# JaapWijnen/metal-raytracing

Hardware: AMD Instinct MI355X
Metric: Mrays/sec (primary+shadow) and ms/frame, DragonScene 1920x1080 spp=1 (higher is better)
Workload: dtype f32

## Files before the change

### include/mrt_debug.h

```cpp
#ifndef MRT_DEBUG_H
#define MRT_DEBUG_H
#include "mrt_abi.h"
#ifdef __cplusplus
extern "C" {
#endif

int mrt_debug_renderer_set_option(MRTRenderer r, const char *key, double value);
int mrt_debug_renderer_get_option(MRTRenderer r, const char *key, double *value);

int mrt_debug_halton(MRTContext ctx, const int32_t *i, const int32_t *d, size_t n, float *out);
int mrt_debug_hemisphere(MRTContext ctx, const float *u2, const float *normal3, size_t n, float *out3);
int mrt_debug_seeds(MRTContext ctx, uint32_t seed, int32_t width, int32_t height, uint32_t *out);
int mrt_debug_traversal_stats(MRTScene scene, const MRTRay *rays, size_t n, int32_t any_hit, uint32_t *out8);
int mrt_debug_stream_stats(MRTScene scene, const MRTRay *rays, size_t n, int32_t any_hit, uint32_t per_wave, uint32_t *out8, size_t nwaves);
int mrt_debug_intersect_stream(MRTScene scene, const MRTRay *rays, size_t n, int32_t any_hit, MRTIntersection *out);
int mrt_debug_wide_histogram(MRTScene scene, uint32_t *out12);
int mrt_debug_read_wnodes(MRTScene scene, void *out, size_t nbytes, uint64_t *num_nodes);
int mrt_debug_read_layout(MRTScene scene, int32_t part, void *out, size_t nbytes, uint64_t *count);
int mrt_debug_scene_refits(MRTScene scene, uint32_t *out);
int mrt_debug_commit_times(MRTScene scene, double *out6);
int mrt_debug_validate(MRTScene scene);
int mrt_debug_validate_patched(MRTScene scene, uint32_t node, uint32_t word, uint32_t value);
#ifdef MRT_DIAGNOSTICS
int mrt_debug_poke_wnode(MRTScene scene, uint32_t node, uint32_t word, uint32_t value, uint32_t *old_value);
#endif
int mrt_debug_host_sah(const float *lo4, const float *hi4, uint32_t n, uint32_t *order, uint32_t *left, uint32_t *right, uint32_t *parent);
int mrt_debug_tlas_host_build(const float *lo4, const float *hi4, uint32_t n, uint32_t *rope_order, uint32_t *rope_links, uint32_t *wide_order, uint32_t *wide_pos, uint32_t *counts68);
int mrt_debug_layout_limits(uint64_t triangles, uint64_t nodes);
int mrt_debug_calibrate(MRTContext ctx, size_t table_bytes, double *out5);

#ifdef __cplusplus
}
#endif
#endif
```

### metal-raytracing_amd/_ffi.py

```python
import ctypes as C
import os

_HERE = os.path.dirname(os.path.abspath(__file__))
LIB_PATH = os.environ.get("MRT_LIB_PATH") or os.path.join(_HERE, "libmrt_hip.so")

MRT_OK = 0
MRT_ERR_INVALID_ARGUMENT, MRT_ERR_NO_DEVICE, MRT_ERR_HIP, MRT_ERR_IO, MRT_ERR_STATE, MRT_ERR_OUT_OF_MEMORY, MRT_ERR_UNSUPPORTED = 1, 2, 3, 4, 5, 6, 7


class MRTError(RuntimeError):
    def __init__(self, code, message):
        super().__init__(f"mrt error {code}: {message}")
        self.code = code


class Float3(C.Structure):
    _fields_ = [("x", C.c_float), ("y", C.c_float), ("z", C.c_float), ("_pad", C.c_float)]

    def __init__(self, x=0.0, y=0.0, z=0.0):
        super().__init__(float(x), float(y), float(z), 0.0)

    def tolist(self):
        return [self.x, self.y, self.z]

# ... 128 lines not shown
    "mrt_scene_refit_device": (C.c_int, [_P, _P]),
    "mrt_scene_device_updates_rejected": (C.c_int, [_P, C.POINTER(C.c_uint64)]),
    "mrt_scene_set_instance_transforms_device": (C.c_int, [_P, _I32, _SZ, _P, _SZ, _P]),
    "mrt_scene_refit_instances_device": (C.c_int, [_P, _P]),
    "mrt_scene_rebuild_tlas_device": (C.c_int, [_P, _P]),
    "mrt_scene_update_blas_device": (C.c_int, [_P, _I32, _P, _SZ, _P, _SZ, _SZ, _P]),
    "mrt_scene_refit_blas_device": (C.c_int, [_P, _P]),
    "mrt_scene_resolve_hits_device": (C.c_int, [_P, _P, _P, _SZ, _P, _P]),
    "mrt_scene_interpolate_device": (C.c_int, [_P, _P, _SZ, _P, _SZ, _I32, _P, _SZ, _P]),
    "mrt_scene_vertex_offsets": (C.c_int, [_P, C.POINTER(C.c_uint64), _SZ]),
    "mrt_obj_load": (C.c_int, [C.c_char_p, C.POINTER(_P)]),
    "mrt_dragon_proxy": (C.c_int, [C.POINTER(_P)]),
    "mrt_dragon_proxy_irregular": (C.c_int, [C.POINTER(_P)]),
    "mrt_dragon_proxy_hostile": (C.c_int, [C.POINTER(_P)]),
    "mrt_bunny_proxy": (C.c_int, [C.POINTER(_P)]),
    "mrt_meshdata_free": (C.c_int, [_P]),
    "mrt_meshdata_counts": (C.c_int, [_P, C.POINTER(_SZ), _PI32]),
    "mrt_meshdata_vertices": (C.c_int, [_P, _P, _P]),
    "mrt_meshdata_submesh": (C.c_int, [_P, _I32, C.POINTER(_SZ), _P, C.POINTER(Material), C.c_char_p, _SZ]),
    "mrt_make_transform": (C.c_int, [_PF, _PF, _F, _PF]),
    "mrt_default_camera": (C.c_int, [_I32, _I32, C.POINTER(Camera)]),
    "mrt_renderer_create": (C.c_int, [_P, _P, _I32, _I32, _U32, _I32, C.POINTER(_P)]),
    "mrt_renderer_destroy": (C.c_int, [_P]),
    "mrt_renderer_resize": (C.c_int, [_P, _I32, _I32]),
    "mrt_renderer_set_camera": (C.c_int, [_P, C.POINTER(Camera)]),
    "mrt_renderer_set_uniforms": (C.c_int, [_P, C.POINTER(Uniforms)]),
    "mrt_renderer_get_uniforms": (C.c_int, [_P, C.POINTER(Uniforms)]),
    "mrt_renderer_frames_completed": (C.c_int, [_P, C.POINTER(C.c_uint64)]),
    "mrt_renderer_set_option": (C.c_int, [_P, C.c_char_p, C.c_double]),
    "mrt_renderer_get_option": (C.c_int, [_P, C.c_char_p, _P]),
    "mrt_debug_renderer_set_option": (C.c_int, [_P, C.c_char_p, C.c_double]),
    "mrt_debug_renderer_get_option": (C.c_int, [_P, C.c_char_p, _P]),
    "mrt_renderer_set_shard": (C.c_int, [_P, _I32, _I32]),
    "mrt_renderer_set_frame_index": (C.c_int, [_P, _U32]),
    "mrt_renderer_frame_index": (C.c_int, [_P, _PU32]),
    "mrt_renderer_render": (C.c_int, [_P, _I32]),
    "mrt_renderer_wait": (C.c_int, [_P]),
    "mrt_renderer_read_accum": (C.c_int, [_P, _P, _SZ]),
    "mrt_renderer_copy_accum_to_device": (C.c_int, [_P, _P, _SZ]),
    "mrt_renderer_write_accum_from_device": (C.c_int, [_P, _P, _SZ]),
    "mrt_renderer_shard_tiles": (C.c_int, [_P, _I32, _I32, C.POINTER(C.c_uint64)]),
    "mrt_renderer_pack_owned_tiles": (C.c_int, [_P, _P, _SZ]),
    "mrt_renderer_unpack_tiles": (C.c_int, [_P, _P, _SZ, _I32, _I32]),
    "mrt_renderer_unpack_tiles_into": (C.c_int, [_P, _P, _SZ, _P, _SZ, _I32, _I32]),
    "mrt_renderer_read_tonemapped_rgba8": (C.c_int, [_P, _P, _SZ]),
    "mrt_renderer_read_guide": (C.c_int, [_P, _I32, _P, _SZ]),
    "mrt_renderer_copy_guide_to_device": (C.c_int, [_P, _I32, _P, _SZ]),
    "mrt_renderer_denoise": (C.c_int, [_P, C.POINTER(DenoiseParams)]),
    "mrt_renderer_read_denoised": (C.c_int, [_P, _P, _SZ]),
    "mrt_renderer_copy_denoised_to_device": (C.c_int, [_P, _P, _SZ]),
    "mrt_renderer_read_denoised_tonemapped_rgba8": (C.c_int, [_P, _P, _SZ]),
    "mrt_renderer_stats": (C.c_int, [_P, C.POINTER(RenderStats)]),
    "mrt_renderer_reset_stats": (C.c_int, [_P]),
    "mrt_renderer_kernel_times": (C.c_int, [_P, C.POINTER(KernelTimes)]),
    "mrt_group_create": (C.c_int, [_PI32, _I32, C.POINTER(_P)]),
    "mrt_group_destroy": (C.c_int, [_P]),
    "mrt_group_size": (C.c_int, [_P, _PI32]),
    "mrt_group_context": (C.c_int, [_P, _I32, C.POINTER(_P)]),
    "mrt_group_reduce_mode": (C.c_int, [_P, _PI32, C.c_char_p, _SZ]),
    "mrt_group_set_reduce_mode": (C.c_int, [_P, _I32]),
    "mrt_group_renderer_create": (C.c_int, [_P, _P, _I32, _I32, _U32, _I32, C.POINTER(_P)]),
    "mrt_group_renderer_destroy": (C.c_int, [_P]),
    "mrt_group_renderer_rank": (C.c_int, [_P, _I32, C.POINTER(_P)]),
    "mrt_group_set_option": (C.c_int, [_P, C.c_char_p, C.c_double]),
    "mrt_group_set_camera": (C.c_int, [_P, C.POINTER(Camera)]),
    "mrt_group_render": (C.c_int, [_P, _I32]),
    "mrt_group_wait": (C.c_int, [_P]),
    "mrt_group_frames_completed": (C.c_int, [_P, C.POINTER(C.c_uint64)]),
    "mrt_group_gather": (C.c_int, [_P, _P, _SZ]),
    "mrt_group_gathered_device_ptr": (C.c_int, [_P, C.POINTER(_P)]),
    "mrt_group_stats": (C.c_int, [_P, C.POINTER(RenderStats)]),
    "mrt_debug_halton": (C.c_int, [_P, _P, _P, _SZ, _P]),
    "mrt_debug_hemisphere": (C.c_int, [_P, _P, _P, _SZ, _P]),
    "mrt_debug_seeds": (C.c_int, [_P, _U32, _I32, _I32, _P]),
    "mrt_debug_traversal_stats": (C.c_int, [_P, _P, _SZ, _I32, _P]),
    "mrt_debug_intersect_stream": (C.c_int, [_P, _P, _SZ, _I32, _P]),
    "mrt_debug_stream_stats": (C.c_int, [_P, _P, _SZ, _I32, _U32, _P, _SZ]),
    "mrt_debug_calibrate": (C.c_int, [_P, _SZ, _P]),
    "mrt_debug_wide_histogram": (C.c_int, [_P, _P]),
    "mrt_debug_commit_times": (C.c_int, [_P, _P]),
    "mrt_debug_read_wnodes": (C.c_int, [_P, _P, _SZ, C.POINTER(C.c_uint64)]),
    "mrt_debug_read_layout": (C.c_int, [_P, _I32, _P, _SZ, C.POINTER(C.c_uint64)]),
    "mrt_debug_layout_limits": (C.c_int, [C.c_uint64, C.c_uint64]),
    "mrt_debug_host_sah": (C.c_int, [_P, _P, _U32, _P, _P, _P, _P]),
    "mrt_debug_tlas_host_build": (C.c_int, [_P, _P, _U32, _P, _P, _P, _P, _P]),
    "mrt_debug_validate": (C.c_int, [_P]),
    "mrt_debug_validate_patched": (C.c_int, [_P, _U32, _U32, _U32]),
}

os.environ.setdefault("GPU_MAX_HW_QUEUES", "16")

if not os.path.exists(LIB_PATH):
    raise ImportError(
        f"{LIB_PATH} is missing: the HIP extension has not been built. Run `python -c 'import __graft_entry__ as g; g.build()'` "
        "or `make -C metal-raytracing_amd/csrc`. There is no CPU fallback for the render path.")



def _share_hip_runtime_with_torch():
    import sys
    if "torch" in sys.modules or os.environ.get("MRT_HIP_RUNTIME", "") == "system":
        return None
    try:
        import importlib.util
        spec = importlib.util.find_spec("torch")
    except (ImportError, ValueError):
        return None
    if spec is None or not spec.submodule_search_locations:
        return None
    libdir = os.path.join(list(spec.submodule_search_locations)[0], "lib")
    loaded = []
    for name in ("libhsa-runtime64.so", "libamdhip64.so"):
        path = os.path.join(libdir, name)
        if os.path.exists(path):
            try:
                C.CDLL(path)
                loaded.append(path)
            except OSError:
                return loaded
    return loaded


HIP_RUNTIME_PRELOADED = _share_hip_runtime_with_torch()
lib = C.CDLL(LIB_PATH)
for _name, (_res, _args) in SIGNATURES.items():
    if os.environ.get("MRT_LIB_PATH") and not hasattr(lib, _name):
        continue
    _fn = getattr(lib, _name)
    _fn.restype, _fn.argtypes = _res, _args


def check(rc):
    if rc != MRT_OK:
        raise MRTError(rc, lib.mrt_last_error().decode("utf-8", "replace"))


def ptr(a):
    return a.ctypes.data_as(C.c_void_p)
```

### metal-raytracing_amd/csrc/api.cpp

```cpp
#include "api_types.h"
#include "abi_check.h"
#include "../../include/mrt_debug.h"
#include <algorithm>
#include <cstring>
#include <cstdio>
#include <memory>
#include <new>

namespace mrt {
static thread_local std::string g_err;
void set_error(const std::string &msg) { g_err = msg; }
int hip_fail(hipError_t e, const char *what, const char *file, int line) {
    char buf[512];
    snprintf(buf, sizeof buf, "HIP error %d (%s) in %s at %s:%d", (int)e, hipGetErrorString(e), what, file, line);
    g_err = buf;
    return e == hipErrorOutOfMemory ? MRT_ERR_OUT_OF_MEMORY : MRT_ERR_HIP;
}
}

static int bind_device(MRTContext ctx) { MRT_HIP(hipSetDevice(ctx->device)); return MRT_OK; }

static int sync_host_meshes(MRTScene scene) {
    bool pending = false;
    int rc = mrt::download_stale_meshes(scene->meshes, scene->dev, &pending);
// ... 650 lines not shown
int mrt_renderer_resize(MRTRenderer r, int32_t width, int32_t height) {
    MRT_TRY
    RENDERER_PROLOGUE("mrt_renderer_resize")
    REQUIRE(width > 0 && height > 0 && (int64_t)width * height < (1ll << 30), "mrt_renderer_resize: bad size");
    MRT_HIP(hipStreamSynchronize(r->r.stream));
    return r->r.resize(width, height);
    MRT_CATCH
}
int mrt_renderer_set_camera(MRTRenderer r, const MRTCamera *camera) {
    REQUIRE(r && camera, "mrt_renderer_set_camera: bad argument");
    r->r.camera = *camera;
    return MRT_OK;
}
int mrt_renderer_set_uniforms(MRTRenderer r, const MRTUniforms *u) {
    MRT_TRY
    RENDERER_PROLOGUE("mrt_renderer_set_uniforms")
    REQUIRE(u, "mrt_renderer_set_uniforms: uniforms is NULL");
    REQUIRE(u->width > 0 && u->height > 0 && (int64_t)u->width * u->height < (1ll << 30), "mrt_renderer_set_uniforms: bad size");
    REQUIRE(u->lightCount >= 1 && u->lightCount <= r->scene->dev.light_count, "mrt_renderer_set_uniforms: lightCount must be in [1, lights of the scene]");
    if (u->width != r->r.width || u->height != r->r.height) {
        MRT_HIP(hipStreamSynchronize(r->r.stream));
        int rc = r->r.resize(u->width, u->height); if (rc) return rc;
    }
    r->r.frame_index = u->frameIndex;
    r->r.light_count_limit = u->lightCount == r->scene->dev.light_count ? 0 : u->lightCount;
    r->r.camera = u->camera;
    return MRT_OK;
    MRT_CATCH
}
int mrt_renderer_get_uniforms(MRTRenderer r, MRTUniforms *u) {
    REQUIRE(r && u, "mrt_renderer_get_uniforms: bad argument");
    memset(u, 0, sizeof *u);
    u->width = r->r.width; u->height = r->r.height; u->blocksWide = (r->r.width + 7) / 8;
    u->frameIndex = r->r.frame_index;
    u->lightCount = r->r.light_count_limit > 0 ? std::min(r->r.light_count_limit, r->scene->dev.light_count) : r->scene->dev.light_count;
    u->camera = r->r.camera;
    return MRT_OK;
}
int mrt_renderer_frames_completed(MRTRenderer r, uint64_t *frames) {
    MRT_TRY
    RENDERER_PROLOGUE("mrt_renderer_frames_completed")
    REQUIRE(frames, "mrt_renderer_frames_completed: NULL");
    return r->r.poll_completed(frames);
    MRT_CATCH
}
int mrt_renderer_set_option(MRTRenderer r, const char *key, double value) {
    MRT_TRY
    REQUIRE(r && key, "mrt_renderer_set_option: bad argument");
    std::string k(key);
    if (k == "max_bounces") { REQUIRE(value >= 1 && value <= (r->r.materials ? 16 : 19), "max_bounces must be in [1,19] ([1,16] with materials = 1)"); r->r.max_bounces = (int)value; }
    else if (k == "frames_in_flight") { REQUIRE(value >= 1 && value <= mrt::MAX_FRAMES_IN_FLIGHT, "frames_in_flight must be in [1,16]"); r->r.frames_in_flight = (int)value; }
    else if (k == "sample_offset") { REQUIRE(value >= 0 && value < 4294967296.0, "sample_offset out of range"); r->r.sample_offset = (uint32_t)value; }
    else if (k == "frame_batch") { REQUIRE(value >= 0 && value <= mrt::MAX_FRAME_BATCH, "frame_batch must be in [1,32], or 0 for the default (by image size)"); r->r.frame_batch = (int)value; }
    else if (k == "megakernel") r->r.megakernel = value != 0;
    else if (k == "guides") { REQUIRE(value == 0 || value == 1, "guides must be 0 or 1"); int rc = bind_device(r->ctx); if (rc) return rc; r->r.stream = r->ctx->stream; rc = r->r.set_guides(value != 0); if (rc) return rc; }
    else if (k == "materials") { REQUIRE(value == 0 || (value == 1 && r->r.max_bounces <= 16), "materials must be 0 or 1 (and max_bounces <= 16: the lobe choice uses Halton dimension 2 + 5 * max_bounces + bounce < 100)"); r->r.materials = value != 0; }
    else { mrt::set_error("mrt_renderer_set_option: unknown key " + k + " (keys: max_bounces, frames_in_flight, sample_offset, frame_batch, megakernel, materials, guides; the library's A/B switches are behind mrt_debug_renderer_set_option)"); return MRT_ERR_INVALID_ARGUMENT; }
    return MRT_OK;
    MRT_CATCH
}
int mrt_renderer_get_option(MRTRenderer r, const char *key, double *value) {
    MRT_TRY
    REQUIRE(r && key && value, "mrt_renderer_get_option: bad argument");
    std::string k(key);
    if (k == "max_bounces") *value = r->r.max_bounces;
    else if (k == "frames_in_flight") *value = r->r.frames_in_flight;
    else if (k == "sample_offset") *value = r->r.sample_offset;
    else if (k == "frame_batch") *value = r->r.batch_wanted();
    else if (k == "megakernel") *value = r->r.megakernel ? 1 : 0;
    else if (k == "materials") *value = r->r.materials ? 1 : 0;
    else if (k == "guides") *value = r->r.guides ? 1 : 0;
    else if (k == "lanes_used") *value = r->r.lanes_used;
    else if (k == "lane_bytes") *value = (double)r->r.lane_bytes();
    else { mrt::set_error("mrt_renderer_get_option: unknown key " + k); return MRT_ERR_INVALID_ARGUMENT; }
    return MRT_OK;
    MRT_CATCH
}
int mrt_debug_renderer_set_option(MRTRenderer r, const char *key, double value) {
    MRT_TRY
    REQUIRE(r && key, "mrt_debug_renderer_set_option: bad argument");
    std::string k(key);
    if (k == "persistent") { REQUIRE(value == 0 || value == 1 || value == 2, "persistent must be 0 (never), 1 (always) or 2 (by launch size)"); r->r.persistent = (int)value; }
    else if (k == "xcd_counters") { REQUIRE(value == 0 || value == 1, "xcd_counters must be 0 or 1"); r->r.xcd_counters = (int)value; }
    else if (k == "tile_groups") { REQUIRE(value >= 0 && value <= mrt::MAX_TILE_GROUPS && value == (int)value, "tile_groups must be 0 (by the draw), 1 (never) or 2..4"); r->r.tile_groups = (int)value; }
    else if (k == "shade_pack") { REQUIRE(value == 0 || value == 1, "shade_pack must be 0 or 1"); r->r.shade_pack = (int)value; }
    else if (k == "hit_lds") { REQUIRE(value == 0 || value == 1, "hit_lds must be 0 or 1"); r->r.hit_lds = (int)value; }
    else if (k == "persist_chunk") { REQUIRE(value >= 64 && value <= 65536 && ((int)value % 64) == 0, "persist_chunk must be a multiple of 64 in [64, 65536]"); r->r.persist_chunk = (int)value; }
    else if (k == "wave_slots") { REQUIRE(value >= 1 && value <= (1 << 20), "wave_slots must be in [1, 2^20]"); r->r.wave_slots = (int)value; r->r.wave_slots_user = true; }
    else if (k == "stream_stride") { REQUIRE(value >= 0 && value <= 2, "stream_stride must be 0 (contiguous ranges), 1 (round-robin batches) or 2 (round-robin for a shard's launches)"); r->r.stream_stride = (int)value; }
    else if (k == "halton_table") r->r.halton_table = value != 0;
    else if (k == "equal_passes") r->r.equal_passes = value != 0;
    else if (k == "frame_bundle") { REQUIRE(value == 0 || value == 1, "frame_bundle must be 0 (off) or 1 (the sub-frames of a slot side by side in a wave)"); r->r.frame_bundle = (int)value; }
    else if (k == "stream_even") { REQUIRE(value >= 0 && value <= 1600, "stream_even must be in [0,1600] (percent of the wave slots; 0 = off)"); r->r.stream_even = (int)value; }
    else if (k == "primary_hint") r->r.primary_hint = value != 0;
    else if (k == "throughput_chain") r->r.throughput_chain = value != 0;
    else if (k == "shadow_planes") r->r.shadow_planes = value != 0 ? 1 : 0;
    else if (k == "tail_accumulate") r->r.tail_accumulate = value != 0;
    else if (k == "fuse_primary") { REQUIRE(value == 0 || value == 1 || value == 2, "fuse_primary must be 0, 1 (not for one frame alone) or 2 (always)"); r->r.fuse_primary = (int)value; }
    else if (k == "wide_bounce") r->r.wide_bounce = value != 0;
    else if (k == "tl_pair_cap") { REQUIRE(value >= 0 && value <= 4294967295.0, "tl_pair_cap out of range"); r->r.tl_pair_cap = (int)std::min(value, 2147483647.0); }
    else if (k == "tl_pairs") { REQUIRE(value == 0 || value == 1 || value == 2, "tl_pairs must be 0 (two-level scenes walked in one loop), 1 (TLAS pass + BLAS pass over (ray, instance) pairs) or 2 (the same, the TLAS pass always as a walk of the 8-wide TLAS)"); r->r.tl_pairs = (int)value; }
    else if (k == "primary_wide") { REQUIRE(value == 0 || value == 1 || value == 2, "primary_wide must be 0 (rope walk inside shade(0)), 1 (own launch of the 8-wide stream kernel) or 2 (8-wide walk inside shade(0))"); r->r.primary_wide = (int)value; }
    else return mrt_renderer_set_option(r, key, value);
    return MRT_OK;
    MRT_CATCH
}
int mrt_debug_renderer_get_option(MRTRenderer r, const char *key, double *value) {
    MRT_TRY
    REQUIRE(r && key && value, "mrt_debug_renderer_get_option: bad argument");
    std::string k(key);
    if (k == "persistent") *value = r->r.persistent;
    else if (k == "persist_chunk") *value = r->r.persist_chunk;
    else if (k == "hit_lds") *value = r->r.hit_lds;
    else if (k == "shade_pack") *value = r->r.shade_pack;
    else if (k == "tile_groups") *value = r->r.tile_groups;
    else if (k == "groups_used") *value = r->r.groups_used;
    else if (k == "xcd_counters") *value = r->r.xcd_counters;
    else if (k == "wave_slots") *value = r->r.wave_slots;
    else if (k == "stream_stride") *value = r->r.stream_stride;
    else if (k == "halton_table") *value = r->r.halton_table;
    else if (k == "frame_bundle") *value = r->r.frame_bundle;
    else if (k == "stream_even") *value = r->r.stream_even;
    else if (k == "primary_hint") *value = r->r.primary_hint ? 1 : 0;
    else if (k == "throughput_chain") *value = r->r.throughput_chain ? 1 : 0;
    else if (k == "shadow_planes") *value = r->r.shadow_planes;
    else if (k == "tail_accumulate") *value = r->r.tail_accumulate ? 1 : 0;
    else if (k == "fuse_primary") *value = r->r.fuse_primary;
    else if (k == "wide_bounce") *value = r->r.wide_bounce ? 1 : 0;
    else if (k == "tl_pairs") *value = r->r.tl_pairs;
    else if (k == "tl_pair_cap") *value = r->r.tl_pair_cap;
    else if (k == "primary_wide") *value = r->r.primary_wide;
    else return mrt_renderer_get_option(r, key, value);
    return MRT_OK;
    MRT_CATCH
}
int mrt_renderer_set_shard(MRTRenderer r, int32_t rank, int32_t world) {
    MRT_TRY
    RENDERER_PROLOGUE("mrt_renderer_set_shard")
    return r->r.set_shard(rank, world);
    MRT_CATCH
}
int mrt_renderer_set_frame_index(MRTRenderer r, uint32_t fi) { REQUIRE(r, "mrt_renderer_set_frame_index: NULL"); r->r.frame_index = fi; return MRT_OK; }
int mrt_renderer_frame_index(MRTRenderer r, uint32_t *fi) { REQUIRE(r && fi, "mrt_renderer_frame_index: bad argument"); *fi = r->r.frame_index; return MRT_OK; }
int mrt_renderer_render(MRTRenderer r, int32_t n_frames) {
    MRT_TRY
    RENDERER_PROLOGUE("mrt_renderer_render")
    REQUIRE(n_frames >= 0, "mrt_renderer_render: n_frames < 0");
    if (!r->scene->committed) { mrt::set_error("mrt_renderer_render: scene was modified and not re-committed"); return MRT_ERR_STATE; }
    if (n_frames == 0) return MRT_OK;
    return r->r.render(n_frames);
    MRT_CATCH
}
int mrt_renderer_wait(MRTRenderer r) {
    MRT_TRY
    RENDERER_PROLOGUE("mrt_renderer_wait")
    return r->r.wait();
    MRT_CATCH
}
int mrt_renderer_read_accum(MRTRenderer r, float *rgba, size_t nbytes) {
    MRT_TRY
    RENDERER_PROLOGUE("mrt_renderer_read_accum")
    REQUIRE(rgba, "mrt_renderer_read_accum: NULL buffer");
    return r->r.read_accum(rgba, nbytes);
    MRT_CATCH
}
int mrt_renderer_copy_accum_to_device(MRTRenderer r, void *dptr, size_t nbytes) {
    MRT_TRY
    RENDERER_PROLOGUE("mrt_renderer_copy_accum_to_device")
    REQUIRE(dptr, "mrt_renderer_copy_accum_to_device: NULL pointer");
    return r->r.copy_accum_to_device(dptr, nbytes);
    MRT_CATCH
}
int mrt_renderer_write_accum_from_device(MRTRenderer r, const void *dptr, size_t nbytes) {
    MRT_TRY
    RENDERER_PROLOGUE("mrt_renderer_write_accum_from_device")
    REQUIRE(dptr, "mrt_renderer_write_accum_from_device: NULL pointer");
    return r->r.write_accum_from_device(dptr, nbytes);
    MRT_CATCH
}
int mrt_renderer_shard_tiles(MRTRenderer r, int32_t rank, int32_t world, uint64_t *tiles) {
    REQUIRE(r && tiles && world >= 1 && rank >= 0 && rank < world, "mrt_renderer_shard_tiles: bad argument");
    *tiles = mrt::shard_tiles(r->r.width, r->r.height, rank, world);
    return MRT_OK;
}
int mrt_renderer_pack_owned_tiles(MRTRenderer r, void *dptr, size_t nbytes) {
    MRT_TRY
    RENDERER_PROLOGUE("mrt_renderer_pack_owned_tiles")
    REQUIRE(dptr || nbytes == 0, "mrt_renderer_pack_owned_tiles: NULL pointer");
    return r->r.pack_owned_tiles(dptr, nbytes);
    MRT_CATCH
}
int mrt_renderer_unpack_tiles(MRTRenderer r, const void *dptr, size_t nbytes, int32_t rank, int32_t world) {
    MRT_TRY
    RENDERER_PROLOGUE("mrt_renderer_unpack_tiles")
    REQUIRE(dptr || nbytes == 0, "mrt_renderer_unpack_tiles: NULL pointer");
    return r->r.unpack_tiles(dptr, nbytes, rank, world);
    MRT_CATCH
}
int mrt_renderer_unpack_tiles_into(MRTRenderer r, void *image, size_t image_nbytes, const void *dptr, size_t nbytes, int32_t rank, int32_t world) {
    MRT_TRY
// ... 121 lines not shown
int mrt_debug_read_layout(MRTScene scene, int32_t part, void *out, size_t nbytes, uint64_t *count) {
    MRT_TRY
    REQUIRE(scene && count, "mrt_debug_read_layout: bad argument");
    REQUIRE(part >= 0 && part <= 7, "mrt_debug_read_layout: part must be 0 .. 7");
    if (!scene->committed) { mrt::set_error("mrt_debug_read_layout: scene not committed"); return MRT_ERR_STATE; }
    const mrt::DeviceScene &d = scene->dev;
    const size_t npk = d.wpackets.p ? d.wpackets.n / mrt::WPK : 0, ninst = d.num_inst, nwt = (d.num_inst && d.wtlas_index.p) ? d.wtlas_index.n : 0;
    uint32_t header[8] = {d.num_wnodes, d.num_inst ? d.tlas_wcap : 0u, d.num_inst, (uint32_t)d.wide_depth, (uint32_t)npk, (uint32_t)d.blas_wdepth, (uint32_t)nwt, mrt::WPK};
    const size_t nrope = d.num_inst ? d.rope_nodes : 0, ntl = d.num_inst ? d.tlas_instances : 0;
    const size_t elem[8] = {16 * (size_t)mrt::WNODE_STRIDE, 16 * (size_t)mrt::WPK, sizeof(mrt::InstanceDev), 64, 4, 4, 64, 4};
    const size_t n[8] = {d.num_wnodes, npk, ninst, ninst, nwt, 8, nrope, ntl};
    const void *src[8] = {d.wnodes.p, d.wpackets.p, d.inst.p, d.inst_box.p, d.wtlas_index.p, header, d.nodes.p, d.tlas_index.p};
    *count = n[part];
    if (out == nullptr) return MRT_OK;
    REQUIRE(nbytes == n[part] * elem[part], "mrt_debug_read_layout: nbytes must be count x the element size of the part");
    if (n[part] == 0) return MRT_OK;
    if (part == 5) { memcpy(out, header, sizeof(header)); return MRT_OK; }
    int rc = bind_device(scene->ctx); if (rc) return rc;
    MRT_HIP(hipMemcpy(out, src[part], nbytes, hipMemcpyDeviceToHost));
    return MRT_OK;
    MRT_CATCH
}
int mrt_debug_scene_refits(MRTScene scene, uint32_t *out) {
    REQUIRE(scene && out, "mrt_debug_scene_refits: bad argument");
    *out = scene->dev.refits;
    return MRT_OK;
}
int mrt_debug_commit_times(MRTScene scene, double *out6) {
    REQUIRE(scene && out6, "mrt_debug_commit_times: bad argument");
    for (int k = 0; k < 6; k++) out6[k] = scene->dev.commit_ms[k];
    return MRT_OK;
}
int mrt_debug_validate(MRTScene scene) {
    MRT_TRY
    REQUIRE(scene, "mrt_debug_validate: scene is NULL");
    if (!scene->committed) { mrt::set_error("mrt_debug_validate: scene not committed"); return MRT_ERR_STATE; }
    int rc = bind_device(scene->ctx); if (rc) return rc;
    return mrt::validate_layout(scene->dev, scene->ctx->stream, false);
    MRT_CATCH
}
int mrt_debug_validate_patched(MRTScene scene, uint32_t node, uint32_t word, uint32_t value) {
    MRT_TRY
    REQUIRE(scene && scene->committed && node < scene->dev.num_wnodes && word < 4 * mrt::WNODE_STRIDE, "mrt_debug_validate_patched: bad argument");
    int rc = bind_device(scene->ctx); if (rc) return rc;
    mrt::DevBuf<float4> copy; MRT_HIP(copy.alloc(scene->dev.wnodes.n));
    MRT_HIP(hipMemcpy(copy.p, scene->dev.wnodes.p, scene->dev.wnodes.bytes(), hipMemcpyDeviceToDevice));
    MRT_HIP(hipMemcpy(reinterpret_cast<uint32_t *>(copy.p + (size_t)mrt::WNODE_STRIDE * node) + word, &value, 4, hipMemcpyHostToDevice));
    return mrt::validate_layout(scene->dev, scene->ctx->stream, false, copy.p);
    MRT_CATCH
}
#ifdef MRT_DIAGNOSTICS
int mrt_debug_poke_wnode(MRTScene scene, uint32_t node, uint32_t word, uint32_t value, uint32_t *old_value) {
    MRT_TRY
    REQUIRE(scene && scene->committed && node < scene->dev.num_wnodes && word < 4 * mrt::WNODE_STRIDE, "mrt_debug_poke_wnode: bad argument");
    int rc = bind_device(scene->ctx); if (rc) return rc;
    uint32_t *p = reinterpret_cast<uint32_t *>(scene->dev.wnodes.p + (size_t)mrt::WNODE_STRIDE * node) + word;
    if (old_value) MRT_HIP(hipMemcpy(old_value, p, 4, hipMemcpyDeviceToHost));
    MRT_HIP(hipMemcpy(p, &value, 4, hipMemcpyHostToDevice));
    return MRT_OK;
    MRT_CATCH
}
#endif
int mrt_debug_host_sah(const float *lo4, const float *hi4, uint32_t n, uint32_t *order, uint32_t *left, uint32_t *right, uint32_t *parent) {
    MRT_TRY
    REQUIRE(lo4 && hi4 && n >= 1 && order && left && right && parent, "mrt_debug_host_sah: bad argument");
    std::vector<uint32_t> o, l, r, p;
    mrt::host_sah_topology(reinterpret_cast<const float4 *>(lo4), reinterpret_cast<const float4 *>(hi4), n, o, l, r, p);
    memcpy(order, o.data(), (size_t)n * 4); memcpy(parent, p.data(), (2 * (size_t)n - 1) * 4);
    if (n > 1) { memcpy(left, l.data(), (size_t)(n - 1) * 4); memcpy(right, r.data(), (size_t)(n - 1) * 4); }
    return MRT_OK;
    MRT_CATCH
}
int mrt_debug_tlas_host_build(const float *lo4, const float *hi4, uint32_t n, uint32_t *rope_order, uint32_t *rope_links, uint32_t *wide_order, uint32_t *wide_pos, uint32_t *counts68) {
    MRT_TRY
    REQUIRE(lo4 && hi4 && n >= 1 && n <= 65536 && rope_order && rope_links && wide_order && wide_pos && counts68, "mrt_debug_tlas_host_build: bad argument");
    return mrt::tlas_host_build(lo4, hi4, n, rope_order, rope_links, wide_order, wide_pos, counts68);
    MRT_CATCH
}
int mrt_debug_layout_limits(uint64_t triangles, uint64_t nodes) {
    MRT_TRY
    return mrt::layout_limits(triangles, nodes);
    MRT_CATCH
}
int mrt_debug_calibrate(MRTContext ctx, size_t table_bytes, double *out3) {
    MRT_TRY
    REQUIRE(ctx && out3 && table_bytes >= 4096 && table_bytes <= ((size_t)1 << 34), "mrt_debug_calibrate: bad argument");
    int rc = bind_device(ctx); if (rc) return rc;
    return mrt::calibrate(ctx->stream, table_bytes, out3);
    MRT_CATCH
}

}
```

### metal-raytracing_amd/csrc/renderer.h

```cpp
#pragma once
#include "scene_device.h"
#include "host_geometry.h"
#include <algorithm>
#include <array>
#include <deque>
#include <vector>

namespace mrt {

struct EvPair { hipEvent_t a = nullptr, b = nullptr; int kind = 0; };

struct FrameLane {
    hipStream_t stream = nullptr;
    hipEvent_t accumulated = nullptr;
    DevBuf<float4> sample;
    DevBuf<float4> rayA[2], rayB[2], thr[2], hits, srayA, srayB, scon;
    DevBuf<unsigned long long> bounce_counts;
    DevBuf<float4> f_con[2];
    DevBuf<uint8_t> f_lit;
    DevBuf<uint4> pairs;
};
constexpr int MAX_FRAMES_IN_FLIGHT = 16;
constexpr int MAX_TILE_GROUPS = 4;
struct TileGroup { int rank = 0, world = 1, tiles_local = 0; uint32_t capacity = 0; uint64_t owned = 0; const uint32_t *seeds = nullptr; };
constexpr int MAX_FRAME_BATCH = 32;
constexpr int DEFAULT_FRAME_BATCH = 8;

struct DrawPlan {
    int n_frames = 0;
    bool mega = false;
    bool equal = true, tail = true;
    int batch_max = 1;
    int n_passes = 0;
    int G = 1;
    int lanes = 1;
    int lanes_plain = 1;
    int Fp = 1;
    int tail_from = 0;
    bool long_call = false;
    int pass_size(int p) const { return equal ? n_frames / n_passes + (p < n_frames % n_passes ? 1 : 0) : std::min(batch_max, n_frames - p * batch_max); }
    void settle(int lanes_ready);
};

enum class PrimaryForm { none, stream, lane_wide, rope };
enum class TraceForm { pairs, pull_x, pull, static_x, static_split, rope };
struct PullGrid { uint32_t chunk = 0, waves = 0; size_t grid_slots = 0; };
struct PassPlan {
    int B = 0;
    uint32_t grid_tiles = 1, grid_shade = 1;
    bool two_level = false, on_wide = false, chain = false, planes = false, pairs = false, tl_flat = false, prim_rope = false;
    bool trace0_pass = false, trace0_wide = false, trace0_hint = false, primary_hinted = false, bundle = false, pull = false, strided = false;
    PrimaryForm primary = PrimaryForm::none;
    TraceForm trace = TraceForm::rope;
    size_t stack_bytes = 0, trace_lds = 0, pair_cap = 0;
    uint32_t pair_cap_used = 0, rpw_p = 0, rpw_m = 0, pack_range = 0;
    int wave_slots = 0;
    PullGrid pg;
    uint32_t even = 0, static_grid = 0;
    uint32_t mega_waves = 0;
};
struct SlotCache { size_t lds_bytes = ~(size_t)0; int per_cu = 0; };
struct DrawCtx;

struct Renderer {
    hipStream_t stream = nullptr;
    const DeviceScene *scene = nullptr;
    int width = 0, height = 0, max_bounces = 3;
    uint32_t seed = 1;
    MRTCamera camera{};
    uint32_t frame_index = 0;
    uint32_t sample_offset = 0;
    int cur = 0;
    int shard_rank = 0, shard_world = 1;
    int tiles_local = 0;
    uint32_t capacity = 0;
    uint64_t owned_pixels = 0;
    uint64_t frames_rendered = 0;

    DevBuf<uint32_t> seeds;
    DevBuf<float> halton_tab;
    uint32_t halton_w0 = 0;
    int halton_table = 1;
    int ensure_halton_table(uint32_t sample_index, uint32_t frames);
    DevBuf<uint32_t> hint;
    bool primary_hint = true;
    bool throughput_chain = true;
    DevBuf<float4> accum[2];
    FrameLane lanes[MAX_FRAMES_IN_FLIGHT];
    int frames_in_flight = 3;
    int frame_batch = 0;
    int batch_wanted() const;
    int tile_groups = 0;
    int groups_used = 1;
    TileGroup tgroups[MAX_TILE_GROUPS];
    DevBuf<uint32_t> seeds_g[MAX_TILE_GROUPS]; int tgroups_for = 0, tgroups_batch = 0;
    int ensure_tile_groups(int G);
    int lanes_used = 0;
    int lanes_ready = 0;
    int alloc_batch = 0;
    bool megakernel = false;
    bool materials = false;
    int primary_wide = 2;
    int persistent = 2;
    int xcd_counters = 1;
    int hit_lds = 1;
    int shade_pack = 1;
    int persist_chunk = 256;
    int wave_slots = 7168;
    bool wave_slots_user = false;
    mutable SlotCache mega_cache, persist_cache, persist_x_cache;
    mutable int cu_count = 0;
    int alloc_planes(FrameLane &L);
    bool tail_accumulate = true;
    int fuse_primary = 1;
    int shadow_planes = 1;
    int equal_passes = 1;
    int frame_bundle = 1;
    int stream_stride = 2;
    int stream_even = 200;
    int tl_pair_cap = 0;
    int tl_pairs = 1;
    bool wide_bounce = true;
    hipEvent_t ev_fork = nullptr;
    DevBuf<unsigned long long> totals;

    bool guides = false;
    bool guides_valid = false;
    bool guides_keep = false;
    DevBuf<float4> guide_nd, guide_albedo; DevBuf<int4> guide_ids;
    hipStream_t guide_stream = nullptr;
    hipEvent_t guide_fork = nullptr, guide_done = nullptr;
    DevBuf<float4> dn_scratch[2], denoised; bool denoised_valid = false;
    int set_guides(bool on);
    int ensure_guides();
    int clear_guides();
    int read_guide(int which, void *out, size_t nbytes);
    int copy_guide_to_device(int which, void *dptr, size_t nbytes);
    int enqueue_denoise(const MRTDenoiseParams *params);
    int read_denoised(float *rgba, size_t nbytes);
    int copy_denoised_to_device(void *dptr, size_t nbytes);
    int read_denoised_tonemapped(uint8_t *rgba, size_t nbytes);

    int light_count_limit = 0;
    struct PassDone { hipEvent_t ev; uint64_t frames_through; };
    std::deque<PassDone> passes_pending;
    std::vector<hipEvent_t> pass_events_free;
    uint64_t frames_completed_known = 0;
    int note_pass(hipStream_t st);
    int poll_completed(uint64_t *out);

    hipEvent_t ev_begin = nullptr, ev_end = nullptr;
    std::array<EvPair, 512> ev_ext;
    int ext_used = 0;
    bool pending_timing = false;
    float ms_last = 0, ms_extend_last = 0; uint32_t extend_launches_last = 0;
    MRTKernelTimes kernel_times{};

    Renderer() = default;
    Renderer(const Renderer &) = delete;
    ~Renderer();
    int init(hipStream_t st, const DeviceScene *sc, int w, int h, uint32_t seed, int max_bounces);
    int resize(int w, int h);
    int alloc_queues();
    int alloc_lane(FrameLane &L);
    void release_lane(FrameLane &L);
    size_t lane_bytes() const;
    int set_shard(int rank, int world);
    int render(int n_frames);
    DrawPlan plan_draw(int n_frames) const;
    int plan_pass(const DrawPlan &dp, const SceneView &sv, const TileGroup &TG, int B, PassPlan &pp) const;
    PullGrid pull_grid(size_t slots, size_t slots_of_chip, size_t min_chunk, bool long_call) const;
    int draw_nothing(int n_frames);
    int rebuild_for_batch();
    int ensure_lanes(int want);
    void begin_draw(DrawCtx &d) const;
    int prepare_lane(FrameLane &L, const TileGroup &TG, const PassPlan &pp);
    int enqueue_pass(DrawCtx &d, FrameLane &L, const TileGroup &TG, const PassPlan &pp, int pass, int g);
    int enqueue_megakernel_pass(DrawCtx &d, FrameLane &L, const TileGroup &TG, const PassPlan &pp);
    void enqueue_primary(DrawCtx &d, FrameLane &L, const TileGroup &TG, const PassPlan &pp);
    void enqueue_shade(DrawCtx &d, FrameLane &L, const TileGroup &TG, const PassPlan &pp, int b);
    void enqueue_trace(DrawCtx &d, FrameLane &L, const TileGroup &TG, const PassPlan &pp, int b);
    int enqueue_accumulate(DrawCtx &d, FrameLane &L, const TileGroup &TG, const PassPlan &pp, int pass, int g);
    int enqueue_guides(DrawCtx &d);
    EvPair *timed(int kind);
    int wait();
    int read_accum(float *rgba, size_t nbytes);
    int copy_accum_to_device(void *dptr, size_t nbytes);
    int write_accum_from_device(const void *dptr, size_t nbytes);
    int read_tonemapped(uint8_t *rgba, size_t nbytes);
    int pack_owned_tiles(void *dptr, size_t nbytes);
    int unpack_tiles(const void *dptr, size_t nbytes, int rank, int world);
    int stats(MRTRenderStats *out);
    int reset_stats();
// ... 19 lines not shown
```

### metal-raytracing_amd/csrc/renderer.hip

```cpp
#include <hip/hip_ext.h>
#include "renderer.h"
#include "device_math.h"
#include "traverse.h"
#include "traverse_wide.h"
#include "traverse_instanced.h"
#include "shade.h"
#include "two_level_passes.h"
#include <cstdlib>
#include <cstring>
#include <algorithm>

namespace mrt {
namespace {

__global__ void k_halton_table(float *__restrict__ tab, uint32_t w0, uint32_t n) {
    const uint32_t j = blockIdx.x * blockDim.x + threadIdx.x;
    if (j < n) tab[MRT_HALTON_INTERLEAVED ? (size_t)j * HALTON_TAB_DIMS + blockIdx.y : (size_t)blockIdx.y * n + j] = halton_dev((int)(w0 + j), (int)blockIdx.y + 1);
}

__global__ void k_seed(uint32_t *__restrict__ seeds, uint32_t n, uint32_t seed) {
    uint32_t i = blockIdx.x * blockDim.x + threadIdx.x;
    if (i < n) seeds[(size_t)blockIdx.y * n + i] = seed_hash_dev(seed, i) + blockIdx.y;
}

// ... 81 lines not shown
#else
constexpr uint32_t WIDE_STREAM_RAYS_FIXED = 0;
#endif
static inline uint32_t stream_rays_per_wave(size_t slots) {
    if (WIDE_STREAM_RAYS_FIXED) return WIDE_STREAM_RAYS_FIXED;
    const size_t batches = slots / 64 / 10240;
    return 64u * (uint32_t)std::min<size_t>(16, std::max<size_t>(6, batches));
}
template <bool TWO_LEVEL>
__global__ void __launch_bounds__(64, TWO_LEVEL ? MRT_TWO_LEVEL_WAVES : MRT_WIDE_STREAM_WAVES) k_trace_mixed_wide_stream(SceneView s, const float4 *__restrict__ rayA, const float4 *__restrict__ rayB, float4 *__restrict__ hits,
                                                                const float4 *__restrict__ srayA, const float4 *__restrict__ srayB, const float4 *__restrict__ scon,
                                                                const unsigned long long *__restrict__ counts, float4 *__restrict__ sample, uint32_t rays_per_wave, uint8_t *__restrict__ lit, uint32_t even_waves) {
    extern __shared__ uint32_t stk_dyn[];
    const unsigned long long c = *counts;
    const uint32_t n_next = (uint32_t)c, n_shadow = (uint32_t)(c >> 32), n = n_next + n_shadow;
    if (even_waves) rays_per_wave = max(64u, ((n + even_waves - 1u) / even_waves + 63u) & ~63u);
    const uint32_t begin = blockIdx.x * rays_per_wave;
    if (begin >= n) return;
    traverse_wide_stream<TWO_LEVEL>(s, OneRange{begin, min(n, begin + rays_per_wave)}, stk_dyn,
        [&](uint32_t i, float4 &A, float4 &B, uint32_t &tag, uint32_t &is_any) {
            const bool sh = i >= n_next; tag = sh ? i - n_next : i; is_any = sh ? 1u : 0u;
            A = qload(sh ? &srayA[tag] : &rayA[tag]); B = qload(sh ? &srayB[tag] : &rayB[tag]);
            if (!sh) A.w = __builtin_inff();
            else if (lit) tag = __float_as_uint(B.w);
        },
        [&](uint32_t j, bool is_any, bool hit, const TravHit &h) {
            if (is_any) {
                if (!hit) {
                    if (lit) lit[4 * (size_t)j] = 1;
                    else { const uint32_t pix = __float_as_uint(srayB[j].w); float4 cc = qload(&scon[j]), a = q2load(&sample[pix]); q2store(&sample[pix], make_float4(a.x + cc.x, a.y + cc.y, a.z + cc.z, 0.0f)); }
                }
            } else {
                qstore(&hits[j], hit ? make_float4(h.t, h.U / h.ad, h.V / h.ad, __uint_as_float(h.gid)) : make_float4(-1.0f, 0.0f, 0.0f, __uint_as_float(0xFFFFFFFFu)));
            }
        });
}

#ifdef MRT_WAVE_TIMES
__device__ unsigned long long g_wave_times[2 * 8192];
__device__ uint32_t g_wave_iters[4 * 8192];
__device__ unsigned long long g_drain_probe[2][9];
#endif
template <bool TWO_LEVEL>
__global__ void __launch_bounds__(64, TWO_LEVEL ? MRT_TWO_LEVEL_WAVES : MRT_WIDE_STREAM_WAVES) k_trace_mixed_wide_persist(SceneView s, const float4 *__restrict__ rayA, const float4 *__restrict__ rayB, float4 *__restrict__ hits,
                                                                const float4 *__restrict__ srayA, const float4 *__restrict__ srayB, const float4 *__restrict__ scon,
                                                                const unsigned long long *__restrict__ counts, float4 *__restrict__ sample, uint32_t *__restrict__ work, uint32_t chunk, uint8_t *__restrict__ lit, uint32_t subframes ) {
    extern __shared__ uint32_t stk_dyn[];
    const unsigned long long c = *counts;
    const uint32_t n_next = (uint32_t)c, n_shadow = (uint32_t)(c >> 32), n = n_next + n_shadow;
#ifdef MRT_WAVE_TIMES
    const uint32_t wt_tag = chunk >> 24; chunk &= 0xFFFFFFu;
    const unsigned long long wt0 = wall_clock64();
    StreamStats wst{0, 0, 0, 0, 0, 0};
    struct WT { unsigned long long t0; uint32_t tag; StreamStats &st; __device__ ~WT() { if ((threadIdx.x & 63) == 0 && tag == 0 && blockIdx.x < 8192) {
        g_wave_times[2 * blockIdx.x] = t0; g_wave_times[2 * blockIdx.x + 1] = wall_clock64();
        g_wave_iters[4 * blockIdx.x] = st.iters | (st.drain_le8 << 16); g_wave_iters[4 * blockIdx.x + 1] = st.drain_iters | (st.maxdt << 12); g_wave_iters[4 * blockIdx.x + 2] = st.drain_live; g_wave_iters[4 * blockIdx.x + 3] = (uint32_t)st.drain_t0; } } } wt{wt0, wt_tag, wst};
#endif
    if (blockIdx.x * chunk >= n) return;
    auto fetch = [&](uint32_t i, float4 &A, float4 &B, uint32_t &tag, uint32_t &is_any) {
            const bool sh = i >= n_next; tag = sh ? i - n_next : i; is_any = sh ? 1u : 0u;
            A = qload(sh ? &srayA[tag] : &rayA[tag]); B = qload(sh ? &srayB[tag] : &rayB[tag]);
            if (!sh) A.w = __builtin_inff();
            else if (lit) tag = __float_as_uint(B.w);
        };
    auto emit = [&](uint32_t j, bool is_any, bool hit, const TravHit &h) {
            if (is_any) {
                if (!hit) {
                    if (lit) lit[4 * (size_t)j] = 1;
                    else { const uint32_t pix = __float_as_uint(srayB[j].w); float4 cc = qload(&scon[j]), a = q2load(&sample[pix]); q2store(&sample[pix], make_float4(a.x + cc.x, a.y + cc.y, a.z + cc.z, 0.0f)); }
                }
            } else {
                qstore(&hits[j], hit ? make_float4(h.t, h.U / h.ad, h.V / h.ad, __uint_as_float(h.gid)) : make_float4(-1.0f, 0.0f, 0.0f, __uint_as_float(0xFFFFFFFFu)));
            }
        };
#ifdef MRT_WAVE_TIMES
    StreamStats *const wss = wt_tag == 0 ? &wst : nullptr;
#else
    StreamStats *const wss = nullptr;
#endif
    if constexpr (TWO_LEVEL) traverse_wide_stream<true>(s, SharedCounter{work, n, chunk}, stk_dyn, fetch, emit, wss);
    else traverse_wide_stream<false>(s, XcdRegions{work, n_next, n, chunk, subframes, blockIdx.x & 7u}, stk_dyn, fetch, emit, wss);
}

__global__ void __launch_bounds__(64, MRT_WIDE_STREAM_WAVES) k_trace_mixed_wide_persist_x(SceneView s, const float4 *__restrict__ rayA, const float4 *__restrict__ rayB, float4 *__restrict__ hits,
                                                                const float4 *__restrict__ srayA, const float4 *__restrict__ srayB, const unsigned long long *__restrict__ counts,
                                                                uint32_t *__restrict__ work, uint32_t chunk, uint8_t *__restrict__ lit, uint32_t subframes) {
    extern __shared__ uint32_t lds_dyn[];
    const unsigned long long c = *counts;
    const uint32_t n_next = (uint32_t)c, n_shadow = (uint32_t)(c >> 32), n = n_next + n_shadow;
    if (blockIdx.x * chunk >= n) return;
    auto fetch = [&](uint32_t i, float4 &A, float4 &B, uint32_t &tag, uint32_t &is_any) {
            const bool sh = i >= n_next; tag = sh ? i - n_next : i; is_any = sh ? 1u : 0u;
            A = qload(sh ? &srayA[tag] : &rayA[tag]); B = qload(sh ? &srayB[tag] : &rayB[tag]);
            if (!sh) A.w = __builtin_inff();
            else tag = __float_as_uint(B.w);
        };
    auto emit = [&](uint32_t j, bool is_any, bool hit, const TravHit &h) {
            if (is_any) { if (!hit) lit[4 * (size_t)j] = 1; }
            else qstore(&hits[j], hit ? make_float4(h.t, h.U / h.ad, h.V / h.ad, __uint_as_float(h.gid)) : make_float4(-1.0f, 0.0f, 0.0f, __uint_as_float(0xFFFFFFFFu)));
        };
    StreamExt<true> ext{reinterpret_cast<float *>(lds_dyn), lds_dyn + 256u};
    traverse_wide_stream<false, false, false, NoPairs, StreamExt<true>>(s, XcdRegions{work, n_next, n, chunk, subframes, blockIdx.x & 7u}, lds_dyn + HIT_LDS_WORDS, fetch, emit, nullptr, NoPairs{}, ext);
}

__global__ void __launch_bounds__(64, MRT_WIDE_STREAM_WAVES) k_trace_mixed_wide_stream_x(SceneView s, const float4 *__restrict__ rayA, const float4 *__restrict__ rayB, float4 *__restrict__ hits,
                                                                const float4 *__restrict__ srayA, const float4 *__restrict__ srayB, const unsigned long long *__restrict__ counts,
                                                                uint32_t rays_per_wave, uint8_t *__restrict__ lit, uint32_t even_waves) {
    extern __shared__ uint32_t lds_dyn[];
    const unsigned long long c = *counts;
    const uint32_t n_next = (uint32_t)c, n_shadow = (uint32_t)(c >> 32), n = n_next + n_shadow;
#ifdef MRT_WAVE_TIMES
    const uint32_t wt_tag = rays_per_wave >> 24; rays_per_wave &= 0xFFFFFFu;
    StreamStats wst{0, 0, 0, 0, 0, 0};
    struct WT { unsigned long long t0; uint32_t tag; StreamStats &st; __device__ ~WT() { if ((threadIdx.x & 63) == 0 && tag == 0 && blockIdx.x < 8192) {
        g_wave_times[2 * blockIdx.x] = t0; g_wave_times[2 * blockIdx.x + 1] = wall_clock64();
        g_wave_iters[4 * blockIdx.x] = st.iters | (st.drain_le8 << 16); g_wave_iters[4 * blockIdx.x + 1] = st.drain_iters | (st.maxdt << 12); g_wave_iters[4 * blockIdx.x + 2] = st.drain_live; g_wave_iters[4 * blockIdx.x + 3] = (uint32_t)st.drain_t0; }
        if ((threadIdx.x & 63) == 0 && tag == 0) for (int c_ = 0; c_ < 2; c_++) { for (int d_ = 0; d_ < 6; d_++) atomicAdd(&g_drain_probe[c_][d_], (unsigned long long)st.dr_hist[c_][d_]);
            atomicAdd(&g_drain_probe[c_][6], (unsigned long long)st.dr_kids[c_]); atomicAdd(&g_drain_probe[c_][7], (unsigned long long)st.dr_tris[c_]); atomicAdd(&g_drain_probe[c_][8], (unsigned long long)st.dr_n[c_]); } } } wt{(unsigned long long)wall_clock64(), wt_tag, wst};
    StreamStats *const wss = wt_tag == 0 ? &wst : nullptr;
#else
    StreamStats *const wss = nullptr;
#endif
    const bool strided = (even_waves >> 31) != 0u; even_waves &= 0x7FFFFFFFu;
    if (even_waves) rays_per_wave = max(64u, ((n + even_waves - 1u) / even_waves + 63u) & ~63u);
    const uint32_t begin = blockIdx.x * rays_per_wave;
    if (begin >= n) return;
    StreamExt<true> ext{reinterpret_cast<float *>(lds_dyn), lds_dyn + 256u};
    const BatchStride src = strided ? BatchStride{blockIdx.x * 64u, 64u * ((n + rays_per_wave - 1u) / rays_per_wave), n} : BatchStride{begin, 64u, min(n, begin + rays_per_wave)};
    traverse_wide_stream<false, false, false, NoPairs, StreamExt<true>>(s, src, lds_dyn + HIT_LDS_WORDS,
        [&](uint32_t i, float4 &A, float4 &B, uint32_t &tag, uint32_t &is_any) {
            const bool sh = i >= n_next; tag = sh ? i - n_next : i; is_any = sh ? 1u : 0u;
            A = qload(sh ? &srayA[tag] : &rayA[tag]); B = qload(sh ? &srayB[tag] : &rayB[tag]);
            if (!sh) A.w = __builtin_inff();
            else tag = __float_as_uint(B.w);
        },
        [&](uint32_t j, bool is_any, bool hit, const TravHit &h) {
            if (is_any) { if (!hit) lit[4 * (size_t)j] = 1; }
            else qstore(&hits[j], hit ? make_float4(h.t, h.U / h.ad, h.V / h.ad, __uint_as_float(h.gid)) : make_float4(-1.0f, 0.0f, 0.0f, __uint_as_float(0xFFFFFFFFu)));
        }, wss, NoPairs{}, ext);
}

#include "megakernel.h"
#include "guides.h"

template <bool TWO_LEVEL, bool SEED>
__global__ void __launch_bounds__(64, 5) k_trace_primary_wide_stream(SceneView s, FrameParams fp, const uint32_t *__restrict__ seeds, float4 *__restrict__ hits, float4 *__restrict__ dirs, uint32_t capacity, uint32_t rays_per_wave,
                                                                     uint32_t *__restrict__ hint ) {
    extern __shared__ uint32_t stk_dyn[];
    const uint32_t begin = blockIdx.x * rays_per_wave, sub = blockIdx.y;
    if (begin >= capacity) return;
    hits += (size_t)sub * capacity; dirs += (size_t)sub * capacity;
    auto make_ray = [&](uint32_t slot, float4 &A, float4 &B, uint32_t &tag, uint32_t &is_any, f3 &org, f3 &dir, int &x, int &y) -> bool {
        is_any = 0u; tag = slot;
        if (slot_to_pixel(fp, slot, x, y)) {
            primary_ray(fp, seeds, sub * fp.capacity + slot, x, y, org, dir);
            A = make_float4(org.x, org.y, org.z, __builtin_inff()); B = make_float4(dir.x, dir.y, dir.z, 0.0f);
            dirs[slot] = make_float4(dir.x, dir.y, dir.z, __uint_as_float(sub * fp.capacity + slot));
            return true;
        }
        A = make_float4(0.0f, 0.0f, 0.0f, -1.0f); B = make_float4(0.0f, 0.0f, 1.0f, 0.0f);
        return false;
    };
    if constexpr (SEED) {
        traverse_wide_stream<TWO_LEVEL, true>(s, OneRange{begin, min(capacity, begin + rays_per_wave)}, stk_dyn,
            [&](uint32_t slot, float4 &A, float4 &B, uint32_t &tag, uint32_t &is_any, uint32_t &seed) {
                f3 org, dir; int x, y;
                seed = 0xFFFFFFFFu;
                if (!make_ray(slot, A, B, tag, is_any, org, dir, x, y)) return;
                const uint32_t guess = hint[(uint32_t)y * (uint32_t)fp.width + (uint32_t)x];
                const uint32_t pk = TWO_LEVEL ? (guess & 0xFFFFFFu) : guess, in = TWO_LEVEL ? guess >> 24 : 0u;
                if (guess == 0xFFFFFFFFu) return;
                float t, U, V, ad;
                if (TWO_LEVEL) {
                    if (in >= s.num_inst) return;
                    const InstanceDev &I = s.inst[in];
                    if (pk - I.packet_base >= I.ntri) return;
                    const float4 *__restrict__ q = s.wpackets + WPK * (size_t)pk;
                    if (tri_test(q[0], q[1], q[2], to_object_point(I, org), to_object_dir(I, dir), 0.0f, __builtin_inff(), t, U, V, ad)) { A.w = t; seed = guess; }
                } else {
                    if (pk >= s.num_tris) return;
                    const float4 *__restrict__ q = s.wpackets + WPK * (size_t)pk;
                    if (tri_test(q[0], q[1], q[2], org, dir, 0.0f, __builtin_inff(), t, U, V, ad)) { A.w = t; seed = guess; }
                }
            },
            [&](uint32_t slot, bool, bool hit, const TravHit &h) {
                hits[slot] = hit ? make_float4(h.t, h.U / h.ad, h.V / h.ad, __uint_as_float(h.gid)) : make_float4(-1.0f, 0.0f, 0.0f, __uint_as_float(0xFFFFFFFFu));
                int x, y;
                if (hit && slot_to_pixel(fp, slot, x, y)) hint[(uint32_t)y * (uint32_t)fp.width + (uint32_t)x] = h.pk;
            });
    } else {
        traverse_wide_stream<TWO_LEVEL>(s, OneRange{begin, min(capacity, begin + rays_per_wave)}, stk_dyn,
            [&](uint32_t slot, float4 &A, float4 &B, uint32_t &tag, uint32_t &is_any) { f3 org, dir; int x, y; (void)make_ray(slot, A, B, tag, is_any, org, dir, x, y); },
            [&](uint32_t slot, bool, bool hit, const TravHit &h) {
                hits[slot] = hit ? make_float4(h.t, h.U / h.ad, h.V / h.ad, __uint_as_float(h.gid)) : make_float4(-1.0f, 0.0f, 0.0f, __uint_as_float(0xFFFFFFFFu));
            });
    }
}

constexpr size_t WORK_COUNTERS = 128, WORK_COUNTERS_PER_BOUNCE = 8 * XCD_COUNTER_STRIDE / 2;
__global__ void __launch_bounds__(64) k_accumulate(FrameParams fp, const float4 *__restrict__ sample, const float4 *__restrict__ prev, float4 *__restrict__ dst,
                                                   unsigned long long *__restrict__ bounce_counts, unsigned long long *__restrict__ totals, uint32_t primary) {
    if (blockIdx.x == 0 && threadIdx.x == 0) {
        unsigned long long closest = primary, shadow = 0;
        for (int b = 0; b < fp.max_bounces; b++) {
            unsigned long long c = bounce_counts[b];
            if (b + 1 < fp.max_bounces) closest += (uint32_t)c;
            shadow += c >> 32;
            bounce_counts[b] = 0;
            bounce_counts[32 + b] = 0;
            for (int x = 0; x < 8; x++) reinterpret_cast<uint32_t *>(bounce_counts + WORK_COUNTERS + (size_t)b * WORK_COUNTERS_PER_BOUNCE)[x * XCD_COUNTER_STRIDE] = 0;
            bounce_counts[65 + b] = 0;
        }
        atomicAdd(&totals[0], closest); atomicAdd(&totals[1], shadow); atomicAdd(&totals[2], (unsigned long long)primary);
    }
    uint32_t slot = blockIdx.x * 64 + threadIdx.x;
    int x, y;
    if (!slot_to_pixel(fp, slot, x, y)) return;
    uint32_t pix = (uint32_t)y * (uint32_t)fp.width + (uint32_t)x;
    float4 c = make_float4(0.0f, 0.0f, 0.0f, 0.0f);
    for (int sub = 0; sub < fp.batch; sub++) {
        const float4 sm = qload(&sample[(size_t)sub * fp.capacity + slot]);
        const uint32_t frame = fp.frameIndex + (uint32_t)sub;
        if (frame > 0) {
            const float4 p = sub == 0 ? q2load(&prev[pix]) : c;
            float fi = (float)frame;
            float den = (float)(frame + 1);
            c.x = (sm.x + p.x * fi) / den; c.y = (sm.y + p.y * fi) / den; c.z = (sm.z + p.z * fi) / den;
        } else c = sm;
    }
    q2store(&dst[pix], make_float4(c.x, c.y, c.z, 1.0f));
}

MRT_DEV float4 planes_sample(const float4 *const (&con)[3], const uint8_t *__restrict__ lit, int max_bounces, size_t sp) {
    float4 sm = make_float4(0.0f, 0.0f, 0.0f, 0.0f);
    const uint32_t flags = reinterpret_cast<const uint32_t *>(lit)[sp];
#pragma unroll
    for (int b = 0; b < 3; b++)
        if (b < max_bounces && ((flags >> (8 * b)) & 0xFFu) != 0u) { const float4 cc = qload(&con[b][sp]); sm = make_float4(sm.x + cc.x, sm.y + cc.y, sm.z + cc.z, 0.0f); }
    return sm;
}
__global__ void __launch_bounds__(64) k_accumulate_planes(FrameParams fp, const float4 *__restrict__ con0, const float4 *__restrict__ con1, const float4 *__restrict__ con2, const uint8_t *__restrict__ lit,
                                                          const float4 *__restrict__ prev, float4 *__restrict__ dst, unsigned long long *__restrict__ bounce_counts, unsigned long long *__restrict__ totals, uint32_t primary) {
    if (blockIdx.x == 0 && threadIdx.x == 0) {
        unsigned long long closest = primary, shadow = 0;
        for (int b = 0; b < fp.max_bounces; b++) {
            unsigned long long c = bounce_counts[b];
            if (b + 1 < fp.max_bounces) closest += (uint32_t)c;
            shadow += c >> 32;
            bounce_counts[b] = 0;
            bounce_counts[32 + b] = 0;
            for (int x = 0; x < 8; x++) reinterpret_cast<uint32_t *>(bounce_counts + WORK_COUNTERS + (size_t)b * WORK_COUNTERS_PER_BOUNCE)[x * XCD_COUNTER_STRIDE] = 0;
            bounce_counts[65 + b] = 0;
        }
        atomicAdd(&totals[0], closest); atomicAdd(&totals[1], shadow); atomicAdd(&totals[2], (unsigned long long)primary);
    }
    const uint32_t slot = blockIdx.x * 64 + threadIdx.x;
    int x, y;
    if (!slot_to_pixel(fp, slot, x, y)) return;
    const uint32_t pix = (uint32_t)y * (uint32_t)fp.width + (uint32_t)x;
    const float4 *const con[3] = {con0, con1, con2};
    float4 c = make_float4(0.0f, 0.0f, 0.0f, 0.0f);
    for (int sub = 0; sub < fp.batch; sub++) {
        const float4 sm = planes_sample(con, lit, fp.max_bounces, (size_t)sub * fp.capacity + slot);
        const uint32_t frame = fp.frameIndex + (uint32_t)sub;
        if (frame > 0) {
            const float4 p = sub == 0 ? q2load(&prev[pix]) : c;
            const float fi = (float)frame, den = (float)(frame + 1);
            c.x = (sm.x + p.x * fi) / den; c.y = (sm.y + p.y * fi) / den; c.z = (sm.z + p.z * fi) / den;
        } else c = sm;
    }
    q2store(&dst[pix], make_float4(c.x, c.y, c.z, 1.0f));
}

struct AccPass { const float4 *con0, *con1, *con2; const uint8_t *lit; unsigned long long *counts; uint32_t frameIndex; int32_t batch; uint32_t primary; uint32_t pad; };
struct AccGroup { AccPass p[MAX_FRAMES_IN_FLIGHT]; int32_t n; };
__global__ void __launch_bounds__(64) k_accumulate_planes_group(FrameParams fp, AccGroup g, const float4 *__restrict__ prev, float4 *__restrict__ dst, unsigned long long *__restrict__ totals) {
    if (blockIdx.x == 0 && threadIdx.x == 0) {
        unsigned long long closest = 0, shadow = 0, primary = 0;
        for (int p = 0; p < MAX_FRAMES_IN_FLIGHT; p++) {
            if (p >= g.n) break;
            closest += g.p[p].primary; primary += g.p[p].primary;
            for (int b = 0; b < fp.max_bounces; b++) {
                const unsigned long long c = g.p[p].counts[b];
                if (b + 1 < fp.max_bounces) closest += (uint32_t)c;
                shadow += c >> 32;
                g.p[p].counts[b] = 0; g.p[p].counts[32 + b] = 0; g.p[p].counts[65 + b] = 0;
                for (int x = 0; x < 8; x++) reinterpret_cast<uint32_t *>(g.p[p].counts + WORK_COUNTERS + (size_t)b * WORK_COUNTERS_PER_BOUNCE)[x * XCD_COUNTER_STRIDE] = 0;
            }
        }
        totals[0] += closest; totals[1] += shadow; totals[2] += primary;
    }
    const uint32_t slot = blockIdx.x * 64 + threadIdx.x;
    int x, y;
    if (!slot_to_pixel(fp, slot, x, y)) return;
    const uint32_t pix = (uint32_t)y * (uint32_t)fp.width + (uint32_t)x;
    float4 c = make_float4(0.0f, 0.0f, 0.0f, 0.0f);
    bool first = true;
    for (int p = 0; p < MAX_FRAMES_IN_FLIGHT; p++) {
        if (p >= g.n) break;
        const float4 *const con[3] = {g.p[p].con0, g.p[p].con1, g.p[p].con2};
        for (int sub = 0; sub < g.p[p].batch; sub++) {
            const float4 sm = planes_sample(con, g.p[p].lit, fp.max_bounces, (size_t)sub * fp.capacity + slot);
            const uint32_t frame = g.p[p].frameIndex + (uint32_t)sub;
            if (frame > 0) {
                const float4 q = first ? q2load(&prev[pix]) : c;
                const float fi = (float)frame, den = (float)(frame + 1);
                c.x = (sm.x + q.x * fi) / den; c.y = (sm.y + q.y * fi) / den; c.z = (sm.z + q.z * fi) / den;
            } else c = sm;
            first = false;
        }
    }
    q2store(&dst[pix], make_float4(c.x, c.y, c.z, 1.0f));
}

template <bool PACK>
__global__ void k_tiles(float4 *__restrict__ image, int w, int h, int tiles_x, int rank, int world, uint32_t tiles_local, float4 *__restrict__ compact) {
    const uint32_t slot = blockIdx.x * blockDim.x + threadIdx.x, lt = slot >> 6, k = slot & 63u;
    if (lt >= tiles_local) return;
    const uint32_t tile = lt * (uint32_t)world + (uint32_t)rank, ty = tile / (uint32_t)tiles_x, tx = tile - ty * (uint32_t)tiles_x;
    const int x = (int)(tx * 8u + (k & 7u)), y = (int)(ty * 8u + (k >> 3));
    const bool in = x < w && y < h;
    if (PACK) compact[slot] = in ? image[(size_t)y * w + x] : make_float4(0.0f, 0.0f, 0.0f, 0.0f);
    else if (in) image[(size_t)y * w + x] = compact[slot];
}

__global__ void k_tonemap(const float4 *__restrict__ accum, int w, int h, uchar4 *__restrict__ out) {
    int x = blockIdx.x * blockDim.x + threadIdx.x, y = blockIdx.y * blockDim.y + threadIdx.y;
    if (x >= w || y >= h) return;
    float4 a = accum[(size_t)(h - 1 - y) * w + x];
    float c[3] = {a.x, a.y, a.z};
    unsigned char o[3];
    for (int k = 0; k < 3; k++) { float v = c[k] / (1.0f + c[k]); v = saturatef(v); o[k] = (unsigned char)(v * 255.0f + 0.5f); }
    out[(size_t)y * w + x] = make_uchar4(o[0], o[1], o[2], 255);
}

template <bool WIDE>
__global__ void __launch_bounds__(64) k_query_closest(SceneView s, const MRTRay *__restrict__ rays, uint32_t n, MRTIntersection *__restrict__ out) {
    extern __shared__ uint32_t stk[];
    uint32_t i = blockIdx.x * 64 + threadIdx.x;
    if (i >= n) return;
    MRTRay r = rays[i];
    TravHit h;
    const f3 ro = mk3(r.origin[0], r.origin[1], r.origin[2]), rd = mk3(r.direction[0], r.direction[1], r.direction[2]);
    bool hit = s.num_inst ? traverse_instanced<false>(s, ro, rd, r.min_distance, r.max_distance, h)
             : WIDE ? traverse_wide<false>(s, ro, rd, r.min_distance, r.max_distance, h, stk) : traverse<false>(s, ro, rd, r.min_distance, r.max_distance, h);
    MRTIntersection o;
    o._pad = 0;
    if (hit) {
        uint32_t inst, geom;
        if (s.num_inst) { inst = instance_of_gid(s, h.gid); const InstanceDev &I = s.inst[inst]; geom = s.tri_shade[I.ts_base + (h.gid - I.gid_base)].w & 0xFFFFu; }
        else { const uint4 ts = s.tri_shade[h.gid]; inst = ts.w >> 16; geom = ts.w & 0xFFFFu; }
        o.type = 1; o.distance = h.t; o.instance_id = (int32_t)inst; o.geometry_id = (int32_t)geom;
        o.primitive_id = (int32_t)(h.gid - s.geom_base[inst * (uint32_t)s.max_sub + geom]);
        o.u = h.U / h.ad; o.v = h.V / h.ad;
    } else { o.type = 0; o.distance = -1.0f; o.instance_id = o.geometry_id = o.primitive_id = -1; o.u = o.v = 0.0f; }
    out[i] = o;
}
template <bool WIDE>
__global__ void __launch_bounds__(64) k_query_any(SceneView s, const MRTRay *__restrict__ rays, uint32_t n, int32_t *__restrict__ out) {
    extern __shared__ uint32_t stk[];
    uint32_t i = blockIdx.x * 64 + threadIdx.x;
    if (i >= n) return;
    MRTRay r = rays[i];
    TravHit h;
    const f3 ro = mk3(r.origin[0], r.origin[1], r.origin[2]), rd = mk3(r.direction[0], r.direction[1], r.direction[2]);
    out[i] = (s.num_inst ? traverse_instanced<true>(s, ro, rd, r.min_distance, r.max_distance, h)
              : WIDE ? traverse_wide<true>(s, ro, rd, r.min_distance, r.max_distance, h, stk) : traverse<true>(s, ro, rd, r.min_distance, r.max_distance, h)) ? 1 : 0;
}

template <bool WIDE>
// ... 89 lines not shown
template <bool TWO_LEVEL, bool ANY>
__global__ void __launch_bounds__(64, TWO_LEVEL ? MRT_TWO_LEVEL_WAVES : MRT_WIDE_STREAM_WAVES) k_query_stream_device(SceneView s, const MRTRay *__restrict__ rays, uint32_t n, void *__restrict__ out) {
    extern __shared__ uint32_t stk_dyn[];
    const uint32_t begin = blockIdx.x * QUERY_STREAM_RAYS;
    if (begin >= n) return;
    traverse_wide_stream<TWO_LEVEL>(s, OneRange{begin, min(n, begin + QUERY_STREAM_RAYS)}, stk_dyn,
        [&](uint32_t i, float4 &A, float4 &B, uint32_t &tag, uint32_t &is_any) {
            const MRTRay r = rays[i]; tag = i; is_any = ANY ? 1u : 0u;
            if (r.min_distance != 0.0f) { A = make_float4(0.0f, 0.0f, 0.0f, -1.0f); B = make_float4(0.0f, 0.0f, 1.0f, 0.0f); }
            else { A = make_float4(r.origin[0], r.origin[1], r.origin[2], r.max_distance); B = make_float4(r.direction[0], r.direction[1], r.direction[2], 0.0f); }
        },
        [&](uint32_t i, bool, bool hit, const TravHit &h) {
            if (rays[i].min_distance != 0.0f) return;
            if (ANY) static_cast<int32_t *>(out)[i] = hit ? 1 : 0;
            else static_cast<MRTIntersection *>(out)[i] = closest_record(s, TWO_LEVEL, hit, h);
        });
}
template <bool WIDE, bool ANY>
__global__ void __launch_bounds__(64) k_query_lane_device(SceneView s, const MRTRay *__restrict__ rays, uint32_t n, void *__restrict__ out) {
    extern __shared__ uint32_t stk[];
    const uint32_t i = blockIdx.x * 64 + threadIdx.x;
    const bool mine = i < n && (s.num_wnodes == 0 || rays[i].min_distance != 0.0f);
    if (__ballot(mine) == 0ull) return;
    if (!mine) return;
    const MRTRay r = rays[i];
    TravHit h;
    const f3 ro = mk3(r.origin[0], r.origin[1], r.origin[2]), rd = mk3(r.direction[0], r.direction[1], r.direction[2]);
    const bool hit = s.num_inst ? traverse_instanced<ANY>(s, ro, rd, r.min_distance, r.max_distance, h)
                   : WIDE ? traverse_wide<ANY>(s, ro, rd, r.min_distance, r.max_distance, h, stk) : traverse<ANY>(s, ro, rd, r.min_distance, r.max_distance, h);
    if (ANY) static_cast<int32_t *>(out)[i] = hit ? 1 : 0;
    else static_cast<MRTIntersection *>(out)[i] = closest_record(s, s.num_inst != 0, hit, h);
}

__global__ void k_probe_halton(const int32_t *i, const int32_t *d, uint32_t n, float *out) {
    uint32_t k = blockIdx.x * blockDim.x + threadIdx.x;
    if (k < n) out[k] = halton_dev(i[k], d[k]);
}
__global__ void k_probe_hemisphere(const float *u2, const float *n3, uint32_t n, float *out3) {
    uint32_t k = blockIdx.x * blockDim.x + threadIdx.x;
    if (k >= n) return;
    f3 v = align_hemisphere_dev(sample_cosine_hemisphere_dev(u2[2 * k], u2[2 * k + 1]), mk3(n3[3 * k], n3[3 * k + 1], n3[3 * k + 2]));
    out3[3 * k] = v.x; out3[3 * k + 1] = v.y; out3[3 * k + 2] = v.z;
}

static inline uint32_t cdiv(size_t a, size_t b) { return (uint32_t)((a + b - 1) / b); }

template <class... KArgs, class... Args>
static inline void launch_timed(EvPair *ev, void (*kernel)(KArgs...), dim3 grid, dim3 block, size_t shmem, hipStream_t st, Args... args) {
    if (ev) hipExtLaunchKernelGGL(kernel, grid, block, (uint32_t)shmem, st, ev->a, ev->b, 0, static_cast<KArgs>(args)...);
    else hipLaunchKernelGGL(kernel, grid, block, shmem, st, static_cast<KArgs>(args)...);
}

}

#ifdef MRT_WAVE_TIMES
int read_wave_times(unsigned long long *out) { return hipMemcpyFromSymbol(out, HIP_SYMBOL(g_wave_times), sizeof(g_wave_times)) == hipSuccess ? MRT_OK : MRT_ERR_HIP; }
int read_wave_iters(uint32_t *out) { return hipMemcpyFromSymbol(out, HIP_SYMBOL(g_wave_iters), sizeof(g_wave_iters)) == hipSuccess ? MRT_OK : MRT_ERR_HIP; }
int read_drain_probe(unsigned long long *out18, int reset) {
    if (hipMemcpyFromSymbol(out18, HIP_SYMBOL(g_drain_probe), sizeof(g_drain_probe)) != hipSuccess) return MRT_ERR_HIP;
    if (reset) { static const unsigned long long z[18] = {0}; if (hipMemcpyToSymbol(HIP_SYMBOL(g_drain_probe), z, sizeof z) != hipSuccess) return MRT_ERR_HIP; }
    return MRT_OK;
}
#endif

int Renderer::ensure_halton_table(uint32_t sample_index, uint32_t frames) {
    const uint64_t first_pass = std::min<uint64_t>(frames, MAX_FRAME_BATCH);
    const bool fits = halton_tab.p != nullptr && sample_index >= halton_w0 && (uint64_t)sample_index + first_pass + (1u << 20) <= (uint64_t)halton_w0 + HALTON_TAB_SPAN;
    if (fits) return MRT_OK;
    if (!halton_tab.p) MRT_HIP(halton_tab.alloc((size_t)HALTON_TAB_DIMS * HALTON_TAB_SPAN));
    halton_w0 = sample_index;
    hipLaunchKernelGGL(k_halton_table, dim3(cdiv(HALTON_TAB_SPAN, 256), HALTON_TAB_DIMS), dim3(256), 0, stream, halton_tab.p, halton_w0, HALTON_TAB_SPAN);
    MRT_HIP(hipGetLastError());
    return MRT_OK;
}

int Renderer::init(hipStream_t st, const DeviceScene *sc, int w, int h, uint32_t seed_, int max_bounces_) {
    stream = st; scene = sc; seed = seed_; max_bounces = max_bounces_;
    MRT_HIP(hipEventCreate(&ev_begin)); MRT_HIP(hipEventCreate(&ev_end));
    MRT_HIP(hipEventCreateWithFlags(&ev_fork, hipEventDisableTiming));
    for (auto &e : ev_ext) { MRT_HIP(hipEventCreate(&e.a)); MRT_HIP(hipEventCreate(&e.b)); }
    for (auto &L : lanes) {
        MRT_HIP(hipStreamCreateWithFlags(&L.stream, hipStreamNonBlocking));
        MRT_HIP(hipEventCreateWithFlags(&L.accumulated, hipEventDisableTiming));
        MRT_HIP(L.bounce_counts.alloc(WORK_COUNTERS + 32 * WORK_COUNTERS_PER_BOUNCE));
        MRT_HIP(hipMemsetAsync(L.bounce_counts.p, 0, L.bounce_counts.bytes(), stream));
    }
    MRT_HIP(totals.alloc(4));
    MRT_HIP(hipMemsetAsync(totals.p, 0, totals.bytes(), stream));
    return resize(w, h);
}

Renderer::~Renderer() {
    if (ev_begin) (void)hipEventDestroy(ev_begin);
    if (ev_end) (void)hipEventDestroy(ev_end);
    if (ev_fork) (void)hipEventDestroy(ev_fork);
    for (auto &e : ev_ext) { if (e.a) (void)hipEventDestroy(e.a); if (e.b) (void)hipEventDestroy(e.b); }
    for (auto &pd : passes_pending) (void)hipEventDestroy(pd.ev);
    for (auto e : pass_events_free) (void)hipEventDestroy(e);
    if (guide_stream) { (void)hipStreamSynchronize(guide_stream); (void)hipStreamDestroy(guide_stream); }
    if (guide_done) (void)hipEventDestroy(guide_done);
    if (guide_fork) (void)hipEventDestroy(guide_fork);
    for (auto &L : lanes) {
        if (L.stream) { (void)hipStreamSynchronize(L.stream); (void)hipStreamDestroy(L.stream); }
        if (L.accumulated) (void)hipEventDestroy(L.accumulated);
    }
}

int Renderer::batch_wanted() const {
    if (frame_batch > 0) return std::min(frame_batch, MAX_FRAME_BATCH);
    const size_t owned = std::max<size_t>(1, (size_t)std::max(width, 1) * (size_t)std::max(height, 1) / (size_t)std::max(shard_world, 1));
    const size_t ref = (size_t)DEFAULT_FRAME_BATCH * 1920 * 1080;
    return (int)std::min<size_t>(MAX_FRAME_BATCH, std::max<size_t>(DEFAULT_FRAME_BATCH, (ref + owned - 1) / owned));
}

int Renderer::resize(int w, int h) {
    width = w; height = h;
    const size_t npix = (size_t)w * h;
    const int B = batch_wanted();
    alloc_batch = B;
    MRT_HIP(hint.alloc(npix));
    MRT_HIP(hipMemsetAsync(hint.p, 0xFF, hint.bytes(), stream));
    MRT_HIP(accum[0].alloc(npix)); MRT_HIP(accum[1].alloc(npix));
    MRT_HIP(hipMemsetAsync(accum[0].p, 0, accum[0].bytes(), stream));
    MRT_HIP(hipMemsetAsync(accum[1].p, 0, accum[1].bytes(), stream));
    default_camera(w, h, &camera);
    frame_index = 0; cur = 0;
    MRT_HIP(hipMemsetAsync(totals.p, 0, totals.bytes(), stream));
    frames_rendered = 0;
    for (auto &pd : passes_pending) pass_events_free.push_back(pd.ev);
    passes_pending.clear(); frames_completed_known = 0;
    denoised_valid = false;
    if (guides && !guides_keep) {
        if (guide_nd.p && guide_nd.n != npix) { guide_nd.release(); guide_albedo.release(); guide_ids.release(); }
        for (auto &b : dn_scratch) b.release();
        denoised.release();
        if (int rc = clear_guides()) return rc;
    }
    return alloc_queues();
}

int Renderer::note_pass(hipStream_t st) {
    if (passes_pending.size() < 1024 || passes_pending.empty()) {
        hipEvent_t e = nullptr;
        if (!pass_events_free.empty()) { e = pass_events_free.back(); pass_events_free.pop_back(); }
        else MRT_HIP(hipEventCreateWithFlags(&e, hipEventDisableTiming));
        passes_pending.push_back(PassDone{e, frames_rendered});
    } else passes_pending.back().frames_through = frames_rendered;
    MRT_HIP(hipEventRecord(passes_pending.back().ev, st));
    return MRT_OK;
}
int Renderer::poll_completed(uint64_t *out) {
    while (!passes_pending.empty()) {
        const hipError_t q = hipEventQuery(passes_pending.front().ev);
        if (q == hipErrorNotReady) { (void)hipGetLastError(); break; }
        if (q != hipSuccess) return hip_fail(q, "hipEventQuery", __FILE__, __LINE__);
        frames_completed_known = passes_pending.front().frames_through;
        pass_events_free.push_back(passes_pending.front().ev);
        passes_pending.pop_front();
    }
    *out = frames_completed_known;
    return MRT_OK;
}

int Renderer::alloc_queues() {
    const int tiles_x = (width + 7) / 8, tiles_y = (height + 7) / 8;
    const int tiles = tiles_x * tiles_y;
    tiles_local = (tiles - shard_rank + shard_world - 1) / shard_world;
    if (tiles_local < 0) tiles_local = 0;
    capacity = (uint32_t)tiles_local * 64u;
    {
        const int B = std::max(1, alloc_batch);
        MRT_HIP(seeds.alloc((size_t)std::max<uint32_t>(capacity, 1u) * B));
        FrameParams sp{}; sp.width = width; sp.height = height; sp.shard_rank = shard_rank; sp.shard_world = shard_world; sp.tiles_x = tiles_x; sp.tiles_local = tiles_local; sp.capacity = capacity;
        if (capacity) hipLaunchKernelGGL(k_seed_slots, dim3(cdiv(capacity, 256), B), dim3(256), 0, stream, seeds.p, sp, seed);
    }
    tgroups_for = 0;
    lanes_ready = 0;
    for (auto &L : lanes) release_lane(L);
    uint64_t owned = 0;
    for (int lt = 0; lt < tiles_local; lt++) {
        int tile = lt * shard_world + shard_rank, ty = tile / tiles_x, tx = tile % tiles_x;
        int pw = std::min(8, width - tx * 8), ph = std::min(8, height - ty * 8);
        owned += (uint64_t)pw * ph;
    }
    owned_pixels = owned;
    return MRT_OK;
}

constexpr int PLANES_MAX_BOUNCES = 3;

size_t Renderer::lane_bytes() const {
    const size_t qcap = (size_t)capacity * (size_t)std::max(1, alloc_batch);
    const bool need_thr = !(throughput_chain && !materials && max_bounces <= 3);
    const size_t spix = (size_t)std::max<uint32_t>(capacity, 1u) * (size_t)std::max(1, alloc_batch);
    const size_t planes_bytes = shadow_planes ? 2 * spix * sizeof(float4) + spix * 4 : 0;
    const bool need_scon = need_thr || !shadow_planes;
    const size_t pairs_bytes = (scene && scene->num_inst && scene->num_wnodes && tl_pairs && shadow_planes && !need_thr) ? 2 * PairQueue::WORDS * qcap * sizeof(uint4) : 0;
    return ((need_thr ? 9 : 7) * qcap + (need_scon ? qcap : 0) + spix) * sizeof(float4) + planes_bytes + pairs_bytes;
}
void Renderer::release_lane(FrameLane &L) {
    for (int k = 0; k < 2; k++) { L.rayA[k].release(); L.rayB[k].release(); L.thr[k].release(); L.f_con[k].release(); }
    L.hits.release(); L.srayA.release(); L.srayB.release(); L.scon.release(); L.sample.release(); L.f_lit.release(); L.pairs.release();
}
int Renderer::alloc_planes(FrameLane &L) {
    const size_t spix = (size_t)std::max<uint32_t>(capacity, 1u) * (size_t)std::max(1, alloc_batch);
    for (int k = 0; k < 2; k++) MRT_HIP(L.f_con[k].alloc(spix));
    MRT_HIP(L.f_lit.alloc(spix * 4));
    return MRT_OK;
}
int Renderer::alloc_lane(FrameLane &L) {
    const size_t qcap = (size_t)capacity * (size_t)std::max(1, alloc_batch);
    const bool need_thr = !(throughput_chain && !materials && max_bounces <= 3);
    for (int k = 0; k < 2; k++) { MRT_HIP(L.rayA[k].alloc(qcap)); MRT_HIP(L.rayB[k].alloc(qcap)); if (need_thr) MRT_HIP(L.thr[k].alloc(qcap)); }
    MRT_HIP(L.hits.alloc(qcap)); MRT_HIP(L.srayA.alloc(qcap)); MRT_HIP(L.srayB.alloc(qcap));
    if (need_thr || !shadow_planes) MRT_HIP(L.scon.alloc(qcap));
    MRT_HIP(L.sample.alloc((size_t)std::max<uint32_t>(capacity, 1u) * (size_t)std::max(1, alloc_batch)));
    MRT_HIP(hipMemsetAsync(L.sample.p, 0, L.sample.bytes(), stream));
    if (shadow_planes && !need_thr) { if (int rc = alloc_planes(L)) return rc; }
    return MRT_OK;
}

int Renderer::ensure_tile_groups(int G) {
    const int Bq = std::max(1, alloc_batch);
    if (tgroups_for == G && tgroups_batch == Bq) return MRT_OK;
    const int tiles_x = (width + 7) / 8, tiles_y = (height + 7) / 8, tiles = tiles_x * tiles_y;
    for (int g = 0; g < G; g++) {
        TileGroup &T = tgroups[g];
        T.rank = g * shard_world + shard_rank; T.world = G * shard_world;
        T.tiles_local = std::max(0, (tiles - T.rank + T.world - 1) / T.world);
        T.capacity = (uint32_t)T.tiles_local * 64u;
        T.owned = 0;
        for (int lt = 0; lt < T.tiles_local; lt++) {
            const int tile = lt * T.world + T.rank, ty = tile / tiles_x, tx = tile % tiles_x;
            T.owned += (uint64_t)std::min(8, width - tx * 8) * (uint64_t)std::min(8, height - ty * 8);
        }
        MRT_HIP(seeds_g[g].alloc((size_t)std::max<uint32_t>(T.capacity, 1u) * Bq));
        FrameParams sp{}; sp.width = width; sp.height = height; sp.shard_rank = T.rank; sp.shard_world = T.world; sp.tiles_x = tiles_x; sp.tiles_local = T.tiles_local; sp.capacity = T.capacity;
        if (T.capacity) hipLaunchKernelGGL(k_seed_slots, dim3(cdiv(T.capacity, 256), Bq), dim3(256), 0, stream, seeds_g[g].p, sp, seed);
        T.seeds = seeds_g[g].p;
    }
    tgroups_for = G; tgroups_batch = Bq;
    return MRT_OK;
}

int Renderer::set_shard(int rank, int world) {
    if (world < 1 || rank < 0 || rank >= world) { set_error("invalid shard"); return MRT_ERR_INVALID_ARGUMENT; }
    shard_rank = rank; shard_world = world;
    MRT_HIP(hipStreamSynchronize(stream));
    MRT_HIP(hipMemsetAsync(accum[0].p, 0, accum[0].bytes(), stream));
    MRT_HIP(hipMemsetAsync(accum[1].p, 0, accum[1].bytes(), stream));
    frame_index = 0; cur = 0;
    if (int rc = clear_guides()) return rc;
    return alloc_queues();
}

int Renderer::clear_guides() {
    guides_valid = false; denoised_valid = false;
    if (guide_nd.p) {
        MRT_HIP(hipMemsetAsync(guide_nd.p, 0, guide_nd.bytes(), stream)); MRT_HIP(hipMemsetAsync(guide_albedo.p, 0, guide_albedo.bytes(), stream));
        MRT_HIP(hipMemsetAsync(guide_ids.p, 0, guide_ids.bytes(), stream));
    }
    return MRT_OK;
}
int Renderer::set_guides(bool on) {
    if (on == guides) return MRT_OK;
    guides = on;
    if (!on) {
        MRT_HIP(hipStreamSynchronize(stream));
        guide_nd.release(); guide_albedo.release(); guide_ids.release(); denoised.release();
        for (auto &b : dn_scratch) b.release();
        guides_valid = false; denoised_valid = false;
    }
    return MRT_OK;
}
int Renderer::ensure_guides() {
    const size_t npix = (size_t)width * height;
    if (!guide_stream) { MRT_HIP(hipStreamCreateWithFlags(&guide_stream, hipStreamNonBlocking)); MRT_HIP(hipEventCreateWithFlags(&guide_done, hipEventDisableTiming)); MRT_HIP(hipEventCreateWithFlags(&guide_fork, hipEventDisableTiming)); }
    if (guide_nd.p && guide_nd.n == npix) return MRT_OK;
    MRT_HIP(guide_nd.alloc(npix)); MRT_HIP(guide_albedo.alloc(npix)); MRT_HIP(guide_ids.alloc(npix));
    return clear_guides();
}
int Renderer::read_guide(int which, void *out, size_t nbytes) {
    if (which < 0 || which >= MRT_GUIDE_COUNT) { set_error("read_guide: which must be MRT_GUIDE_NORMAL_DEPTH, MRT_GUIDE_ALBEDO or MRT_GUIDE_IDS"); return MRT_ERR_INVALID_ARGUMENT; }
    if (nbytes != (size_t)width * height * 16) { set_error("read_guide: nbytes must be width*height*16"); return MRT_ERR_INVALID_ARGUMENT; }
    if (!guides || !guides_valid) { set_error("read_guide: no guide buffers (renderer option guides = 1, then render)"); return MRT_ERR_STATE; }
    int rc = wait(); if (rc) return rc;
    MRT_HIP(hipMemcpy(out, which == MRT_GUIDE_NORMAL_DEPTH ? (const void *)guide_nd.p : which == MRT_GUIDE_ALBEDO ? (const void *)guide_albedo.p : (const void *)guide_ids.p, nbytes, hipMemcpyDeviceToHost));
    return MRT_OK;
}
int Renderer::copy_guide_to_device(int which, void *dptr, size_t nbytes) {
    if (which < 0 || which >= MRT_GUIDE_COUNT) { set_error("copy_guide_to_device: which must be MRT_GUIDE_NORMAL_DEPTH, MRT_GUIDE_ALBEDO or MRT_GUIDE_IDS"); return MRT_ERR_INVALID_ARGUMENT; }
    if (nbytes != (size_t)width * height * 16) { set_error("copy_guide_to_device: nbytes must be width*height*16"); return MRT_ERR_INVALID_ARGUMENT; }
    if (!guides || !guides_valid) { set_error("copy_guide_to_device: no guide buffers (renderer option guides = 1, then render)"); return MRT_ERR_STATE; }
    MRT_HIP(hipMemcpyAsync(dptr, which == MRT_GUIDE_NORMAL_DEPTH ? (const void *)guide_nd.p : which == MRT_GUIDE_ALBEDO ? (const void *)guide_albedo.p : (const void *)guide_ids.p, nbytes, hipMemcpyDeviceToDevice, stream));
    return MRT_OK;
}
int Renderer::enqueue_denoise(const MRTDenoiseParams *params) {
    MRTDenoiseParams p{};
    if (params) p = *params;
    else { p.iterations = MRT_DENOISE_DEFAULT_ITERATIONS; p.sigma_color = MRT_DENOISE_DEFAULT_SIGMA_COLOR; p.sigma_normal = MRT_DENOISE_DEFAULT_SIGMA_NORMAL; p.sigma_depth = MRT_DENOISE_DEFAULT_SIGMA_DEPTH; p.demodulate = 1; }
    if (p.iterations < 1 || p.iterations > 8) { set_error("denoise: iterations must be in [1,8]"); return MRT_ERR_INVALID_ARGUMENT; }
    const float big = 3.0e38f;
    if (!(p.sigma_color > 0.0f && p.sigma_color < big) || !(p.sigma_normal > 0.0f && p.sigma_normal < big) || !(p.sigma_depth > 0.0f && p.sigma_depth < big)) { set_error("denoise: sigma_color, sigma_normal and sigma_depth must be finite and > 0"); return MRT_ERR_INVALID_ARGUMENT; }
    if (p.demodulate != 0 && p.demodulate != 1) { set_error("denoise: demodulate must be 0 or 1"); return MRT_ERR_INVALID_ARGUMENT; }
    if (!guides || !guides_valid) { set_error("denoise: no guide buffers (renderer option guides = 1, then render)"); return MRT_ERR_STATE; }
    if (shard_world > 1) { set_error("denoise: a sharded renderer holds only its own tiles and the filter needs a pixel's neighbours"); return MRT_ERR_STATE; }
    const size_t npix = (size_t)width * height;
    for (auto &b : dn_scratch) MRT_HIP(b.alloc(npix));
    MRT_HIP(denoised.alloc(npix));
    if (int rc = denoise_enqueue(stream, width, height, accum[cur].p, guide_nd.p, guide_albedo.p, dn_scratch[0].p, dn_scratch[1].p, denoised.p, p)) return rc;
    denoised_valid = true;
    return MRT_OK;
}
int Renderer::read_denoised(float *rgba, size_t nbytes) {
    if (nbytes != (size_t)width * height * 16) { set_error("read_denoised: nbytes must be width*height*16"); return MRT_ERR_INVALID_ARGUMENT; }
    if (!denoised_valid) { set_error("read_denoised: no denoised image (mrt_renderer_denoise first)"); return MRT_ERR_STATE; }
    int rc = wait(); if (rc) return rc;
    MRT_HIP(hipMemcpy(rgba, denoised.p, nbytes, hipMemcpyDeviceToHost));
    return MRT_OK;
}
int Renderer::copy_denoised_to_device(void *dptr, size_t nbytes) {
    if (nbytes != (size_t)width * height * 16) { set_error("copy_denoised_to_device: nbytes must be width*height*16"); return MRT_ERR_INVALID_ARGUMENT; }
    if (!denoised_valid) { set_error("copy_denoised_to_device: no denoised image (mrt_renderer_denoise first)"); return MRT_ERR_STATE; }
    MRT_HIP(hipMemcpyAsync(dptr, denoised.p, nbytes, hipMemcpyDeviceToDevice, stream));
    return MRT_OK;
}
int Renderer::read_denoised_tonemapped(uint8_t *rgba, size_t nbytes) {
    if (nbytes != (size_t)width * height * 4) { set_error("read_denoised_tonemapped: nbytes must be width*height*4"); return MRT_ERR_INVALID_ARGUMENT; }
    if (!denoised_valid) { set_error("read_denoised_tonemapped: no denoised image (mrt_renderer_denoise first)"); return MRT_ERR_STATE; }
    DevBuf<uchar4> tmp; MRT_HIP(tmp.alloc((size_t)width * height));
    hipLaunchKernelGGL(k_tonemap, dim3(cdiv(width, 16), cdiv(height, 16)), dim3(16, 16), 0, stream, (const float4 *)denoised.p, width, height, tmp.p);
    int rc = wait(); if (rc) return rc;
    MRT_HIP(hipMemcpy(rgba, tmp.p, nbytes, hipMemcpyDeviceToHost));
    return MRT_OK;
}

#ifdef MRT_DIAGNOSTICS
static inline int ablate_mask() { static const int mask = getenv("MRT_ABLATE") ? atoi(getenv("MRT_ABLATE")) : 0; return mask; }
#else
static constexpr int ablate_mask() { return 0; }
#endif
static inline uint32_t tag_bounce(uint32_t arg, int b) {
#ifdef MRT_WAVE_TIMES
    return arg | ((uint32_t)b << 24);
#else
    (void)b; return arg;
#endif
}

struct DrawCtx {
    SceneView sv;
    DrawPlan dp;
    FrameParams fp;
    FrameParams gp;
    hipEvent_t last_acc, last_acc_g[MAX_TILE_GROUPS];
    AccGroup tail;
};

template <class K>
static int wave_slots_for(K kernel, size_t lds_bytes, SlotCache &cache, int &cu_count) {
    if (cu_count == 0) { int dev = 0; hipDeviceProp_t prop; MRT_HIP(hipGetDevice(&dev)); MRT_HIP(hipGetDeviceProperties(&prop, dev)); cu_count = prop.multiProcessorCount; }
    if (cache.lds_bytes != lds_bytes) { MRT_HIP(hipOccupancyMaxActiveBlocksPerMultiprocessor(&cache.per_cu, kernel, 64, lds_bytes)); cache.lds_bytes = lds_bytes; }
    return MRT_OK;
}

EvPair *Renderer::timed(int kind) { if (ext_used >= (int)ev_ext.size()) return nullptr; ev_ext[ext_used].kind = kind; return &ev_ext[ext_used++]; }

DrawPlan Renderer::plan_draw(int n_frames) const {
    DrawPlan dp;
    dp.n_frames = n_frames; dp.mega = megakernel; dp.equal = equal_passes != 0; dp.tail = tail_accumulate;
    const int batch_cap = alloc_batch > DEFAULT_FRAME_BATCH ? std::min(alloc_batch, std::max(DEFAULT_FRAME_BATCH, (n_frames + 2) / 3)) : alloc_batch;
    dp.batch_max = megakernel ? 1 : batch_cap;
    dp.n_passes = (n_frames + dp.batch_max - 1) / dp.batch_max;
    dp.lanes = dp.lanes_plain = std::max(1, std::min(frames_in_flight, MAX_FRAMES_IN_FLIGHT));
    if (!megakernel && tile_groups != 1 && tiles_local >= 64) {
        const int in_flight = std::max(1, std::min(dp.lanes, dp.n_passes));
        const int by_draw = tile_groups >= 2 ? tile_groups : dp.batch_max > 1 ? 1 : in_flight == 1 ? 3 : in_flight <= 3 ? 2 : 1;
        dp.G = std::max(1, std::min(by_draw, std::min(MAX_FRAMES_IN_FLIGHT / in_flight, tiles_local / 32)));
        if (dp.G > 1) dp.lanes = in_flight * dp.G;
    }
    return dp;
}

void DrawPlan::settle(int lanes_ready) {
    if (G > 1 && lanes_ready < lanes) { G = 1; lanes = lanes_plain; }
    lanes = std::min(lanes, lanes_ready);
    Fp = G > 1 ? lanes / G : lanes;
    tail_from = (tail && G == 1) ? n_passes - std::min(lanes, n_passes) : n_passes;
    long_call = n_passes >= 2 * lanes;
}

PullGrid Renderer::pull_grid(size_t slots, size_t slots_of_chip, size_t min_chunk, bool long_call) const {
    PullGrid pg;
    pg.chunk = (uint32_t)std::min<size_t>((size_t)persist_chunk, std::max<size_t>(min_chunk, slots / (slots_of_chip * 4) / 64 * 64));
    pg.grid_slots = (!wave_slots_user && long_call) ? std::max<size_t>(1, slots_of_chip / 2) : slots_of_chip;
    pg.waves = (uint32_t)std::max<size_t>(1, std::min<size_t>(cdiv(slots, pg.chunk), pg.grid_slots));
    return pg;
}

int Renderer::plan_pass(const DrawPlan &dp, const SceneView &sv, const TileGroup &TG, int B, PassPlan &pp) const {
    pp = PassPlan{};
    pp.B = B; pp.two_level = sv.num_inst > 0;
    pp.grid_tiles = std::max<uint32_t>(1u, (uint32_t)TG.tiles_local); pp.grid_shade = std::max<uint32_t>(1u, cdiv(TG.capacity, SHADE_THREADS));
    pp.wave_slots = wave_slots;
    const bool two_level = pp.two_level;
    const size_t wide_stack = (size_t)scene->wide_depth * WIDE_STACK_LEVEL_BYTES;
    if (dp.mega) {
        if (two_level || materials || sv.num_wnodes == 0) {
            set_error(std::string("megakernel = 1 renders flattened scenes with the 8-wide layout and the reference's diffuse kernel only; this renderer has ") + (two_level ? "a two-level scene (scene option instancing = 1)" : materials ? "materials = 1" : "a scene without the 8-wide layout") + ": set megakernel = 0");
            return MRT_ERR_UNSUPPORTED;
        }
        pp.stack_bytes = wide_stack;
        if (int rc = wave_slots_for(k_megakernel, wide_stack, mega_cache, cu_count)) return rc;
        pp.mega_waves = (uint32_t)std::min<size_t>(std::max<size_t>(1, cdiv(TG.capacity, 64)), (size_t)(std::max(1, mega_cache.per_cu) * cu_count));
        return MRT_OK;
    }
    pp.on_wide = wide_bounce && sv.num_wnodes > 0;
    pp.stack_bytes = wide_stack + (two_level ? WIDE_WORLD_RAY_BYTES : 0);
    if (pp.on_wide && persistent != 0) {
        if (int rc = two_level ? wave_slots_for(k_trace_mixed_wide_persist<true>, pp.stack_bytes, persist_cache, cu_count) : wave_slots_for(k_trace_mixed_wide_persist<false>, pp.stack_bytes, persist_cache, cu_count)) return rc;
        if (!wave_slots_user) pp.wave_slots = std::max(1, persist_cache.per_cu) * cu_count;
    }
    pp.chain = throughput_chain && !materials && max_bounces <= 3 && (uint64_t)scene->stats.instances * (uint64_t)std::max(1, scene->stats.max_submeshes) <= 65536ull;
    const size_t slots = 2 * (size_t)TG.capacity * B;
    pp.rpw_p = stream_rays_per_wave((size_t)TG.capacity * B); pp.rpw_m = stream_rays_per_wave(slots);
    pp.planes = shadow_planes != 0 && pp.chain && pp.on_wide && !materials && max_bounces <= PLANES_MAX_BOUNCES && !ablate_mask();
    pp.pairs = two_level && pp.planes && tl_pairs != 0 && sv.tri_packet != nullptr;
    pp.pair_cap = 2 * (size_t)capacity * (size_t)std::max(1, alloc_batch);
    pp.tl_flat = pp.pairs && sv.num_inst <= TL_FLAT_MAX_INSTANCES && tl_pairs != 2;
    pp.pair_cap_used = (uint32_t)std::min<size_t>(tl_pair_cap > 0 ? std::min<size_t>((size_t)tl_pair_cap, pp.pair_cap) : pp.pair_cap, 0xFFFFFFFFu);
    pp.prim_rope = !two_level && (!sv.num_wnodes || primary_wide == 0);
    if (pp.prim_rope && sv.num_nodes == 0 && sv.num_tris != 0) { set_error("primary_wide = 0 walks the rope layout: commit the scene with scene option rope = 1"); return MRT_ERR_STATE; }
    if (!pp.on_wide && !two_level && sv.num_nodes == 0 && sv.num_tris != 0) { set_error("wide_bounce = 0 walks the rope layout: commit the scene with scene option rope = 1"); return MRT_ERR_STATE; }
    pp.trace0_pass = pp.planes && fuse_primary != 0 && primary_wide != 1 && !(two_level && primary_wide == 0) && (fuse_primary == 2 || dp.lanes > 1 || B > 1 || two_level);
    pp.trace0_wide = pp.trace0_pass && !pp.prim_rope;
    pp.trace0_hint = primary_hint && (!two_level || (sv.num_inst <= 255u && scene->wpackets.n / WPK < ((size_t)1 << 24)));
    pp.primary = ((ablate_mask() & 1) || pp.trace0_pass) ? PrimaryForm::none
               : ((two_level && pp.on_wide) || (primary_wide == 1 && sv.num_wnodes && !two_level)) ? PrimaryForm::stream
               : (two_level || pp.prim_rope) ? PrimaryForm::rope : PrimaryForm::lane_wide;
    pp.primary_hinted = pp.trace0_hint && !(two_level && pp.primary == PrimaryForm::rope);
    pp.bundle = frame_bundle && pp.trace0_wide && B > 1;
    pp.pack_range = (uint32_t)std::min<size_t>(SHADE_PACK_RANGE, std::max<size_t>(2 * SHADE_THREADS, (size_t)TG.capacity * B / 2048 / SHADE_THREADS * SHADE_THREADS));
    pp.pull = persistent == 1 || (persistent == 2 && (slots >= (size_t)pp.wave_slots * 1024 || (std::min(dp.lanes, dp.G > 1 ? dp.Fp * dp.G : dp.n_passes) >= 5 && slots >= (size_t)pp.wave_slots * 256)));
    const bool takes_x = !two_level && pp.planes && hit_lds;
    pp.trace = pp.pairs ? TraceForm::pairs : !pp.on_wide ? TraceForm::rope : pp.pull ? (takes_x ? TraceForm::pull_x : TraceForm::pull) : (takes_x ? TraceForm::static_x : TraceForm::static_split);
    pp.trace_lds = pp.trace == TraceForm::rope ? 0 : pp.stack_bytes + (takes_x ? (size_t)HIT_LDS_WORDS * 4 : 0);
    if (pp.trace == TraceForm::pairs) pp.pg = pull_grid(slots, (size_t)pp.wave_slots, 64, dp.long_call);
    else if (pp.trace == TraceForm::pull) pp.pg = pull_grid(slots, (size_t)pp.wave_slots, 128, dp.long_call);
    else if (pp.trace == TraceForm::pull_x) {
        if (int rc = wave_slots_for(k_trace_mixed_wide_persist_x, pp.trace_lds, persist_x_cache, cu_count)) return rc;
        if (persist_x_cache.per_cu < 1) { set_error("hit_lds: the traversal kernel does not fit a compute unit with " + std::to_string(pp.trace_lds) + " bytes of LDS"); return MRT_ERR_UNSUPPORTED; }
        pp.pg = pull_grid(slots, wave_slots_user ? (size_t)pp.wave_slots : (size_t)(persist_x_cache.per_cu * cu_count), 128, dp.long_call);
    }
    else if (pp.trace != TraceForm::rope) {
        const bool shard_auto = stream_stride == 2 && stream_even == 200 && shard_world > 1 && dp.G == 1 && takes_x;
        pp.strided = stream_stride == 1 || shard_auto;
        const int even_pct = shard_auto ? 100 : stream_even;
        pp.even = even_pct > 0 ? (uint32_t)std::max<size_t>(1, std::min<size_t>(cdiv(slots, 64), (size_t)pp.wave_slots * (size_t)even_pct / 100)) : 0u;
        pp.static_grid = pp.even ? pp.even : cdiv(slots, pp.rpw_m);
    }
    return MRT_OK;
}

int Renderer::draw_nothing(int n_frames) {
    if (guides) { if (int rc = ensure_guides()) return rc; guides_valid = true; }
    MRT_HIP(hipEventRecord(ev_begin, stream));
    frame_index += (uint32_t)n_frames; frames_rendered += (uint64_t)n_frames;
    ext_used = 0;
    if (int rc = note_pass(stream)) return rc;
    MRT_HIP(hipEventRecord(ev_end, stream));
    pending_timing = true;
    return MRT_OK;
}

int Renderer::rebuild_for_batch() {
    MRT_HIP(hipStreamSynchronize(stream));
    const uint32_t keep_frame = frame_index; const int keep_cur = cur; const uint64_t keep_rendered = frames_rendered;
    DevBuf<float4> keep; MRT_HIP(keep.alloc(accum[cur].n));
    MRT_HIP(hipMemcpyAsync(keep.p, accum[cur].p, accum[cur].bytes(), hipMemcpyDeviceToDevice, stream));
    const MRTCamera keep_cam = camera;
    unsigned long long keep_totals[3] = {0, 0, 0};
    MRT_HIP(hipMemcpy(keep_totals, totals.p, sizeof keep_totals, hipMemcpyDeviceToHost));
    const bool keep_denoised = denoised_valid;
    guides_keep = true;
    int rc = resize(width, height);
    guides_keep = false; denoised_valid = keep_denoised;
    if (rc) return rc;
    MRT_HIP(hipMemcpyAsync(totals.p, keep_totals, sizeof keep_totals, hipMemcpyHostToDevice, stream));
    MRT_HIP(hipMemcpyAsync(accum[keep_cur].p, keep.p, keep.bytes(), hipMemcpyDeviceToDevice, stream));
    MRT_HIP(hipStreamSynchronize(stream));
    frame_index = keep_frame; cur = keep_cur; frames_rendered = keep_rendered; frames_completed_known = keep_rendered; camera = keep_cam;
    return MRT_OK;
}

int Renderer::ensure_lanes(int want) {
    for (; lanes_ready < want; lanes_ready++) {
        const size_t need = lane_bytes() + (lanes_ready == 0 && !halton_tab.p ? (size_t)HALTON_TAB_DIMS * HALTON_TAB_SPAN * sizeof(float) : 0);
        size_t free_b = 0, total_b = 0;
        const bool fits = hipMemGetInfo(&free_b, &total_b) != hipSuccess || free_b > need + (size_t(1) << 30);
        int rc = fits ? alloc_lane(lanes[lanes_ready]) : MRT_ERR_OUT_OF_MEMORY;
        if (rc == MRT_ERR_OUT_OF_MEMORY && lanes_ready >= 1) { (void)hipGetLastError(); release_lane(lanes[lanes_ready]); break; }
        if (rc == MRT_ERR_OUT_OF_MEMORY) { set_error("not enough device memory for one pass in flight: " + std::to_string(need >> 20) + " MiB of ray queues needed (" + std::to_string(width) + "x" + std::to_string(height) + ", frame_batch " + std::to_string(alloc_batch) + "); lower frame_batch"); return rc; }
        if (rc) return rc;
    }
    return MRT_OK;
}

void Renderer::begin_draw(DrawCtx &d) const {
    FrameParams &fp = d.fp;
    fp = FrameParams{};
    fp.width = width; fp.height = height; fp.lightCount = light_count_limit > 0 ? std::min(light_count_limit, d.sv.light_count) : d.sv.light_count;
    fp.cam_pos = make_float4(camera.position.x, camera.position.y, camera.position.z, 0);
    fp.cam_right = make_float4(camera.right.x, camera.right.y, camera.right.z, 0);
    fp.cam_up = make_float4(camera.up.x, camera.up.y, camera.up.z, 0);
    fp.cam_fwd = make_float4(camera.forward.x, camera.forward.y, camera.forward.z, 0);
    fp.shard_rank = shard_rank; fp.shard_world = shard_world;
    fp.tiles_x = (width + 7) / 8; fp.tiles_local = tiles_local; fp.max_bounces = max_bounces;
    d.gp = fp;
    d.gp.frameIndex = frame_index; d.gp.sampleIndex = frame_index + sample_offset; d.gp.npix = (uint32_t)((size_t)width * height); d.gp.capacity = capacity; d.gp.batch = 1;
    fp.npix = (uint32_t)((size_t)width * height); fp.capacity = capacity;
    d.last_acc = nullptr;
    for (hipEvent_t &e : d.last_acc_g) e = nullptr;
    d.tail.n = 0;
}

int Renderer::prepare_lane(FrameLane &L, const TileGroup &TG, const PassPlan &pp) {
    const size_t shard_qcap = (size_t)capacity * (size_t)std::max(1, alloc_batch);
    if (!pp.chain && !L.thr[0].p) {
        for (int k = 0; k < 2; k++) MRT_HIP(L.thr[k].alloc(shard_qcap));
    }
    if (pp.planes) {
        if (!L.f_lit.p) { if (int rc = alloc_planes(L)) return rc; }
        MRT_HIP(hipMemsetAsync(L.f_lit.p, 0, 4 * (size_t)TG.capacity * (size_t)pp.B, L.stream));
    }
    if (pp.pairs && !L.pairs.p) MRT_HIP(L.pairs.alloc(std::max<size_t>(PairQueue::WORDS * pp.pair_cap, 1)));
    if (!pp.planes && !L.scon.p) MRT_HIP(L.scon.alloc(shard_qcap));
    return MRT_OK;
}

int Renderer::enqueue_megakernel_pass(DrawCtx &d, FrameLane &L, const TileGroup &TG, const PassPlan &pp) {
    FrameParams &fp = d.fp;
    uint32_t *work = reinterpret_cast<uint32_t *>(L.bounce_counts.p + 64);
    for (int sub = 0; sub < pp.B; sub++) {
        fp.frameIndex = frame_index + (uint32_t)sub; fp.sampleIndex = frame_index + (uint32_t)sub + sample_offset; fp.batch = 1;
        if (d.last_acc) { MRT_HIP(hipStreamWaitEvent(L.stream, d.last_acc, 0)); d.last_acc = nullptr; }
        MRT_HIP(hipMemsetAsync(work, 0, 4, L.stream));
        launch_timed(timed(MRT_KERNEL_TRACE), k_megakernel, dim3(pp.mega_waves), dim3(64), pp.stack_bytes, L.stream, d.sv, fp, TG.seeds, accum[cur].p, accum[1 - cur].p, work, totals.p, (uint32_t)TG.owned);
        cur = 1 - cur;
    }
    MRT_HIP(hipEventRecord(L.accumulated, L.stream));
    d.last_acc = L.accumulated;
    frame_index += (uint32_t)pp.B; frames_rendered += (uint64_t)pp.B;
    return note_pass(L.stream);
}

void Renderer::enqueue_primary(DrawCtx &d, FrameLane &L, const TileGroup &TG, const PassPlan &pp) {
    if (pp.primary == PrimaryForm::none) return;
    float4 *const dirs = L.rayB[1].p;
    uint32_t *const hint_p = pp.primary_hinted ? hint.p : nullptr;
    if (pp.primary == PrimaryForm::stream) {
        const auto kernel = pp.two_level ? (pp.primary_hinted ? k_trace_primary_wide_stream<true, true> : k_trace_primary_wide_stream<true, false>)
                                         : (pp.primary_hinted ? k_trace_primary_wide_stream<false, true> : k_trace_primary_wide_stream<false, false>);
        launch_timed(timed(MRT_KERNEL_PRIMARY), kernel, dim3(cdiv(TG.capacity, pp.rpw_p), pp.B), dim3(64), pp.stack_bytes, L.stream, d.sv, d.fp, TG.seeds, L.hits.p, dirs, TG.capacity, pp.rpw_p, hint_p);
        return;
    }
    const bool lane_wide = pp.primary == PrimaryForm::lane_wide;
    auto kernel = k_trace_primary<true>;
    if (!pp.two_level) kernel = lane_wide ? k_trace_primary<false, true> : k_trace_primary<false>;
    launch_timed(timed(MRT_KERNEL_PRIMARY), kernel, dim3(pp.grid_tiles, pp.B), dim3(64), lane_wide ? pp.stack_bytes : 0, L.stream, d.sv, d.fp, TG.seeds, L.hits.p, dirs, hint_p);
}

using ShadeKernel = void (*)(SceneView, FrameParams, const uint32_t *, const float4 *, const float4 *, const float4 *, const float4 *, const unsigned long long *, uint32_t, float4 *, float4 *, float4 *, float4 *, float4 *, float4 *,
                             unsigned long long *, float4 *, float4 *, uint32_t *);
static ShadeKernel shade_kernel_for(const PassPlan &pp, bool materials, bool pack, int b) {
    if (pack) return materials ? (ShadeKernel)k_shade_pack<true, false, false, false>
                   : pp.pairs ? (ShadeKernel)k_shade_pack<false, true, true, true>
                   : pp.planes ? (ShadeKernel)k_shade_pack<false, true, true, false>
                   : pp.chain ? (ShadeKernel)k_shade_pack<false, true, false, false> : (ShadeKernel)k_shade_pack<false, false, false, false>;
    return materials ? (ShadeKernel)k_shade<true, false, false, false>
         : (pp.pairs && b > 0) ? (ShadeKernel)k_shade<false, true, true, true>
         : (pp.trace0_wide && b == 0 && pp.two_level) ? (ShadeKernel)k_shade_primary<3>
         : (pp.trace0_wide && b == 0) ? (ShadeKernel)k_shade_primary<2>
         : (pp.trace0_pass && b == 0) ? (ShadeKernel)k_shade_primary<1>
         : pp.planes ? (ShadeKernel)k_shade<false, true, true, false>
         : pp.chain ? (ShadeKernel)k_shade<false, true, false, false> : (ShadeKernel)k_shade<false, false, false, false>;
}

void Renderer::enqueue_shade(DrawCtx &d, FrameLane &L, const TileGroup &TG, const PassPlan &pp, int b) {
    FrameParams &fp = d.fp;
    const int q = b & 1, B = pp.B;
    unsigned long long *const bc = L.bounce_counts.p;
    fp.bounce = b;
    const bool pack = shade_pack && b > 0;
    fp.pack_range = pp.pack_range;
    fp.frame_bundle = (pp.bundle && b == 0) ? 1 : 0;
    if (fp.frame_bundle) {
        fp.bundle_groups = ((uint32_t)B + 7u) / 8u; fp.bundle_w = ((uint32_t)B + fp.bundle_groups - 1u) / fp.bundle_groups;
        fp.bundle_per_wave = 64u / fp.bundle_w; fp.bundle_magic = (65536u + fp.bundle_w - 1u) / fp.bundle_w;
    }
    fp.halton_tab = nullptr; fp.halton_w0 = 0; fp.halton_n = 0;
    if (fp.frame_bundle && fp.bundle_w >= 4u && halton_table && halton_tab.p) {
        fp.halton_tab = halton_tab.p; fp.halton_w0 = halton_w0; fp.halton_n = HALTON_TAB_SPAN;
    }
    const dim3 gs = b == 0 ? (fp.frame_bundle ? dim3(cdiv(cdiv((size_t)TG.capacity * fp.bundle_groups, fp.bundle_per_wave) * 64, SHADE_THREADS), 1) : dim3(pp.grid_shade, B)) : dim3(cdiv((size_t)TG.capacity * B, pack ? fp.pack_range : (uint32_t)SHADE_THREADS));
    float4 *const con_b = !pp.planes ? L.scon.p : b == 0 ? L.sample.p : L.f_con[b - 1].p;
    const size_t shade_lds = (pp.trace0_wide && b == 0) ? (size_t)SHADE_WAVES * (scene->wide_depth * WIDE_STACK_LEVEL_BYTES + (MRT_LANE_HIT_LDS ? 1024 : 0)) : 0;
    launch_timed(timed(MRT_KERNEL_SHADE), shade_kernel_for(pp, materials, pack, b), gs, dim3(SHADE_THREADS), shade_lds, L.stream, d.sv, fp, TG.seeds, L.rayA[1 - q].p, L.rayB[1 - q].p, L.thr[1 - q].p, L.hits.p,
                 b == 0 ? nullptr : bc + (b - 1), TG.capacity, L.rayA[q].p, L.rayB[q].p, L.thr[q].p, L.srayA.p, L.srayB.p, con_b, bc + b, b == 0 ? L.sample.p : nullptr, L.sample.p,
                 (b == 0 && pp.trace0_pass && pp.trace0_hint) ? hint.p : nullptr);
}

void Renderer::enqueue_trace(DrawCtx &d, FrameLane &L, const TileGroup &TG, const PassPlan &pp, int b) {
    if (ablate_mask() & 2) return;
    const int q = b & 1;
    hipStream_t st = L.stream;
    unsigned long long *const bc = L.bounce_counts.p;
    const unsigned long long *const counts = bc + b;
    uint32_t *const work = reinterpret_cast<uint32_t *>(bc + WORK_COUNTERS + (size_t)b * WORK_COUNTERS_PER_BOUNCE);
    uint8_t *const lit_b = pp.planes ? L.f_lit.p + b : nullptr;
    const float4 *const rayA = L.rayA[q].p, *const rayB = L.rayB[q].p, *const srayA = L.srayA.p, *const srayB = L.srayB.p;
    const uint32_t xcd_frames = xcd_counters ? (uint32_t)pp.B : 0u;
    switch (pp.trace) {
    case TraceForm::pairs: {
        unsigned long long *const keys = reinterpret_cast<unsigned long long *>(L.hits.p);
        uint32_t *const pc = reinterpret_cast<uint32_t *>(bc + 65 + b);
        const uint32_t stack_words = (uint32_t)(pp.stack_bytes / 4);
        if (pp.tl_flat) launch_timed(timed(MRT_KERNEL_TRACE), k_tl_top_flat, dim3((uint32_t)std::max<size_t>(1, std::min<size_t>(cdiv(2 * (size_t)TG.capacity * pp.B, 64), 2 * pp.pg.grid_slots))), dim3(64), pp.stack_bytes + 8, st, d.sv, rayA, rayB, keys, srayA, srayB,
                                     counts, lit_b, L.pairs.p, pc, pp.pair_cap_used, stack_words);
        else launch_timed(timed(MRT_KERNEL_TRACE), k_tl_top, dim3(pp.pg.waves), dim3(64), pp.stack_bytes + 8, st, d.sv, rayA, rayB, keys, srayA, srayB,
                          counts, reinterpret_cast<uint32_t *>(bc + 32 + b), pp.pg.chunk, lit_b, L.pairs.p, pc, pp.pair_cap_used, stack_words);
        launch_timed(timed(MRT_KERNEL_TRACE), k_tl_blas, dim3((uint32_t)pp.pg.grid_slots), dim3(64), (size_t)scene->wide_depth * WIDE_STACK_LEVEL_BYTES, st, d.sv, rayA, rayB, keys, srayA, srayB,
                     counts, pc + 1, 256u, lit_b, (const uint4 *)L.pairs.p, (const uint32_t *)pc, pp.pair_cap_used);
        break;
    }
    case TraceForm::pull_x:
        launch_timed(timed(MRT_KERNEL_TRACE), k_trace_mixed_wide_persist_x, dim3(pp.pg.waves), dim3(64), pp.trace_lds, st, d.sv, rayA, rayB, L.hits.p, srayA, srayB, counts, work, pp.pg.chunk, lit_b, xcd_frames);
        break;
    case TraceForm::pull:
        launch_timed(timed(MRT_KERNEL_TRACE), pp.two_level ? k_trace_mixed_wide_persist<true> : k_trace_mixed_wide_persist<false>, dim3(pp.pg.waves), dim3(64), pp.trace_lds, st, d.sv, rayA, rayB, L.hits.p, srayA, srayB, L.scon.p,
                     counts, L.sample.p, work, tag_bounce(pp.pg.chunk, b), lit_b, xcd_frames);
        break;
    case TraceForm::static_x:
        launch_timed(timed(MRT_KERNEL_TRACE), k_trace_mixed_wide_stream_x, dim3(pp.static_grid), dim3(64), pp.trace_lds, st, d.sv, rayA, rayB, L.hits.p, srayA, srayB, counts, tag_bounce(pp.rpw_m, b), lit_b, pp.even | (pp.strided ? 0x80000000u : 0u));
        break;
    case TraceForm::static_split:
        launch_timed(timed(MRT_KERNEL_TRACE), pp.two_level ? k_trace_mixed_wide_stream<true> : k_trace_mixed_wide_stream<false>, dim3(pp.static_grid), dim3(64), pp.trace_lds, st, d.sv, rayA, rayB, L.hits.p, srayA, srayB, L.scon.p,
                     counts, L.sample.p, pp.rpw_m, lit_b, pp.even);
        break;
    case TraceForm::rope:
        launch_timed(timed(MRT_KERNEL_TRACE), pp.two_level ? k_trace_mixed<true> : k_trace_mixed<false>, dim3(2 * pp.grid_tiles * (uint32_t)pp.B), dim3(64), 0, st, d.sv, rayA, rayB, L.hits.p, srayA, srayB, L.scon.p, counts, L.sample.p);
        break;
    }
}

int Renderer::enqueue_accumulate(DrawCtx &d, FrameLane &L, const TileGroup &TG, const PassPlan &pp, int pass, int g) {
    const int B = pp.B;
    hipStream_t st = L.stream;
    unsigned long long *const bc = L.bounce_counts.p;
    const uint32_t primary = (uint32_t)(TG.owned * (uint64_t)B);
    if (pp.planes && pass >= d.dp.tail_from && d.tail.n < MAX_FRAMES_IN_FLIGHT) {
        AccPass &P = d.tail.p[d.tail.n++];
        P.con0 = L.sample.p; P.con1 = L.f_con[0].p; P.con2 = L.f_con[1].p; P.lit = L.f_lit.p; P.counts = bc; P.frameIndex = d.fp.frameIndex; P.batch = B; P.primary = primary; P.pad = 0;
        MRT_HIP(hipEventRecord(L.accumulated, st));
        frame_index += (uint32_t)B; frames_rendered += (uint64_t)B;
        return MRT_OK;
    }
    const bool grouped = d.dp.G > 1;
    if (grouped) { if (d.last_acc_g[g] && d.last_acc_g[g] != L.accumulated) MRT_HIP(hipStreamWaitEvent(st, d.last_acc_g[g], 0)); }
    else if (d.last_acc) MRT_HIP(hipStreamWaitEvent(st, d.last_acc, 0));
    if (pp.planes) launch_timed(timed(MRT_KERNEL_ACCUMULATE), k_accumulate_planes, dim3(pp.grid_tiles), dim3(64), 0, st, d.fp, L.sample.p, L.f_con[0].p, L.f_con[1].p, L.f_lit.p, accum[cur].p, accum[1 - cur].p, bc, totals.p, primary);
    else launch_timed(timed(MRT_KERNEL_ACCUMULATE), k_accumulate, dim3(pp.grid_tiles), dim3(64), 0, st, d.fp, L.sample.p, accum[cur].p, accum[1 - cur].p, bc, totals.p, primary);
    MRT_HIP(hipEventRecord(L.accumulated, st));
    if (grouped) { d.last_acc_g[g] = L.accumulated; return MRT_OK; }
    d.last_acc = L.accumulated;
    cur = 1 - cur;
    frame_index += (uint32_t)B; frames_rendered += (uint64_t)B;
    return note_pass(st);
}

int Renderer::enqueue_pass(DrawCtx &d, FrameLane &L, const TileGroup &TG, const PassPlan &pp, int pass, int g) {
    FrameParams &fp = d.fp;
    fp.batch = pp.B;
    fp.frameIndex = frame_index;
    fp.sampleIndex = frame_index + sample_offset;
    fp.shard_rank = TG.rank; fp.shard_world = TG.world; fp.tiles_local = TG.tiles_local; fp.capacity = TG.capacity;
    if (d.dp.mega) return enqueue_megakernel_pass(d, L, TG, pp);
    if (int rc = prepare_lane(L, TG, pp)) return rc;
    fp.bounce = 0; fp.chain = pp.chain ? 1 : 0;
    fp.wide_stack_words = (uint32_t)((size_t)scene->wide_depth * WIDE_STACK_LEVEL_BYTES / 4);
    enqueue_primary(d, L, TG, pp);
    for (int b = 0; b < max_bounces; b++) { enqueue_shade(d, L, TG, pp, b); enqueue_trace(d, L, TG, pp, b); }
    return enqueue_accumulate(d, L, TG, pp, pass, g);
}

int Renderer::enqueue_guides(DrawCtx &d) {
    const bool two_level = d.sv.num_inst > 0;
    const size_t lds = d.sv.num_wnodes ? (size_t)scene->wide_depth * WIDE_STACK_LEVEL_BYTES : 0;
    const auto kernel = two_level ? (d.sv.num_wnodes ? k_guides<3> : k_guides<0>) : (d.sv.num_wnodes ? k_guides<2> : k_guides<1>);
    hipLaunchKernelGGL(kernel, dim3(std::max<uint32_t>(1u, (uint32_t)tiles_local)), dim3(64), lds, guide_stream, d.sv, d.gp, (const uint32_t *)seeds.p, (uint32_t)d.dp.n_frames, guide_nd.p, guide_albedo.p, guide_ids.p);
    const hipError_t le = hipGetLastError();
    (void)hipEventRecord(guide_done, guide_stream);
    (void)hipStreamWaitEvent(stream, guide_done, 0);
    if (le != hipSuccess) return hip_fail(le, "k_guides launch", __FILE__, __LINE__);
    guides_valid = true;
    return MRT_OK;
}

int Renderer::render(int n_frames) {
    if (!scene) { set_error("renderer has no scene"); return MRT_ERR_STATE; }
    DrawCtx d;
    d.sv = scene->view();
    if (d.sv.light_count < 1) { set_error("scene has no lights (lightCount must be >= 1, Raytracing.metal:273)"); return MRT_ERR_STATE; }
    if (tiles_local == 0) return draw_nothing(n_frames);
    if (alloc_batch != batch_wanted()) { if (int rc = rebuild_for_batch()) return rc; return render(n_frames); }
    DrawPlan &dp = d.dp;
    dp = plan_draw(n_frames);
    if (int rc = ensure_lanes(dp.lanes)) return rc;
    dp.settle(lanes_ready);
    lanes_used = dp.lanes; groups_used = dp.G;
    if (dp.G > 1) { if (int rc = ensure_tile_groups(dp.G)) return rc; }
    const TileGroup self_group{shard_rank, shard_world, tiles_local, capacity, owned_pixels, seeds.p};
    PassPlan plans[2][MAX_TILE_GROUPS];
    for (int k = 0; k < 2; k++)
        for (int g = 0; g < dp.G; g++) { if (int rc = plan_pass(dp, d.sv, dp.G > 1 ? tgroups[g] : self_group, dp.pass_size(k == 0 ? 0 : dp.n_passes - 1), plans[k][g])) return rc; }
    wave_slots = plans[0][0].wave_slots;
    begin_draw(d);
    ext_used = 0;
    if (halton_table && frame_bundle && !megakernel && n_frames > 1) { if (int rc = ensure_halton_table(frame_index + sample_offset, (uint32_t)n_frames)) return rc; }
    MRT_HIP(hipEventRecord(ev_begin, stream));
    MRT_HIP(hipEventRecord(ev_fork, stream));
    for (int k = 0; k < dp.lanes; k++) MRT_HIP(hipStreamWaitEvent(lanes[k].stream, ev_fork, 0));
    if (guides) {
        if (int rc = ensure_guides()) return rc;
        MRT_HIP(hipEventRecord(guide_fork, stream));
        MRT_HIP(hipStreamWaitEvent(guide_stream, guide_fork, 0));
    }
    for (int pass = 0; pass < dp.n_passes; pass++) {
        const int B = dp.pass_size(pass);
        for (int g = 0; g < dp.G; g++) {
            const TileGroup &TG = dp.G > 1 ? tgroups[g] : self_group;
            if (dp.G > 1 && TG.capacity == 0) continue;
            FrameLane &L = lanes[dp.G > 1 ? (pass % dp.Fp) * dp.G + g : pass % dp.lanes];
            if (int rc = enqueue_pass(d, L, TG, plans[B == plans[0][g].B ? 0 : 1][g], pass, g)) return rc;
        }
        if (dp.G > 1) { cur = 1 - cur; frame_index += (uint32_t)B; frames_rendered += (uint64_t)B; }
    }
    for (int k = 0; k < (dp.G > 1 ? std::min(dp.Fp, dp.n_passes) * dp.G : std::min(dp.lanes, dp.n_passes)); k++) MRT_HIP(hipStreamWaitEvent(stream, lanes[k].accumulated, 0));
    if (guides) { if (int rc = enqueue_guides(d)) return rc; }
    if (dp.G > 1) { if (int rc = note_pass(stream)) return rc; }
    if (d.tail.n > 0) {
        launch_timed(timed(MRT_KERNEL_ACCUMULATE), k_accumulate_planes_group, dim3(std::max<uint32_t>(1u, (uint32_t)tiles_local)), dim3(64), 0, stream, d.fp, d.tail, accum[cur].p, accum[1 - cur].p, totals.p);
        cur = 1 - cur;
        if (int rc = note_pass(stream)) return rc;
    }
    MRT_HIP(hipEventRecord(ev_end, stream));
    MRT_HIP(hipGetLastError());
    pending_timing = true;
    return MRT_OK;
}

#ifdef MRT_DEBUG_BOUNDS
static int check_bounds_record() {
    uint32_t v = 0;
    MRT_HIP(hipMemcpyFromSymbol(&v, HIP_SYMBOL(g_bounds_violation), 4));
    if (v) {
        static const char *kinds[] = {"?", "8-wide node", "triangle packet", "wtlas_index slot", "instance id"};
        const uint32_t zero = 0; (void)hipMemcpyToSymbol(HIP_SYMBOL(g_bounds_violation), &zero, 4);
        set_error(std::string("MRT_DEBUG_BOUNDS: the stream traversal followed an index outside its array: ") + kinds[std::min(v >> 28, 4u)] + " " + std::to_string(v & 0x0FFFFFFFu));
        return MRT_ERR_STATE;
    }
    return MRT_OK;
}
#else
static int check_bounds_record() { return MRT_OK; }
#endif

int Renderer::wait() {
    MRT_HIP(hipStreamSynchronize(stream));
    if (int rc = check_bounds_record()) return rc;
    { uint64_t done = 0; if (int rc = poll_completed(&done)) return rc; }
    if (pending_timing) {
        float ms = 0;
        MRT_HIP(hipEventElapsedTime(&ms, ev_begin, ev_end));
        ms_last = ms;
        float ext = 0; uint32_t next = 0;
        kernel_times = MRTKernelTimes{};
        for (int k = 0; k < ext_used; k++) {
            float e = 0; MRT_HIP(hipEventElapsedTime(&e, ev_ext[k].a, ev_ext[k].b));
            const int kind = ev_ext[k].kind;
            kernel_times.ms[kind] += e; kernel_times.launches[kind]++;
            if (kind == MRT_KERNEL_PRIMARY || kind == MRT_KERNEL_TRACE) { ext += e; next++; }
        }
        ms_extend_last = ext; extend_launches_last = next;
        pending_timing = false;
    }
    return MRT_OK;
}

int Renderer::read_accum(float *rgba, size_t nbytes) {
    if (nbytes != (size_t)width * height * 16) { set_error("read_accum: nbytes must be width*height*16"); return MRT_ERR_INVALID_ARGUMENT; }
    int rc = wait(); if (rc) return rc;
    MRT_HIP(hipMemcpy(rgba, accum[cur].p, nbytes, hipMemcpyDeviceToHost));
    return MRT_OK;
}
int Renderer::copy_accum_to_device(void *dptr, size_t nbytes) {
    if (nbytes != (size_t)width * height * 16) { set_error("copy_accum_to_device: nbytes must be width*height*16"); return MRT_ERR_INVALID_ARGUMENT; }
    MRT_HIP(hipMemcpyAsync(dptr, accum[cur].p, nbytes, hipMemcpyDeviceToDevice, stream));
    return MRT_OK;
}
int Renderer::write_accum_from_device(const void *dptr, size_t nbytes) {
    if (nbytes != (size_t)width * height * 16) { set_error("write_accum_from_device: nbytes must be width*height*16"); return MRT_ERR_INVALID_ARGUMENT; }
    MRT_HIP(hipMemcpyAsync(accum[cur].p, dptr, nbytes, hipMemcpyDeviceToDevice, stream));
    return MRT_OK;
}
uint32_t shard_tiles(int width, int height, int rank, int world) {
    const int tiles = ((width + 7) / 8) * ((height + 7) / 8);
    return (uint32_t)std::max(0, (tiles - rank + world - 1) / world);
}
int unpack_tiles_into(float4 *image, int width, int height, const void *compact, size_t nbytes, int rank, int world, hipStream_t st) {
    if (world < 1 || rank < 0 || rank >= world) { set_error("unpack_tiles: invalid shard"); return MRT_ERR_INVALID_ARGUMENT; }
    const uint32_t tl = shard_tiles(width, height, rank, world);
    if (nbytes != (size_t)tl * 64 * sizeof(float4)) { set_error("unpack_tiles: nbytes must be tiles x 64 x 16 for that shard (mrt_renderer_shard_tiles)"); return MRT_ERR_INVALID_ARGUMENT; }
    if (tl) hipLaunchKernelGGL(k_tiles<false>, dim3(cdiv((size_t)tl * 64, 256)), dim3(256), 0, st, image, width, height, (width + 7) / 8, rank, world, tl, (float4 *)const_cast<void *>(compact));
    MRT_HIP(hipGetLastError());
    return MRT_OK;
}
int Renderer::pack_owned_tiles(void *dptr, size_t nbytes) {
    const uint32_t tl = shard_tiles(width, height, shard_rank, shard_world);
    if (nbytes != (size_t)tl * 64 * sizeof(float4)) { set_error("pack_owned_tiles: nbytes must be tiles x 64 x 16 for this renderer's shard (mrt_renderer_shard_tiles)"); return MRT_ERR_INVALID_ARGUMENT; }
    if (tl) hipLaunchKernelGGL(k_tiles<true>, dim3(cdiv((size_t)tl * 64, 256)), dim3(256), 0, stream, accum[cur].p, width, height, (width + 7) / 8, shard_rank, shard_world, tl, (float4 *)dptr);
    MRT_HIP(hipGetLastError());
    return MRT_OK;
}
int Renderer::unpack_tiles(const void *dptr, size_t nbytes, int rank, int world) { return unpack_tiles_into(accum[cur].p, width, height, dptr, nbytes, rank, world, stream); }
int Renderer::read_tonemapped(uint8_t *rgba, size_t nbytes) {
    if (nbytes != (size_t)width * height * 4) { set_error("read_tonemapped: nbytes must be width*height*4"); return MRT_ERR_INVALID_ARGUMENT; }
    DevBuf<uchar4> tmp; MRT_HIP(tmp.alloc((size_t)width * height));
    hipLaunchKernelGGL(k_tonemap, dim3(cdiv(width, 16), cdiv(height, 16)), dim3(16, 16), 0, stream, accum[cur].p, width, height, tmp.p);
    int rc = wait(); if (rc) return rc;
    MRT_HIP(hipMemcpy(rgba, tmp.p, nbytes, hipMemcpyDeviceToHost));
    return MRT_OK;
}

int Renderer::stats(MRTRenderStats *out) {
    int rc = wait(); if (rc) return rc;
    unsigned long long t[4];
    MRT_HIP(hipMemcpy(t, totals.p, sizeof t, hipMemcpyDeviceToHost));
    memset(out, 0, sizeof *out);
    out->frames = frames_rendered; out->closest_rays = t[0]; out->shadow_rays = t[1]; out->primary_rays = t[2];
    uint64_t px = owned_pixels;
    uint64_t per_frame_px = px * 36;
    out->bytes_alg = t[0] * 96 + t[1] * 72 + frames_rendered * per_frame_px + frames_rendered * scene->stats.scene_bytes;
    out->ms_gpu_last = ms_last; out->ms_extend_last = ms_extend_last; out->extend_launches_last = extend_launches_last;
    return MRT_OK;
}
int Renderer::reset_stats() {
    MRT_HIP(hipMemsetAsync(totals.p, 0, totals.bytes(), stream));
    MRT_HIP(hipStreamSynchronize(stream));
    for (auto &pd : passes_pending) pass_events_free.push_back(pd.ev);
    passes_pending.clear(); frames_completed_known = 0;
    frames_rendered = 0;
    return MRT_OK;
}

int query_closest(const DeviceScene &sc, hipStream_t stream, const MRTRay *rays, size_t n, MRTIntersection *out) {
    if (n == 0) return MRT_OK;
    DevBuf<MRTRay> d_r; DevBuf<MRTIntersection> d_o;
    MRT_HIP(d_r.alloc(n)); MRT_HIP(d_o.alloc(n));
    MRT_HIP(hipMemcpyAsync(d_r.p, rays, n * sizeof(MRTRay), hipMemcpyHostToDevice, stream));
    if (sc.num_wnodes) hipLaunchKernelGGL(k_query_closest<true>, dim3(cdiv(n, 64)), dim3(64), (size_t)sc.wide_depth * WIDE_STACK_LEVEL_BYTES, stream, sc.view(), d_r.p, (uint32_t)n, d_o.p);
    else hipLaunchKernelGGL(k_query_closest<false>, dim3(cdiv(n, 64)), dim3(64), 0, stream, sc.view(), d_r.p, (uint32_t)n, d_o.p);
    MRT_HIP(hipMemcpyAsync(out, d_o.p, n * sizeof(MRTIntersection), hipMemcpyDeviceToHost, stream));
    MRT_HIP(hipStreamSynchronize(stream));
// ... 114 lines not shown
```

### metal-raytracing_amd/csrc/shade.h

```cpp
#pragma once
#include "device_math.h"
#include "traverse.h"
#include "traverse_wide.h"
#include "traverse_instanced.h"

namespace mrt {
namespace {

struct FrameParams {
    int32_t width, height;
    uint32_t frameIndex;
    uint32_t sampleIndex;
    int32_t lightCount;
    float4 cam_pos, cam_right, cam_up, cam_fwd;
    int32_t shard_rank, shard_world;
    int32_t tiles_x, tiles_local;
    int32_t bounce, max_bounces;
    uint32_t npix, capacity;
    int32_t batch;
    int32_t chain;
    uint32_t pack_range;
    uint32_t wide_stack_words;
    int32_t frame_bundle;
    uint32_t bundle_w, bundle_groups, bundle_per_wave, bundle_magic;
    const float *halton_tab; uint32_t halton_w0, halton_n;
};
#ifndef MRT_HALTON_INTERLEAVED
#define MRT_HALTON_INTERLEAVED 1
#endif
constexpr uint32_t HALTON_TAB_DIMS = 6, HALTON_TAB_SPAN = (1u << 20) + (1u << 16);
MRT_DEV float halton_b0(const FrameParams &fp, int idx, int d ) {
    const uint32_t j = (uint32_t)idx - fp.halton_w0;
    if (fp.halton_tab != nullptr && j < fp.halton_n) return fp.halton_tab[MRT_HALTON_INTERLEAVED ? (size_t)j * HALTON_TAB_DIMS + (uint32_t)(d - 1) : (size_t)(d - 1) * fp.halton_n + j];
    return halton_dev(idx, d);
}

MRT_DEV bool slot_to_pixel(const FrameParams &fp, uint32_t slot, int &x, int &y) {
    uint32_t lt = slot >> 6, k = slot & 63;
    if ((int)lt >= fp.tiles_local) return false;
    uint32_t tile = lt * (uint32_t)fp.shard_world + (uint32_t)fp.shard_rank;
    uint32_t ty = tile / (uint32_t)fp.tiles_x, tx = tile - ty * (uint32_t)fp.tiles_x;
    x = (int)(tx * 8 + (k & 7)); y = (int)(ty * 8 + (k >> 3));
    return x < fp.width && y < fp.height;
}

MRT_DEV void primary_ray(const FrameParams &fp, const uint32_t *__restrict__ seeds, uint32_t sample_index, int x, int y, f3 &org, f3 &dir) {
    uint32_t offset = q2load(&seeds[sample_index]);
    int idx = (int)(offset + fp.sampleIndex);
    float r0, r1;
    r0 = halton_dev(idx, 0); r1 = halton_b0(fp, idx, 1);
    float px = (float)x + r0, py = (float)y + r1;
    float uvx = px / (float)fp.width, uvy = py / (float)fp.height;
    uvx = uvx * 2.0f - 1.0f; uvy = uvy * 2.0f - 1.0f;
    dir = normalize3((uvx * mk3(fp.cam_right) + uvy * mk3(fp.cam_up)) + mk3(fp.cam_fwd));
    org = mk3(fp.cam_pos);
}

#ifndef MRT_SHADE_THREADS
#define MRT_SHADE_THREADS 256
#endif
#ifndef MRT_SHADE_WAVES
#define MRT_SHADE_WAVES 6
#endif
#ifndef MRT_SHADE_WIDE_WAVES
#define MRT_SHADE_WIDE_WAVES 5
#endif
constexpr int SHADE_THREADS = MRT_SHADE_THREADS;
constexpr int SHADE_WAVES = SHADE_THREADS / 64;
#ifndef MRT_SHADE_PACK_RANGE
#define MRT_SHADE_PACK_RANGE 4096
#endif
constexpr uint32_t SHADE_PACK_RANGE = MRT_SHADE_PACK_RANGE;

struct ShadeIO {
    const uint32_t *__restrict__ seeds;
    const float4 *__restrict__ rayA, *__restrict__ rayB, *__restrict__ thr;
    const float4 *__restrict__ hits;
    const unsigned long long *__restrict__ count_in;
    uint32_t capacity;
    float4 *__restrict__ nrayA, *__restrict__ nrayB, *__restrict__ nthr;
    float4 *__restrict__ srayA, *__restrict__ srayB, *__restrict__ scon;
    unsigned long long *__restrict__ count_out;
    float4 *__restrict__ sample_primary;
    float4 *__restrict__ sample;
    uint32_t *__restrict__ hint;
};
#define SHADE_IO_PARAMS const uint32_t *__restrict__ seeds, const float4 *__restrict__ rayA, const float4 *__restrict__ rayB, const float4 *__restrict__ thr, \
                        const float4 *__restrict__ hits, const unsigned long long *__restrict__ count_in, uint32_t capacity,                               \
                        float4 *__restrict__ nrayA, float4 *__restrict__ nrayB, float4 *__restrict__ nthr,                                                    \
                        float4 *__restrict__ srayA, float4 *__restrict__ srayB, float4 *__restrict__ scon, unsigned long long *__restrict__ count_out,       \
                        float4 *__restrict__ sample_primary, float4 *__restrict__ sample, uint32_t *__restrict__ hint
#define SHADE_IO_GATHER ShadeIO{seeds, rayA, rayB, thr, hits, count_in, capacity, nrayA, nrayB, nthr, srayA, srayB, scon, count_out, sample_primary, sample, hint}
struct ShadeShared { uint32_t w_next[SHADE_WAVES], w_shadow[SHADE_WAVES], w_spec[SHADE_WAVES]; unsigned long long blk_base; };

MRT_DEV float4 pairs_hit(const SceneView &s, const ShadeIO &io, const uint32_t i, const unsigned long long key) {
    if (key == ~0ull) return make_float4(-1.0f, 0.0f, 0.0f, __uint_as_float(0xFFFFFFFFu));
    const uint32_t g = (uint32_t)key;
    const InstanceDev &I = s.inst[instance_of_gid(s, g)];
    const uint32_t pk = s.tri_packet[I.ts_base + (g - I.gid_base)];
    const float4 Aw = qload(&io.rayA[i]), Bw = qload(&io.rayB[i]);
    const float4 *__restrict__ q = s.wpackets + WPK * (size_t)pk;
    float t_, U, V, ad;
    (void)tri_test(q[0], q[1], q[2], to_object_point(I, mk3(Aw)), to_object_dir(I, mk3(Bw)), 0.0f, __builtin_inff(), t_, U, V, ad);
    return make_float4(__uint_as_float((uint32_t)(key >> 32)), U / ad, V / ad, __uint_as_float(g));
}

template <bool MATERIALS, bool CHAIN, bool PLANES, bool B0TAB>
MRT_DEV void shade_entry(const SceneView &s, const FrameParams &fp, const ShadeIO &io, ShadeShared &sh, const uint32_t i, const float4 H, bool active, const float4 Bprim) {
    uint32_t gid = __float_as_uint(H.w);
    active = active && gid != 0xFFFFFFFFu;
    bool want_shadow = false, want_next = false;
    f3 P = mk3(0, 0, 0), nrm = mk3(0, 1, 0), ldir = mk3(0, 1, 0), lcol = mk3(0, 0, 0), color = mk3(0, 0, 0), ndir = mk3(0, 1, 0), norg = mk3(0, 0, 0);
    float ldist = 0.0f; uint32_t pix = 0;
    bool special = false;
    uint32_t chain_in = 0, chain_out = 0;
    if (active) {
        float4 A, B, C;
        if (io.sample_primary) {
            A = make_float4(fp.cam_pos.x, fp.cam_pos.y, fp.cam_pos.z, __builtin_inff());
            B = B0TAB ? Bprim : qload(&io.rayB[i]);
            C = make_float4(1.0f, 1.0f, 1.0f, 0.0f);
        } else if (CHAIN) {
            A = qload(&io.rayA[i]); B = qload(&io.rayB[i]);
            const uint32_t ch = __float_as_uint(A.w);
            chain_in = ch;
            C = s.base_color[ch & 0xFFFFu];
            if (fp.bounce >= 2) { const float4 s1 = s.base_color[ch >> 16]; C = make_float4(C.x * s1.x, C.y * s1.y, C.z * s1.z, 0.0f); }
            A.w = __builtin_inff();
        } else { A = qload(&io.rayA[i]); B = qload(&io.rayB[i]); C = qload(&io.thr[i]); }
        pix = __float_as_uint(B.w);
        uint32_t inst, geom, rec = gid, vb = 0;
        if (s.num_inst) {
            inst = instance_of_gid(s, gid);
            const InstanceDev &I = s.inst[inst];
            rec = I.ts_base + (gid - I.gid_base); vb = I.vbase;
        } else inst = 0;
        float bu = H.y, bv = H.z;
        P = mk3(A) + mk3(B) * H.x;
        float bw = 1.0f - bu - bv;
        const uint4 ts = s.tri_shade[rec];
        if (!s.num_inst) inst = ts.w >> 16;
        geom = ts.w & 0xFFFFu;
        const f3 n_obj = (bu * mk3(s.normals[vb + ts.y]) + bv * mk3(s.normals[vb + ts.z])) + bw * mk3(s.normals[vb + ts.x]);
        f3 c0 = mk3(s.inst_cols[inst * 4 + 0]), c1 = mk3(s.inst_cols[inst * 4 + 1]), c2 = mk3(s.inst_cols[inst * 4 + 2]);
        f3 n_w = mk3((c0.x * n_obj.x + c1.x * n_obj.y) + c2.x * n_obj.z,
                     (c0.y * n_obj.x + c1.y * n_obj.y) + c2.y * n_obj.z,
                     (c0.z * n_obj.x + c1.z * n_obj.y) + c2.z * n_obj.z);
        nrm = normalize3(n_w);
        const uint32_t rslot = inst * (uint32_t)s.max_sub + geom;
        f3 surf = mk3(s.base_color[rslot]);
        if (CHAIN) chain_out = fp.bounce == 0 ? rslot : (chain_in & 0xFFFFu) | (rslot << 16);
// ... 26 lines not shown
                float F = 1.0f, cost = 0.0f;
                if (sin2t < 1.0f) { cost = __builtin_sqrtf(1.0f - sin2t); const float c = entering ? cosi : cost; const float x = 1.0f - c; const float x2 = x * x; F = r0 + (1.0f - r0) * ((x2 * x2) * x); }
                f3 nd;
                if (u2 < F) { nd = dir + nn * (2.0f * cosi); norg = P + nn * 1e-3f; }
                else { nd = dir * eta + nn * (eta * cosi - cost); norg = P + nn * -1e-3f; }
                ndir = normalize3(nd);
                diffuse = false; special = true;
                want_next = fp.bounce + 1 < fp.max_bounces;
            } else {
                const float ud = trn > 0.0f ? (ul - trn) / (1.0f - trn) : ul;
                const float ps = (ks > 0.0f && ns > 0.0f) ? ks / (ks + kd) : 0.0f;
                if (ud < ps) {
                    const float hx = halton_dev(idx, dim0 + 3), hy = halton_dev(idx, dim0 + 4);
                    const float a2 = 2.0f / (ns + 2.0f);
                    const float ct2 = (1.0f - hy) / (1.0f + (a2 - 1.0f) * hy);
                    const float ct = __builtin_sqrtf(ct2), st = __builtin_sqrtf(1.0f - ct2);
                    float sp_, cp_; sincos_2pi_dev(hx, sp_, cp_);
                    const f3 hw = align_hemisphere_dev(mk3(st * cp_, ct, st * sp_), nrm);
                    const f3 dir = mk3(B);
                    const float dh = dot3(dir, hw);
                    const f3 wi = dir - hw * (2.0f * dh);
                    diffuse = false; special = true;
                    if (dot3(wi, nrm) > 0.0f) {
                        color = color * (spec * (1.0f / ps));
                        ndir = normalize3(wi);
                        want_next = fp.bounce + 1 < fp.max_bounces;
                    }
                } else if (ps > 0.0f) surf = surf * (1.0f / (1.0f - ps));
            }
        }
        if (diffuse) {
            float ls = B0TAB ? halton_b0(fp, idx, 2) : halton_dev(idx, dim0 + 0);
            int li = min((int)(ls * (float)fp.lightCount), fp.lightCount - 1);
            const LightDev L = s.lights[li];
            int ltype = __float_as_int(L.position.w);
            if (ltype == MRTLightTypeAreaLight) {
                float ax = (B0TAB ? halton_b0(fp, idx, 3) : halton_dev(idx, dim0 + 1)) * 2.0f - 1.0f;
                float ay = (B0TAB ? halton_b0(fp, idx, 4) : halton_dev(idx, dim0 + 2)) * 2.0f - 1.0f;
                f3 sp = (mk3(L.position) + mk3(L.right) * ax) + mk3(L.up) * ay;
                ldir = sp - P;
                ldist = length3(ldir);
                float inv = 1.0f / (ldist > 1e-3f ? ldist : 1e-3f);
                ldir = ldir * inv;
                lcol = mk3(L.color) * (inv * inv);
                lcol = lcol * saturatef(dot3(neg3(ldir), mk3(L.forward)));
            } else if (ltype == MRTLightTypeSpotlight) {
                ldir = mk3(L.position) - P;
                ldist = length3(ldir);
                float inv = 1.0f / (ldist > 1e-3f ? ldist : 1e-3f);
                ldir = ldir * inv;
                lcol = mk3(0, 0, 0);
                float spot = dot3(neg3(ldir), mk3(L.dirn));
                if (spot > L.dirn.w) lcol = (mk3(L.color) * inv) * inv;
            } else if (ltype == MRTLightTypePointlight) {
                ldir = mk3(L.position) - P;
                ldist = length3(ldir);
                float inv = 1.0f / (ldist > 1e-3f ? ldist : 1e-3f);
                ldir = ldir * inv;
                lcol = (mk3(L.color) * inv) * inv;
            } else {
                ldir = neg3(mk3(L.dirn));
                ldist = __builtin_inff();
                lcol = mk3(L.color);
            }
            lcol = lcol * saturatef(dot3(nrm, ldir));
            lcol = lcol * (float)fp.lightCount;
            color = mk3(C) * surf;
            want_shadow = length3(lcol) > 0.0001f;
            want_next = fp.bounce + 1 < fp.max_bounces;
            if (want_next) {
                float hx = B0TAB ? halton_b0(fp, idx, 5) : halton_dev(idx, dim0 + 3), hy = B0TAB ? halton_b0(fp, idx, 6) : halton_dev(idx, dim0 + 4);
                ndir = align_hemisphere_dev(sample_cosine_hemisphere_dev(hx, hy), nrm);
            }
        }
    }
    const uint32_t lane = threadIdx.x & 63, wv = threadIdx.x >> 6;
    const unsigned long long m_sh = __ballot(want_shadow), m_nx = __ballot(want_next && !(MATERIALS && special)), m_sp = MATERIALS ? __ballot(want_next && special) : 0ull;
    if (lane == 0) { sh.w_shadow[wv] = (uint32_t)__popcll(m_sh); sh.w_next[wv] = (uint32_t)__popcll(m_nx); if (MATERIALS) sh.w_spec[wv] = (uint32_t)__popcll(m_sp); }
    __syncthreads();
    if (threadIdx.x == 0) {
        uint32_t tn = 0, ts = 0, tp = 0;
        for (int k = 0; k < SHADE_WAVES; k++) { uint32_t a = sh.w_next[k], b = sh.w_shadow[k]; sh.w_next[k] = tn; sh.w_shadow[k] = ts; tn += a; ts += b; }
        if (MATERIALS) for (int k = 0; k < SHADE_WAVES; k++) { uint32_t a = sh.w_spec[k]; sh.w_spec[k] = tn + tp; tp += a; }
        sh.blk_base = (tn | ts | tp) ? atomicAdd(io.count_out, ((unsigned long long)ts << 32) | (tn + tp)) : 0ull;
    }
    __syncthreads();
    const unsigned long long base = sh.blk_base;
    const unsigned long long lt = (1ull << lane) - 1ull;
    uint32_t ss = 0, ns = 0;
    if (want_shadow) {
        ss = (uint32_t)(base >> 32) + sh.w_shadow[wv] + (uint32_t)__popcll(m_sh & lt);
        f3 so = P + nrm * 1e-3f;
        f3 con = lcol * color;
        qstore(&io.srayA[ss], make_float4(so.x, so.y, so.z, ldist - 1e-3f));
        qstore(&io.srayB[ss], make_float4(ldir.x, ldir.y, ldir.z, __uint_as_float(pix)));
        if (PLANES) q2store(&io.scon[pix], make_float4(con.x, con.y, con.z, 0.0f)); else qstore(&io.scon[ss], make_float4(con.x, con.y, con.z, 0.0f));
    }
    if (want_next) {
        const bool sp = MATERIALS && special;
        ns = (uint32_t)base + (sp ? sh.w_spec[wv] + (uint32_t)__popcll(m_sp & lt) : sh.w_next[wv] + (uint32_t)__popcll(m_nx & lt));
        qstore(&io.nrayA[ns], make_float4(norg.x, norg.y, norg.z, CHAIN ? __uint_as_float(chain_out) : __builtin_inff()));
        qstore(&io.nrayB[ns], make_float4(ndir.x, ndir.y, ndir.z, __uint_as_float(pix)));
        if (!CHAIN) qstore(&io.nthr[ns], make_float4(color.x, color.y, color.z, 0.0f));
    }
}

MRT_DEV bool bounce0_slot(const FrameParams &fp, uint32_t &slot, uint32_t &sub) {
    sub = blockIdx.y; slot = blockIdx.x * SHADE_THREADS + threadIdx.x;
    if (!fp.frame_bundle) return true;
    const uint32_t lane = threadIdx.x & 63u, wave = slot >> 6;
    const uint32_t bi = (lane * fp.bundle_magic) >> 16, q = wave * fp.bundle_per_wave + bi;
    slot = q / fp.bundle_groups; sub = (q - slot * fp.bundle_groups) * fp.bundle_w + (lane - bi * fp.bundle_w);
    return bi < fp.bundle_per_wave && sub < (uint32_t)fp.batch;
}

template <int WALK>
__global__ void __launch_bounds__(SHADE_THREADS, WALK >= 2 ? MRT_SHADE_WIDE_WAVES : MRT_SHADE_WAVES) k_shade_primary(SceneView s, FrameParams fp, SHADE_IO_PARAMS) {
    const ShadeIO io = SHADE_IO_GATHER;
    __shared__ ShadeShared sh;
    extern __shared__ uint32_t shade_stk[];
    uint32_t slot, sub;
    const bool in_batch = bounce0_slot(fp, slot, sub);
    const uint32_t spix = sub * io.capacity + slot;
    int px_x = 0, px_y = 0;
    const bool active = slot < io.capacity && in_batch && slot_to_pixel(fp, slot, px_x, px_y);
    float4 H = make_float4(-1.0f, 0.0f, 0.0f, __uint_as_float(0xFFFFFFFFu)), Bprim = make_float4(0.0f, 0.0f, 1.0f, 0.0f);
    if (active) {
        f3 org, dir;
        primary_ray(fp, io.seeds, spix, px_x, px_y, org, dir);
        Bprim = make_float4(dir.x, dir.y, dir.z, __uint_as_float(spix));
        const uint32_t pixel = (uint32_t)px_y * (uint32_t)fp.width + (uint32_t)px_x;
        uint32_t *const stk = shade_stk + (threadIdx.x >> 6) * fp.wide_stack_words;
        TravHit h;
        bool hit;
        if (WALK == 3) {
            if (io.hint != nullptr) {
                const uint32_t guess = io.hint[pixel];
                float t0 = __builtin_inff(); uint32_t seed = 0xFFFFFFFFu;
                const uint32_t gpk = guess & 0xFFFFFFu, gin = guess >> 24;
                if (guess != 0xFFFFFFFFu && gin < s.num_inst) {
                    const InstanceDev &I = s.inst[gin];
                    if (gpk - I.packet_base < I.ntri) {
                        const float4 *__restrict__ pk = s.wpackets + WPK * (size_t)gpk;
                        float t, U, V, ad;
                        if (tri_test(pk[0], pk[1], pk[2], to_object_point(I, org), to_object_dir(I, dir), 0.0f, __builtin_inff(), t, U, V, ad)) { t0 = t; seed = guess; }
                    }
                }
                hit = traverse_wide_lane_two_level<true>(s, org, dir, t0, seed, h, stk);
                if (hit && h.pk != guess) io.hint[pixel] = h.pk;
            }
            else hit = traverse_wide_lane_two_level<false>(s, org, dir, __builtin_inff(), 0xFFFFFFFFu, h, stk);
        }
        else if (WALK == 2) {
            if (io.hint != nullptr) {
                const uint32_t guess = io.hint[pixel];
                float t0 = __builtin_inff(); uint32_t seed = 0xFFFFFFFFu;
                TravHit sh_; sh_.U = 0.0f; sh_.V = 0.0f; sh_.ad = 1.0f; sh_.gid = 0xFFFFFFFFu;
                if (guess < s.num_wpackets) {
                    const float4 *__restrict__ pk = s.wpackets + WPK * (size_t)guess;
                    const float4 q0_ = pk[0];
                    float t, U, V, ad;
                    if (tri_test(q0_, pk[1], pk[2], org, dir, 0.0f, __builtin_inff(), t, U, V, ad)) { t0 = t; seed = guess; sh_.U = U; sh_.V = V; sh_.ad = ad; sh_.gid = __float_as_uint(q0_.w); }
                }
#if MRT_LANE_HIT_LDS
                hit = traverse_wide_lane<true>(s, org, dir, t0, seed, h, stk, reinterpret_cast<float *>(shade_stk + SHADE_WAVES * fp.wide_stack_words + (threadIdx.x >> 6) * 256u), &sh_);
#else
                hit = traverse_wide_lane<true>(s, org, dir, t0, seed, h, stk);
#endif
                if (h.pk != guess) io.hint[pixel] = h.pk;
            }
            else hit = traverse_wide_lane<false>(s, org, dir, __builtin_inff(), 0xFFFFFFFFu, h, stk);
        }
        else if (io.hint != nullptr) {
            const uint32_t guess = io.hint[pixel];
            h.t = __builtin_inff(); h.U = 0.0f; h.V = 0.0f; h.ad = 1.0f; h.gid = 0xFFFFFFFFu; h.pk = 0xFFFFFFFFu;
            if (guess < s.num_tris) {
                const float4 *__restrict__ pk = s.packets + 3 * (size_t)guess;
                const float4 q0 = pk[0];
                float t, U, V, ad;
                if (tri_test(q0, pk[1], pk[2], org, dir, 0.0f, __builtin_inff(), t, U, V, ad)) { h.t = t; h.U = U; h.V = V; h.ad = ad; h.gid = __float_as_uint(q0.w); h.pk = guess; }
            }
            hit = traverse<false, false, false, true>(s, org, dir, 0.0f, h.t, h);
            if (h.pk != guess) io.hint[pixel] = h.pk;
        }
        else hit = traverse<false>(s, org, dir, 0.0f, __builtin_inff(), h);
        if (hit) H = make_float4(h.t, h.U / h.ad, h.V / h.ad, __uint_as_float(h.gid));
    }
    shade_entry<false, true, true, true>(s, fp, io, sh, spix, H, active, Bprim);
}

template <bool MATERIALS, bool CHAIN, bool PLANES, bool PAIRS>
__global__ void __launch_bounds__(SHADE_THREADS, MRT_SHADE_WAVES) k_shade_pack(SceneView s, FrameParams fp, SHADE_IO_PARAMS) {
    const ShadeIO io = SHADE_IO_GATHER;
    __shared__ ShadeShared sh;
    __shared__ uint32_t p_idx[2 * SHADE_THREADS], p_w[SHADE_WAVES];
    __shared__ float4 p_hit[2 * SHADE_THREADS];
    const uint32_t n = io.count_in ? (uint32_t)*io.count_in : io.capacity;
    const float4 miss = make_float4(-1.0f, 0.0f, 0.0f, __uint_as_float(0xFFFFFFFFu)), noB = make_float4(0.0f, 0.0f, 1.0f, 0.0f);
    const uint32_t begin = blockIdx.x * fp.pack_range, end = min(n, begin + fp.pack_range);
    const uint32_t lane_ = threadIdx.x & 63, wv_ = threadIdx.x >> 6;
    uint32_t head = 0, tail = 0, cur = begin;
    for (;;) {
        const uint32_t pending = tail - head;
        if (pending < (uint32_t)SHADE_THREADS && cur < end) {
            const uint32_t e = cur + threadIdx.x;
            float4 He = miss;
            if (PAIRS) {
                const unsigned long long key = e < end ? __builtin_nontemporal_load(reinterpret_cast<const unsigned long long *>(io.hits) + e) : ~0ull;
                He = make_float4(__uint_as_float((uint32_t)key), __uint_as_float((uint32_t)(key >> 32)), 0.0f, __uint_as_float(key != ~0ull ? 0u : 0xFFFFFFFFu));
            }
            else if (e < end) He = qload(&io.hits[e]);
            const bool a = __float_as_uint(He.w) != 0xFFFFFFFFu;
            const unsigned long long m = __ballot(a);
            if (lane_ == 0) p_w[wv_] = (uint32_t)__popcll(m);
            __syncthreads();
            uint32_t off = 0, tot = 0;
            for (int k = 0; k < SHADE_WAVES; k++) { const uint32_t c = p_w[k]; if ((uint32_t)k < wv_) off += c; tot += c; }
            if (a) { const uint32_t pos = (tail + off + (uint32_t)__popcll(m & ((1ull << lane_) - 1ull))) & (2u * SHADE_THREADS - 1u); p_idx[pos] = e; p_hit[pos] = He; }
            __syncthreads();
            tail += tot; cur += SHADE_THREADS;
            continue;
        }
        if (pending == 0u) break;
        const uint32_t take = min(pending, (uint32_t)SHADE_THREADS);
        const bool act = threadIdx.x < take;
        const uint32_t pos = (head + threadIdx.x) & (2u * SHADE_THREADS - 1u);
        const uint32_t ie = act ? p_idx[pos] : 0u;
        float4 He = act ? p_hit[pos] : miss;
        if (PAIRS && act) He = pairs_hit(s, io, ie, (unsigned long long)__float_as_uint(He.x) | ((unsigned long long)__float_as_uint(He.y) << 32));
        head += take;
        shade_entry<MATERIALS, CHAIN, PLANES, false>(s, fp, io, sh, ie, He, act, noB);
    }
}

template <bool MATERIALS, bool CHAIN, bool PLANES, bool PAIRS>
__global__ void __launch_bounds__(SHADE_THREADS, MRT_SHADE_WAVES) k_shade(SceneView s, FrameParams fp, SHADE_IO_PARAMS) {
    const ShadeIO io = SHADE_IO_GATHER;
    __shared__ ShadeShared sh;
    const uint32_t sub = io.sample_primary ? blockIdx.y : 0u, slot = blockIdx.x * SHADE_THREADS + threadIdx.x;
    const uint32_t i = sub * io.capacity + slot;
    const uint32_t n = io.count_in ? (uint32_t)*io.count_in : io.capacity;
    bool active = slot < n;
    if (io.sample_primary) {
        int px_x, px_y;
        active = active && slot_to_pixel(fp, slot, px_x, px_y);
        if (active && !PLANES) q2store(&io.sample_primary[i], make_float4(0.0f, 0.0f, 0.0f, 0.0f));
    }
    float4 H = make_float4(-1.0f, 0.0f, 0.0f, __uint_as_float(0xFFFFFFFFu));
    if (active && PAIRS) H = pairs_hit(s, io, i, __builtin_nontemporal_load(reinterpret_cast<const unsigned long long *>(io.hits) + i));
    else if (active) H = qload(&io.hits[i]);
    shade_entry<MATERIALS, CHAIN, PLANES, false>(s, fp, io, sh, i, H, active, make_float4(0.0f, 0.0f, 1.0f, 0.0f));
}

}
}
```

### metal-raytracing_amd/csrc/traverse_wide.h

```cpp
#pragma once
#include "traverse.h"
#include "traverse_instanced.h"

namespace mrt {
namespace {

#ifndef MRT_WIDE_SCALED
#define MRT_WIDE_SCALED 1
#endif
#ifndef MRT_WIDE_SPEC
#define MRT_WIDE_SPEC 1
#endif
#ifndef MRT_WIDE_SPEC_TWO_LEVEL
#define MRT_WIDE_SPEC_TWO_LEVEL 0
#endif
#ifndef MRT_COOP_MODE
#define MRT_COOP_MODE 3
#endif
#ifdef MRT_DEBUG_BOUNDS
__device__ uint32_t g_bounds_violation = 0;
#define MRT_BOUND(idx, limit, kind) do { if ((idx) >= (limit)) { atomicMax(&g_bounds_violation, ((uint32_t)(kind) << 28) | min((uint32_t)(idx), 0x0FFFFFFFu)); (idx) = 0; } } while (0)
#else
#define MRT_BOUND(idx, limit, kind) do { } while (0)
#endif
// ... 311 lines not shown
                if (better) { best_t = t; best_pk = tri_pk; insts = (insts & 0xFFFFu) | (insts << 16); }
            }
        }
        if (want_node) {
            uint32_t node_hits, tri_hits;
            wide_node_test<MRT_WIDE_SCALED != 0>(n0, n1, n2, n3, n4, o, rb.ix, rb.iy, rb.iz, rb.nx, rb.ny, rb.nz, rb.oct, 0.0f, best_t, node_hits, tri_hits);
            enter_node<true>(stack, lane, g_base, g_mask, n0, n1, node_hits);
            t_base = __float_as_uint(n1.y); t_mask = tri_hits;
        }
    }
    h.t = best_t; h.U = 0.0f; h.V = 0.0f; h.ad = 1.0f; h.gid = 0xFFFFFFFFu; h.pk = 0xFFFFFFFFu;
    if (best_pk == 0xFFFFFFFFu) return false;
    retest_winner<true>(s, best_pk, insts >> 16, wo, wd, h);
    h.pk = best_pk | ((insts >> 16) << 24);
    return true;
}

#ifndef MRT_WIDE_REFILL_AT
#define MRT_WIDE_REFILL_AT 16
#endif
#ifndef MRT_TWO_LEVEL_WAVES
#define MRT_TWO_LEVEL_WAVES 6
#endif
#ifndef MRT_WIDE_STREAM_WAVES
#define MRT_WIDE_STREAM_WAVES (MRT_WIDE_SPEC ? 6 : 7)
#endif
constexpr int WIDE_REFILL_AT = MRT_WIDE_REFILL_AT;

struct StreamStats {
    uint32_t iters, live_sum, node_sum, tri_sum, refills, refill_lanes;
#ifdef MRT_STATS_PROBE
    uint32_t level_end[3] = {0, 0, 0};
    uint32_t probe[3] = {0, 0, 0};
#endif
#ifdef MRT_WAVE_TIMES
    uint32_t drain_iters = 0, drain_live = 0, maxdt = 0, drain_le8 = 0; unsigned long long prev = 0ull, drain_t0 = 0ull;
    uint32_t dr_hist[2][6] = {{0, 0, 0, 0, 0, 0}, {0, 0, 0, 0, 0, 0}}, dr_kids[2] = {0, 0}, dr_n[2] = {0, 0}, dr_tris[2] = {0, 0};
#endif
};

struct OneRange {
    uint32_t b, e; bool used = false;
    MRT_DEV bool operator()(uint32_t &ob, uint32_t &oe) { if (used) return false; used = true; ob = b; oe = e; return b < e; }
};
struct BatchStride {
    uint32_t next, step, limit;
    MRT_DEV bool operator()(uint32_t &ob, uint32_t &oe) { if (next >= limit) return false; ob = next; oe = min(limit, next + 64u); next += step; return true; }
};
struct SharedCounter {
    uint32_t *counter; uint32_t n, chunk;
    MRT_DEV bool operator()(uint32_t &ob, uint32_t &oe) {
        uint32_t base = 0;
        if ((threadIdx.x & 63) == 0) base = atomicAdd(counter, chunk);
        base = (uint32_t)__builtin_amdgcn_readfirstlane((int)base);
        if (base >= n) return false;
        ob = base; oe = min(n, base + chunk);
        return true;
    }
};

constexpr uint32_t XCD_COUNTER_STRIDE = 32;
struct XcdRegions {
    uint32_t *counters; uint32_t n_next, n, chunk, subframes; uint32_t home; uint32_t tries = 0;
    MRT_DEV bool operator()(uint32_t &ob, uint32_t &oe) {
        const uint32_t regions = subframes ? 8u : 1u;
        const uint32_t C1 = subframes ? (n_next + chunk - 1u) / chunk : (n + chunk - 1u) / chunk, C2 = subframes ? (n - n_next + chunk - 1u) / chunk : 0u;
        const uint32_t B = subframes ? subframes : 1u;
        const uint32_t F1 = (C1 + B - 1u) / B, S1 = (F1 + regions - 1u) / regions, F2 = (C2 + B - 1u) / B, S2 = (F2 + regions - 1u) / regions;
        const uint32_t K1 = B * S1, K = K1 + B * S2;
        while (tries < regions) {
            const uint32_t x = (home + tries) & (regions - 1u);
            uint32_t k = 0;
            if ((threadIdx.x & 63) == 0) k = atomicAdd(&counters[x * XCD_COUNTER_STRIDE], 1u);
            k = (uint32_t)__builtin_amdgcn_readfirstlane((int)k);
            if (k >= K) { tries++; continue; }
            const bool p2 = k >= K1;
            const uint32_t kk = p2 ? k - K1 : k, S = p2 ? S2 : S1, F = p2 ? F2 : F1, Cp = p2 ? C2 : C1;
            const uint32_t f = kk / S, lc = x * S + (kk - f * S);
            if (lc >= F) continue;
            const uint32_t c = f * F + lc;
            if (c >= Cp) continue;
            const uint32_t first = subframes && p2 ? n_next : 0u, lim = subframes && !p2 ? n_next : n;
            ob = first + c * chunk; oe = min(lim, ob + chunk);
            return true;
        }
        return false;
    }
};

struct NoPairs { static constexpr bool on = false; };
struct PairQueue {
    static constexpr bool on = true;
    static constexpr uint32_t WORDS = 1u;
    static constexpr uint32_t BLOCK = 256;
    uint4 *__restrict__ pairs; uint32_t *__restrict__ count; uint32_t cap;
    uint32_t *cursor;
    MRT_DEV bool push(uint32_t ray_index, uint32_t inst, float tmax, uint32_t tagw) const {
        const unsigned long long m = __ballot(1);
        const int leader = __ffsll((long long)m) - 1;
        const uint32_t lane = threadIdx.x & 63, n = (uint32_t)__popcll(m), rank = (uint32_t)__popcll(m & ((1ull << lane) - 1ull));
        uint32_t cur = 0, fits = 0, fresh = 0xFFFFFFFFu;
        if ((int)lane == leader) {
            cur = cursor[0]; const uint32_t end = cursor[1];
            fits = min(n, end - cur);
            if (fits < n) {
                const uint32_t base = atomicAdd(count, BLOCK);
                if (base < cap && cap - base >= BLOCK) { fresh = base; cursor[0] = base + (n - fits); cursor[1] = base + BLOCK; }
                else { cursor[0] = end; }
            } else cursor[0] = cur + n;
        }
        cur = (uint32_t)__builtin_amdgcn_readlane((int)cur, leader); fits = (uint32_t)__builtin_amdgcn_readlane((int)fits, leader); fresh = (uint32_t)__builtin_amdgcn_readlane((int)fresh, leader);
        uint32_t slot;
        if (rank < fits) slot = cur + rank;
        else if (fresh != 0xFFFFFFFFu) slot = fresh + (rank - fits);
        else return false;
        qstore(reinterpret_cast<float4 *>(&pairs[slot]), make_float4(__uint_as_float(ray_index), __uint_as_float(inst), tmax, __uint_as_float(tagw)));
        return true;
    }
    MRT_DEV void close() const {
        const uint32_t lane = threadIdx.x & 63, cur = cursor[0], end = cursor[1];
        for (uint32_t k = cur + lane; k < end; k += 64) qstore(reinterpret_cast<float4 *>(pairs) + k, make_float4(__uint_as_float(0xFFFFFFFFu), 0.0f, 0.0f, 0.0f));
        cursor[0] = end;
    }
};

struct NoExt { static constexpr bool hit_lds = false, root_pre = false; float *hit = nullptr; uint32_t *root = nullptr; };
template <bool HIT> struct StreamExt {
    static constexpr bool hit_lds = HIT, root_pre = HIT && MRT_ROOT_AT_FETCH != 0;
    float *hit;
    uint32_t *root = nullptr;
};
constexpr uint32_t HIT_LDS_WORDS = 256u + (MRT_ROOT_AT_FETCH ? 128u : 0u);

#ifdef MRT_WAVE_TIMES
MRT_DEV void hook_wave_times(StreamStats *ss, bool TWO_LEVEL, bool draining, bool live, uint32_t g_mask, uint32_t t_mask, uint32_t u_mask, const uint32_t *stack, uint32_t lane) {
    if (!ss) return;
    if (draining) {
        const uint32_t nl_ = (uint32_t)__popcll(__ballot(live)); ss->drain_iters++; ss->drain_live += nl_; if (nl_ <= 8u) ss->drain_le8++;
        if (!TWO_LEVEL && nl_ <= 16u) {
            const uint32_t sp_ = live ? g_mask >> 16 : 0u;
            uint32_t kids_ = live ? (uint32_t)__popc((g_mask >> 8) & 0xFFu) : 0u;
            for (uint32_t l_ = 0; l_ < sp_; l_++) kids_ += (uint32_t)__popc(stack[l_ * (WIDE_STACK_LEVEL_BYTES / 4u) + lane] & 0xFFu);
            uint32_t tris_ = live ? (uint32_t)__popc(t_mask) + (uint32_t)__popc(u_mask) : 0u;
            for (int o_ = 32; o_ > 0; o_ >>= 1) { kids_ += (uint32_t)__shfl_xor((int)kids_, o_); tris_ += (uint32_t)__shfl_xor((int)tris_, o_); }
            for (int c_ = 0; c_ < 2; c_++) if (c_ == 0 || nl_ <= 4u) {
                for (uint32_t d_ = 0; d_ < 6u; d_++) ss->dr_hist[c_][d_] += (uint32_t)__popcll(__ballot(live && (d_ < 5u ? sp_ == d_ : sp_ >= 5u)));
                ss->dr_kids[c_] += kids_; ss->dr_tris[c_] += tris_; ss->dr_n[c_] += nl_;
            }
        }
    }
    const unsigned long long now_ = wall_clock64(); const uint32_t dt_ = (uint32_t)(now_ - ss->prev);
    if (ss->prev != 0ull && dt_ > ss->maxdt) ss->maxdt = dt_;
    ss->prev = now_; if (draining && ss->drain_t0 == 0ull) ss->drain_t0 = now_;
}
#else
#define hook_wave_times(...) ((void)0)
#endif
#ifdef MRT_STATS_PROBE
MRT_DEV void hook_stats_probe(StreamStats *ss, bool has_tri, bool want_node, uint32_t node, uint32_t pend) {
    if (!ss) return;
#if MRT_STATS_PROBE == 1
    for (int k = 0; k < 3; k++) ss->probe[k] += (uint32_t)__popcll(__ballot(want_node && node < ss->level_end[k]));
#elif MRT_STATS_PROBE == 2
    uint32_t tot = pend;
    for (int o_ = 32; o_ > 0; o_ >>= 1) tot += (uint32_t)__shfl_xor((int)tot, o_);
    ss->probe[0] += tot; ss->probe[1] += (uint32_t)__popcll(__ballot(pend >= 2u)); ss->probe[2] += __popcll(__ballot(has_tri)) < 16 ? 1u : 0u;
// ... 254 lines not shown
```

Baseline: 14360.

## Split shade output queues into eight per-XCD segments with separate tail counters

Shade blocks now append next-bounce and shadow rays into one of eight queue segments chosen by block index, each with its own tail counter, instead of a single global atomic counter. The persistent traversal kernel gets a SegRegions work distributor that pulls chunks per segment, and shadow rays are flagged with a high bit. The aim is to cut contention on the single global atomic and keep producer and consumer work local to an XCD. The cost is extra queue padding, counter folding at accumulate time, and some imbalance or empty chunks at segment boundaries. The path is on by default when its pull_x, chain, shade_pack and bounce conditions are met.

```diff
diff --git a/include/mrt_debug.h b/include/mrt_debug.h
--- a/include/mrt_debug.h
+++ b/include/mrt_debug.h
@@ -27,6 +27,7 @@
 int mrt_debug_host_sah(const float *lo4, const float *hi4, uint32_t n, uint32_t *order, uint32_t *left, uint32_t *right, uint32_t *parent);
 int mrt_debug_tlas_host_build(const float *lo4, const float *hi4, uint32_t n, uint32_t *rope_order, uint32_t *rope_links, uint32_t *wide_order, uint32_t *wide_pos, uint32_t *counts68);
 int mrt_debug_layout_limits(uint64_t triangles, uint64_t nodes);
+int mrt_debug_segment_sizing(uint32_t capacity, int32_t batch, uint64_t *out4);
 int mrt_debug_calibrate(MRTContext ctx, size_t table_bytes, double *out5);
 
 #ifdef __cplusplus
diff --git a/metal-raytracing_amd/_ffi.py b/metal-raytracing_amd/_ffi.py
--- a/metal-raytracing_amd/_ffi.py
+++ b/metal-raytracing_amd/_ffi.py
@@ -234,6 +234,7 @@
     "mrt_debug_read_wnodes": (C.c_int, [_P, _P, _SZ, C.POINTER(C.c_uint64)]),
     "mrt_debug_read_layout": (C.c_int, [_P, _I32, _P, _SZ, C.POINTER(C.c_uint64)]),
     "mrt_debug_layout_limits": (C.c_int, [C.c_uint64, C.c_uint64]),
+    "mrt_debug_segment_sizing": (C.c_int, [C.c_uint32, C.c_int32, C.POINTER(C.c_uint64)]),
     "mrt_debug_host_sah": (C.c_int, [_P, _P, _U32, _P, _P, _P, _P]),
     "mrt_debug_tlas_host_build": (C.c_int, [_P, _P, _U32, _P, _P, _P, _P, _P]),
     "mrt_debug_validate": (C.c_int, [_P]),
diff --git a/metal-raytracing_amd/csrc/api.cpp b/metal-raytracing_amd/csrc/api.cpp
--- a/metal-raytracing_amd/csrc/api.cpp
+++ b/metal-raytracing_amd/csrc/api.cpp
@@ -756,6 +756,7 @@
     std::string k(key);
     if (k == "persistent") { REQUIRE(value == 0 || value == 1 || value == 2, "persistent must be 0 (never), 1 (always) or 2 (by launch size)"); r->r.persistent = (int)value; }
     else if (k == "xcd_counters") { REQUIRE(value == 0 || value == 1, "xcd_counters must be 0 or 1"); r->r.xcd_counters = (int)value; }
+    else if (k == "queue_segments") { REQUIRE(value == 1 || value == 8, "queue_segments must be 1 or 8"); r->r.queue_segments = r->r.segments_used = (int)value; }
     else if (k == "tile_groups") { REQUIRE(value >= 0 && value <= mrt::MAX_TILE_GROUPS && value == (int)value, "tile_groups must be 0 (by the draw), 1 (never) or 2..4"); r->r.tile_groups = (int)value; }
     else if (k == "shade_pack") { REQUIRE(value == 0 || value == 1, "shade_pack must be 0 or 1"); r->r.shade_pack = (int)value; }
     else if (k == "hit_lds") { REQUIRE(value == 0 || value == 1, "hit_lds must be 0 or 1"); r->r.hit_lds = (int)value; }
@@ -790,6 +791,7 @@
     else if (k == "tile_groups") *value = r->r.tile_groups;
     else if (k == "groups_used") *value = r->r.groups_used;
     else if (k == "xcd_counters") *value = r->r.xcd_counters;
+    else if (k == "queue_segments") *value = r->r.segments_used;
     else if (k == "wave_slots") *value = r->r.wave_slots;
     else if (k == "stream_stride") *value = r->r.stream_stride;
     else if (k == "halton_table") *value = r->r.halton_table;
@@ -1077,6 +1079,14 @@
     return mrt::layout_limits(triangles, nodes);
     MRT_CATCH
 }
+int mrt_debug_segment_sizing(uint32_t capacity, int32_t batch, uint64_t *out4) {
+    MRT_TRY
+    if (!out4 || batch < 1 || batch > mrt::MAX_FRAME_BATCH) { mrt::set_error("mrt_debug_segment_sizing: NULL output or batch outside 1 .. MAX_FRAME_BATCH"); return MRT_ERR_INVALID_ARGUMENT; }
+    const mrt::SegmentSizing z = mrt::segment_sizing(capacity, batch);
+    out4[0] = z.blocks; out4[1] = z.per_block; out4[2] = z.seg_cap; out4[3] = mrt::queue_entries(capacity, batch);
+    return MRT_OK;
+    MRT_CATCH
+}
 int mrt_debug_calibrate(MRTContext ctx, size_t table_bytes, double *out3) {
     MRT_TRY
     REQUIRE(ctx && out3 && table_bytes >= 4096 && table_bytes <= ((size_t)1 << 34), "mrt_debug_calibrate: bad argument");
diff --git a/metal-raytracing_amd/csrc/renderer.h b/metal-raytracing_amd/csrc/renderer.h
--- a/metal-raytracing_amd/csrc/renderer.h
+++ b/metal-raytracing_amd/csrc/renderer.h
@@ -58,10 +58,17 @@
     PullGrid pg;
     uint32_t even = 0, static_grid = 0;
     uint32_t mega_waves = 0;
-};
+    int segs = 1; uint32_t seg_cap = 0;
+};
+struct SegmentSizing { uint32_t bundle_groups = 1, bundle_w = 1, bundle_per_wave = 64, per_block = 0; uint64_t blocks = 0, seg_cap = 0; };
+SegmentSizing segment_sizing(uint32_t capacity, int B);
+size_t queue_entries(uint32_t capacity, int alloc_batch);
 struct SlotCache { size_t lds_bytes = ~(size_t)0; int per_cu = 0; };
 struct DrawCtx;
 
+#ifndef MRT_QUEUE_SEGMENTS_DEFAULT
+#define MRT_QUEUE_SEGMENTS_DEFAULT 8
+#endif
 struct Renderer {
     hipStream_t stream = nullptr;
     const DeviceScene *scene = nullptr;
@@ -103,12 +110,14 @@
     int primary_wide = 2;
     int persistent = 2;
     int xcd_counters = 1;
+    int queue_segments = MRT_QUEUE_SEGMENTS_DEFAULT;
+    int segments_used = MRT_QUEUE_SEGMENTS_DEFAULT;
     int hit_lds = 1;
     int shade_pack = 1;
     int persist_chunk = 256;
     int wave_slots = 7168;
     bool wave_slots_user = false;
-    mutable SlotCache mega_cache, persist_cache, persist_x_cache;
+    mutable SlotCache mega_cache, persist_cache, persist_x_cache, persist_xs_cache;
     mutable int cu_count = 0;
     int alloc_planes(FrameLane &L);
     bool tail_accumulate = true;
diff --git a/metal-raytracing_amd/csrc/renderer.hip b/metal-raytracing_amd/csrc/renderer.hip
--- a/metal-raytracing_amd/csrc/renderer.hip
+++ b/metal-raytracing_amd/csrc/renderer.hip
@@ -187,15 +187,17 @@
     else traverse_wide_stream<false>(s, XcdRegions{work, n_next, n, chunk, subframes, blockIdx.x & 7u}, stk_dyn, fetch, emit, wss);
 }
 
+template <bool SEG>
 __global__ void __launch_bounds__(64, MRT_WIDE_STREAM_WAVES) k_trace_mixed_wide_persist_x(SceneView s, const float4 *__restrict__ rayA, const float4 *__restrict__ rayB, float4 *__restrict__ hits,
                                                                 const float4 *__restrict__ srayA, const float4 *__restrict__ srayB, const unsigned long long *__restrict__ counts,
                                                                 uint32_t *__restrict__ work, uint32_t chunk, uint8_t *__restrict__ lit, uint32_t subframes) {
     extern __shared__ uint32_t lds_dyn[];
-    const unsigned long long c = *counts;
+    unsigned long long c = *counts;
+    if (SEG) for (uint32_t x = 1; x < QUEUE_SEGMENTS; x++) c += counts[(size_t)x * SEG_TAIL_STRIDE];
     const uint32_t n_next = (uint32_t)c, n_shadow = (uint32_t)(c >> 32), n = n_next + n_shadow;
-    if (blockIdx.x * chunk >= n) return;
+    if ((unsigned long long)blockIdx.x * chunk >= (unsigned long long)n + (SEG ? 2ull * QUEUE_SEGMENTS * chunk : 0ull)) return;
     auto fetch = [&](uint32_t i, float4 &A, float4 &B, uint32_t &tag, uint32_t &is_any) {
-            const bool sh = i >= n_next; tag = sh ? i - n_next : i; is_any = sh ? 1u : 0u;
+            const bool sh = SEG ? (i & SEG_SHADOW_BIT) != 0u : i >= n_next; tag = SEG ? i & ~SEG_SHADOW_BIT : sh ? i - n_next : i; is_any = sh ? 1u : 0u;
             A = qload(sh ? &srayA[tag] : &rayA[tag]); B = qload(sh ? &srayB[tag] : &rayB[tag]);
             if (!sh) A.w = __builtin_inff();
             else tag = __float_as_uint(B.w);
@@ -205,7 +207,8 @@
             else qstore(&hits[j], hit ? make_float4(h.t, h.U / h.ad, h.V / h.ad, __uint_as_float(h.gid)) : make_float4(-1.0f, 0.0f, 0.0f, __uint_as_float(0xFFFFFFFFu)));
         };
     StreamExt<true> ext{reinterpret_cast<float *>(lds_dyn), lds_dyn + 256u};
-    traverse_wide_stream<false, false, false, NoPairs, StreamExt<true>>(s, XcdRegions{work, n_next, n, chunk, subframes, blockIdx.x & 7u}, lds_dyn + HIT_LDS_WORDS, fetch, emit, nullptr, NoPairs{}, ext);
+    if constexpr (SEG) traverse_wide_stream<false, false, false, NoPairs, StreamExt<true>>(s, SegRegions{work, counts, subframes, chunk, blockIdx.x & 7u}, lds_dyn + HIT_LDS_WORDS, fetch, emit, nullptr, NoPairs{}, ext);
+    else traverse_wide_stream<false, false, false, NoPairs, StreamExt<true>>(s, XcdRegions{work, n_next, n, chunk, subframes, blockIdx.x & 7u}, lds_dyn + HIT_LDS_WORDS, fetch, emit, nullptr, NoPairs{}, ext);
 }
 
 __global__ void __launch_bounds__(64, MRT_WIDE_STREAM_WAVES) k_trace_mixed_wide_stream_x(SceneView s, const float4 *__restrict__ rayA, const float4 *__restrict__ rayB, float4 *__restrict__ hits,
@@ -303,18 +306,30 @@
 }
 
 constexpr size_t WORK_COUNTERS = 128, WORK_COUNTERS_PER_BOUNCE = 8 * XCD_COUNTER_STRIDE / 2;
+constexpr size_t SEG_TAILS = WORK_COUNTERS + 32 * WORK_COUNTERS_PER_BOUNCE, SEG_TAILS_PER_BOUNCE = QUEUE_SEGMENTS * SEG_TAIL_STRIDE;
+MRT_DEV unsigned long long fold_bounce_counters(unsigned long long *__restrict__ bounce_counts, int b) {
+    unsigned long long c = bounce_counts[b];
+    unsigned long long *const tails = bounce_counts + SEG_TAILS + (size_t)b * SEG_TAILS_PER_BOUNCE;
+    for (uint32_t x = 0; x < QUEUE_SEGMENTS; x++) { c += tails[x * SEG_TAIL_STRIDE]; tails[x * SEG_TAIL_STRIDE] = 0; }
+    bounce_counts[b] = 0;
+    bounce_counts[32 + b] = 0;
+    for (int x = 0; x < 8; x++) reinterpret_cast<uint32_t *>(bounce_counts + WORK_COUNTERS + (size_t)b * WORK_COUNTERS_PER_BOUNCE)[x * XCD_COUNTER_STRIDE] = 0;
+    bounce_counts[65 + b] = 0;
+    return c;
+}
+#ifdef MRT_PROBE_SHADE_TAILS
+constexpr size_t PROBE_TAIL_WORDS = 32 * 8 * 16;
+#else
+constexpr size_t PROBE_TAIL_WORDS = 0;
+#endif
 __global__ void __launch_bounds__(64) k_accumulate(FrameParams fp, const float4 *__restrict__ sample, const float4 *__restrict__ prev, float4 *__restrict__ dst,
                                                    unsigned long long *__restrict__ bounce_counts, unsigned long long *__restrict__ totals, uint32_t primary) {
     if (blockIdx.x == 0 && threadIdx.x == 0) {
         unsigned long long closest = primary, shadow = 0;
         for (int b = 0; b < fp.max_bounces; b++) {
-            unsigned long long c = bounce_counts[b];
+            const unsigned long long c = fold_bounce_counters(bounce_counts, b);
             if (b + 1 < fp.max_bounces) closest += (uint32_t)c;
             shadow += c >> 32;
-            bounce_counts[b] = 0;
-            bounce_counts[32 + b] = 0;
-            for (int x = 0; x < 8; x++) reinterpret_cast<uint32_t *>(bounce_counts + WORK_COUNTERS + (size_t)b * WORK_COUNTERS_PER_BOUNCE)[x * XCD_COUNTER_STRIDE] = 0;
-            bounce_counts[65 + b] = 0;
         }
         atomicAdd(&totals[0], closest); atomicAdd(&totals[1], shadow); atomicAdd(&totals[2], (unsigned long long)primary);
     }
@@ -349,13 +364,9 @@
     if (blockIdx.x == 0 && threadIdx.x == 0) {
         unsigned long long closest = primary, shadow = 0;
         for (int b = 0; b < fp.max_bounces; b++) {
-            unsigned long long c = bounce_counts[b];
+            const unsigned long long c = fold_bounce_counters(bounce_counts, b);
             if (b + 1 < fp.max_bounces) closest += (uint32_t)c;
             shadow += c >> 32;
-            bounce_counts[b] = 0;
-            bounce_counts[32 + b] = 0;
-            for (int x = 0; x < 8; x++) reinterpret_cast<uint32_t *>(bounce_counts + WORK_COUNTERS + (size_t)b * WORK_COUNTERS_PER_BOUNCE)[x * XCD_COUNTER_STRIDE] = 0;
-            bounce_counts[65 + b] = 0;
         }
         atomicAdd(&totals[0], closest); atomicAdd(&totals[1], shadow); atomicAdd(&totals[2], (unsigned long long)primary);
     }
@@ -386,11 +397,9 @@
             if (p >= g.n) break;
             closest += g.p[p].primary; primary += g.p[p].primary;
             for (int b = 0; b < fp.max_bounces; b++) {
-                const unsigned long long c = g.p[p].counts[b];
+                const unsigned long long c = fold_bounce_counters(g.p[p].counts, b);
                 if (b + 1 < fp.max_bounces) closest += (uint32_t)c;
                 shadow += c >> 32;
-                g.p[p].counts[b] = 0; g.p[p].counts[32 + b] = 0; g.p[p].counts[65 + b] = 0;
-                for (int x = 0; x < 8; x++) reinterpret_cast<uint32_t *>(g.p[p].counts + WORK_COUNTERS + (size_t)b * WORK_COUNTERS_PER_BOUNCE)[x * XCD_COUNTER_STRIDE] = 0;
             }
         }
         totals[0] += closest; totals[1] += shadow; totals[2] += primary;
@@ -646,7 +655,7 @@
     for (auto &L : lanes) {
         MRT_HIP(hipStreamCreateWithFlags(&L.stream, hipStreamNonBlocking));
         MRT_HIP(hipEventCreateWithFlags(&L.accumulated, hipEventDisableTiming));
-        MRT_HIP(L.bounce_counts.alloc(WORK_COUNTERS + 32 * WORK_COUNTERS_PER_BOUNCE));
+        MRT_HIP(L.bounce_counts.alloc(SEG_TAILS + 32 * SEG_TAILS_PER_BOUNCE + PROBE_TAIL_WORDS));
         MRT_HIP(hipMemsetAsync(L.bounce_counts.p, 0, L.bounce_counts.bytes(), stream));
     }
     MRT_HIP(totals.alloc(4));
@@ -753,8 +762,25 @@
 
 constexpr int PLANES_MAX_BOUNCES = 3;
 
+SegmentSizing segment_sizing(uint32_t capacity, int B) {
+    SegmentSizing z;
+    z.bundle_groups = ((uint32_t)B + 7u) / 8u; z.bundle_w = ((uint32_t)B + z.bundle_groups - 1u) / z.bundle_groups; z.bundle_per_wave = 64u / z.bundle_w;
+    const uint64_t waves = cdiv((uint64_t)capacity * z.bundle_groups, (uint64_t)z.bundle_per_wave);
+    z.blocks = cdiv(waves * 64u, (uint64_t)SHADE_THREADS);
+    z.per_block = (uint32_t)SHADE_WAVES * z.bundle_per_wave * z.bundle_w;
+    z.seg_cap = cdiv(z.blocks, (uint64_t)QUEUE_SEGMENTS) * z.per_block;
+    return z;
+}
+size_t queue_entries(uint32_t capacity, int alloc_batch) {
+    size_t qcap = (size_t)capacity * (size_t)std::max(1, alloc_batch);
+    qcap += (size_t)QUEUE_SEGMENTS * SHADE_THREADS;
+#ifdef MRT_PROBE_SHADE_TAILS
+    qcap += 8 * (size_t)SHADE_PACK_RANGE;
+#endif
+    return qcap;
+}
 size_t Renderer::lane_bytes() const {
-    const size_t qcap = (size_t)capacity * (size_t)std::max(1, alloc_batch);
+    const size_t qcap = queue_entries(capacity, alloc_batch);
     const bool need_thr = !(throughput_chain && !materials && max_bounces <= 3);
     const size_t spix = (size_t)std::max<uint32_t>(capacity, 1u) * (size_t)std::max(1, alloc_batch);
     const size_t planes_bytes = shadow_planes ? 2 * spix * sizeof(float4) + spix * 4 : 0;
@@ -773,7 +799,7 @@
     return MRT_OK;
 }
 int Renderer::alloc_lane(FrameLane &L) {
-    const size_t qcap = (size_t)capacity * (size_t)std::max(1, alloc_batch);
+    const size_t qcap = queue_entries(capacity, alloc_batch);
     const bool need_thr = !(throughput_chain && !materials && max_bounces <= 3);
     for (int k = 0; k < 2; k++) { MRT_HIP(L.rayA[k].alloc(qcap)); MRT_HIP(L.rayB[k].alloc(qcap)); if (need_thr) MRT_HIP(L.thr[k].alloc(qcap)); }
     MRT_HIP(L.hits.alloc(qcap)); MRT_HIP(L.srayA.alloc(qcap)); MRT_HIP(L.srayB.alloc(qcap));
@@ -903,6 +929,13 @@
 static inline int ablate_mask() { static const int mask = getenv("MRT_ABLATE") ? atoi(getenv("MRT_ABLATE")) : 0; return mask; }
 #else
 static constexpr int ablate_mask() { return 0; }
+#endif
+#ifdef MRT_PROBE_SHADE_TAILS
+static inline int probe_disjoint() { static const int v = getenv("MRT_PROBE_DISJOINT") ? atoi(getenv("MRT_PROBE_DISJOINT")) : 0; return v; }
+__global__ void k_probe_tails_init(unsigned long long *__restrict__ words, uint32_t seg_cap) {
+    if (threadIdx.x < 8u) { const unsigned long long v = (unsigned long long)seg_cap * threadIdx.x; words[threadIdx.x * 16u] = v | (v << 32); }
+}
+static inline int probe_tails_mask() { static const int mask = getenv("MRT_PROBE_TAILS") ? atoi(getenv("MRT_PROBE_TAILS")) : 0; return mask; }
 #endif
 static inline uint32_t tag_bounce(uint32_t arg, int b) {
 #ifdef MRT_WAVE_TIMES
@@ -1009,12 +1042,22 @@
     const bool takes_x = !two_level && pp.planes && hit_lds;
     pp.trace = pp.pairs ? TraceForm::pairs : !pp.on_wide ? TraceForm::rope : pp.pull ? (takes_x ? TraceForm::pull_x : TraceForm::pull) : (takes_x ? TraceForm::static_x : TraceForm::static_split);
     pp.trace_lds = pp.trace == TraceForm::rope ? 0 : pp.stack_bytes + (takes_x ? (size_t)HIT_LDS_WORDS * 4 : 0);
+    pp.segs = 1; pp.seg_cap = 0;
+    if (queue_segments == (int)QUEUE_SEGMENTS && pp.trace == TraceForm::pull_x && pp.trace0_wide && !two_level && pp.bundle && shade_pack && pp.chain && xcd_counters && max_bounces <= 3) {
+        const SegmentSizing z = segment_sizing(TG.capacity, B);
+        const uint64_t all = (uint64_t)QUEUE_SEGMENTS * z.seg_cap;
+        if (all <= (uint64_t)queue_entries(capacity, alloc_batch) && all < (uint64_t)SEG_SHADOW_BIT) { pp.segs = (int)QUEUE_SEGMENTS; pp.seg_cap = (uint32_t)z.seg_cap; }
+    }
+#ifdef MRT_PROBE_SHADE_TAILS
+    if (probe_tails_mask()) { pp.segs = 1; pp.seg_cap = 0; }
+#endif
     if (pp.trace == TraceForm::pairs) pp.pg = pull_grid(slots, (size_t)pp.wave_slots, 64, dp.long_call);
     else if (pp.trace == TraceForm::pull) pp.pg = pull_grid(slots, (size_t)pp.wave_slots, 128, dp.long_call);
     else if (pp.trace == TraceForm::pull_x) {
-        if (int rc = wave_slots_for(k_trace_mixed_wide_persist_x, pp.trace_lds, persist_x_cache, cu_count)) return rc;
-        if (persist_x_cache.per_cu < 1) { set_error("hit_lds: the traversal kernel does not fit a compute unit with " + std::to_string(pp.trace_lds) + " bytes of LDS"); return MRT_ERR_UNSUPPORTED; }
-        pp.pg = pull_grid(slots, wave_slots_user ? (size_t)pp.wave_slots : (size_t)(persist_x_cache.per_cu * cu_count), 128, dp.long_call);
+        SlotCache &xc = pp.segs > 1 ? persist_xs_cache : persist_x_cache;
+        if (int rc = pp.segs > 1 ? wave_slots_for(k_trace_mixed_wide_persist_x<true>, pp.trace_lds, xc, cu_count) : wave_slots_for(k_trace_mixed_wide_persist_x<false>, pp.trace_lds, xc, cu_count)) return rc;
+        if (xc.per_cu < 1) { set_error("hit_lds: the traversal kernel does not fit a compute unit with " + std::to_string(pp.trace_lds) + " bytes of LDS"); return MRT_ERR_UNSUPPORTED; }
+        pp.pg = pull_grid(slots, wave_slots_user ? (size_t)pp.wave_slots : (size_t)(xc.per_cu * cu_count), 128, dp.long_call);
     }
     else if (pp.trace != TraceForm::rope) {
         const bool shard_auto = stream_stride == 2 && stream_even == 200 && shard_world > 1 && dp.G == 1 && takes_x;
@@ -1157,6 +1200,8 @@
     fp.bounce = b;
     const bool pack = shade_pack && b > 0;
     fp.pack_range = pp.pack_range;
+    const bool seg = pp.segs > 1;
+    fp.segs = (uint32_t)pp.segs; fp.seg_cap = pp.seg_cap;
     fp.frame_bundle = (pp.bundle && b == 0) ? 1 : 0;
     if (fp.frame_bundle) {
         fp.bundle_groups = ((uint32_t)B + 7u) / 8u; fp.bundle_w = ((uint32_t)B + fp.bundle_groups - 1u) / fp.bundle_groups;
@@ -1166,11 +1211,21 @@
     if (fp.frame_bundle && fp.bundle_w >= 4u && halton_table && halton_tab.p) {
         fp.halton_tab = halton_tab.p; fp.halton_w0 = halton_w0; fp.halton_n = HALTON_TAB_SPAN;
     }
-    const dim3 gs = b == 0 ? (fp.frame_bundle ? dim3(cdiv(cdiv((size_t)TG.capacity * fp.bundle_groups, fp.bundle_per_wave) * 64, SHADE_THREADS), 1) : dim3(pp.grid_shade, B)) : dim3(cdiv((size_t)TG.capacity * B, pack ? fp.pack_range : (uint32_t)SHADE_THREADS));
+    const dim3 gs = b == 0 ? (fp.frame_bundle ? dim3(cdiv(cdiv((size_t)TG.capacity * fp.bundle_groups, fp.bundle_per_wave) * 64, SHADE_THREADS), 1) : dim3(pp.grid_shade, B)) : (seg && pack) ? dim3(QUEUE_SEGMENTS * cdiv(pp.seg_cap, fp.pack_range)) : dim3(cdiv((size_t)TG.capacity * B, pack ? fp.pack_range : (uint32_t)SHADE_THREADS));
     float4 *const con_b = !pp.planes ? L.scon.p : b == 0 ? L.sample.p : L.f_con[b - 1].p;
     const size_t shade_lds = (pp.trace0_wide && b == 0) ? (size_t)SHADE_WAVES * (scene->wide_depth * WIDE_STACK_LEVEL_BYTES + (MRT_LANE_HIT_LDS ? 1024 : 0)) : 0;
+    unsigned long long *count_out = seg ? bc + SEG_TAILS + (size_t)b * SEG_TAILS_PER_BOUNCE : bc + b;
+    const unsigned long long *const count_in = b == 0 ? nullptr : seg ? bc + SEG_TAILS + (size_t)(b - 1) * SEG_TAILS_PER_BOUNCE : bc + (b - 1);
+#ifdef MRT_PROBE_SHADE_TAILS
+    fp.probe_tails = (probe_tails_mask() >> b) & 1;
+    if (fp.probe_tails) {
+        count_out = bc + SEG_TAILS + 32 * SEG_TAILS_PER_BOUNCE + (size_t)b * 8 * 16;
+        const uint32_t per_block = pack ? fp.pack_range : (uint32_t)SHADE_THREADS, seg_cap = (probe_disjoint() && pp.planes && pp.chain && gs.y == 1u) ? cdiv(gs.x, 8u) * per_block : 0u;
+        hipLaunchKernelGGL(k_probe_tails_init, dim3(1), dim3(64), 0, L.stream, count_out, seg_cap);
+    }
+#endif
     launch_timed(timed(MRT_KERNEL_SHADE), shade_kernel_for(pp, materials, pack, b), gs, dim3(SHADE_THREADS), shade_lds, L.stream, d.sv, fp, TG.seeds, L.rayA[1 - q].p, L.rayB[1 - q].p, L.thr[1 - q].p, L.hits.p,
-                 b == 0 ? nullptr : bc + (b - 1), TG.capacity, L.rayA[q].p, L.rayB[q].p, L.thr[q].p, L.srayA.p, L.srayB.p, con_b, bc + b, b == 0 ? L.sample.p : nullptr, L.sample.p,
+                 count_in, TG.capacity, L.rayA[q].p, L.rayB[q].p, L.thr[q].p, L.srayA.p, L.srayB.p, con_b, count_out, b == 0 ? L.sample.p : nullptr, L.sample.p,
                  (b == 0 && pp.trace0_pass && pp.trace0_hint) ? hint.p : nullptr);
 }
 
@@ -1198,7 +1253,9 @@
         break;
     }
     case TraceForm::pull_x:
-        launch_timed(timed(MRT_KERNEL_TRACE), k_trace_mixed_wide_persist_x, dim3(pp.pg.waves), dim3(64), pp.trace_lds, st, d.sv, rayA, rayB, L.hits.p, srayA, srayB, counts, work, pp.pg.chunk, lit_b, xcd_frames);
+        if (pp.segs > 1) launch_timed(timed(MRT_KERNEL_TRACE), k_trace_mixed_wide_persist_x<true>, dim3(pp.pg.waves), dim3(64), pp.trace_lds, st, d.sv, rayA, rayB, L.hits.p, srayA, srayB,
+                                      (const unsigned long long *)(bc + SEG_TAILS + (size_t)b * SEG_TAILS_PER_BOUNCE), work, pp.pg.chunk, lit_b, pp.seg_cap);
+        else launch_timed(timed(MRT_KERNEL_TRACE), k_trace_mixed_wide_persist_x<false>, dim3(pp.pg.waves), dim3(64), pp.trace_lds, st, d.sv, rayA, rayB, L.hits.p, srayA, srayB, counts, work, pp.pg.chunk, lit_b, xcd_frames);
         break;
     case TraceForm::pull:
         launch_timed(timed(MRT_KERNEL_TRACE), pp.two_level ? k_trace_mixed_wide_persist<true> : k_trace_mixed_wide_persist<false>, dim3(pp.pg.waves), dim3(64), pp.trace_lds, st, d.sv, rayA, rayB, L.hits.p, srayA, srayB, L.scon.p,
@@ -1288,6 +1345,7 @@
     for (int k = 0; k < 2; k++)
         for (int g = 0; g < dp.G; g++) { if (int rc = plan_pass(dp, d.sv, dp.G > 1 ? tgroups[g] : self_group, dp.pass_size(k == 0 ? 0 : dp.n_passes - 1), plans[k][g])) return rc; }
     wave_slots = plans[0][0].wave_slots;
+    segments_used = plans[0][0].segs;
     begin_draw(d);
     ext_used = 0;
     if (halton_table && frame_bundle && !megakernel && n_frames > 1) { if (int rc = ensure_halton_table(frame_index + sample_offset, (uint32_t)n_frames)) return rc; }
@@ -1353,6 +1411,9 @@
             float e = 0; MRT_HIP(hipEventElapsedTime(&e, ev_ext[k].a, ev_ext[k].b));
             const int kind = ev_ext[k].kind;
             kernel_times.ms[kind] += e; kernel_times.launches[kind]++;
+#ifdef MRT_PROBE_SHADE_TAILS
+            if (getenv("MRT_PROBE_LOG")) fprintf(stderr, "probe_launch %d kind %d ms %.5f\n", k, kind, e);
+#endif
             if (kind == MRT_KERNEL_PRIMARY || kind == MRT_KERNEL_TRACE) { ext += e; next++; }
         }
         ms_extend_last = ext; extend_launches_last = next;
diff --git a/metal-raytracing_amd/csrc/shade.h b/metal-raytracing_amd/csrc/shade.h
--- a/metal-raytracing_amd/csrc/shade.h
+++ b/metal-raytracing_amd/csrc/shade.h
@@ -24,6 +24,10 @@
     int32_t frame_bundle;
     uint32_t bundle_w, bundle_groups, bundle_per_wave, bundle_magic;
     const float *halton_tab; uint32_t halton_w0, halton_n;
+    uint32_t segs, seg_cap;
+#ifdef MRT_PROBE_SHADE_TAILS
+    uint32_t probe_tails;
+#endif
 };
 #ifndef MRT_HALTON_INTERLEAVED
 #define MRT_HALTON_INTERLEAVED 1
@@ -67,6 +71,8 @@
 #endif
 constexpr int SHADE_THREADS = MRT_SHADE_THREADS;
 constexpr int SHADE_WAVES = SHADE_THREADS / 64;
+constexpr uint32_t QUEUE_SEGMENTS = 8;
+constexpr uint32_t SEG_TAIL_STRIDE = 16;
 #ifndef MRT_SHADE_PACK_RANGE
 #define MRT_SHADE_PACK_RANGE 4096
 #endif
@@ -259,7 +265,14 @@
         uint32_t tn = 0, ts = 0, tp = 0;
         for (int k = 0; k < SHADE_WAVES; k++) { uint32_t a = sh.w_next[k], b = sh.w_shadow[k]; sh.w_next[k] = tn; sh.w_shadow[k] = ts; tn += a; ts += b; }
         if (MATERIALS) for (int k = 0; k < SHADE_WAVES; k++) { uint32_t a = sh.w_spec[k]; sh.w_spec[k] = tn + tp; tp += a; }
-        sh.blk_base = (tn | ts | tp) ? atomicAdd(io.count_out, ((unsigned long long)ts << 32) | (tn + tp)) : 0ull;
+        const uint32_t seg = fp.segs > 1u ? blockIdx.x & (QUEUE_SEGMENTS - 1u) : 0u;
+#ifdef MRT_PROBE_SHADE_TAILS
+        unsigned long long *const tail = io.count_out + (fp.probe_tails ? (size_t)(blockIdx.x & 7u) * 16u : (size_t)seg * SEG_TAIL_STRIDE);
+#else
+        unsigned long long *const tail = io.count_out + (size_t)seg * SEG_TAIL_STRIDE;
+#endif
+        const unsigned long long first = (unsigned long long)seg * fp.seg_cap;
+        sh.blk_base = (tn | ts | tp) ? atomicAdd(tail, ((unsigned long long)ts << 32) | (tn + tp)) + ((first << 32) | first) : 0ull;
     }
     __syncthreads();
     const unsigned long long base = sh.blk_base;
@@ -372,9 +385,10 @@
     __shared__ ShadeShared sh;
     __shared__ uint32_t p_idx[2 * SHADE_THREADS], p_w[SHADE_WAVES];
     __shared__ float4 p_hit[2 * SHADE_THREADS];
-    const uint32_t n = io.count_in ? (uint32_t)*io.count_in : io.capacity;
+    const uint32_t seg = fp.segs > 1u ? blockIdx.x & (QUEUE_SEGMENTS - 1u) : 0u, range = fp.segs > 1u ? blockIdx.x / QUEUE_SEGMENTS : blockIdx.x, first = seg * fp.seg_cap;
+    const uint32_t n = io.count_in ? (uint32_t)io.count_in[(size_t)seg * SEG_TAIL_STRIDE] : io.capacity;
     const float4 miss = make_float4(-1.0f, 0.0f, 0.0f, __uint_as_float(0xFFFFFFFFu)), noB = make_float4(0.0f, 0.0f, 1.0f, 0.0f);
-    const uint32_t begin = blockIdx.x * fp.pack_range, end = min(n, begin + fp.pack_range);
+    const uint32_t begin = first + min(n, range * fp.pack_range), end = first + min(n, (range + 1u) * fp.pack_range);
     const uint32_t lane_ = threadIdx.x & 63, wv_ = threadIdx.x >> 6;
     uint32_t head = 0, tail = 0, cur = begin;
     for (;;) {
diff --git a/metal-raytracing_amd/csrc/traverse_wide.h b/metal-raytracing_amd/csrc/traverse_wide.h
--- a/metal-raytracing_amd/csrc/traverse_wide.h
+++ b/metal-raytracing_amd/csrc/traverse_wide.h
@@ -417,6 +417,28 @@
             if (c >= Cp) continue;
             const uint32_t first = subframes && p2 ? n_next : 0u, lim = subframes && !p2 ? n_next : n;
             ob = first + c * chunk; oe = min(lim, ob + chunk);
+            return true;
+        }
+        return false;
+    }
+};
+
+constexpr uint32_t SEG_SHADOW_BIT = 0x80000000u;
+struct SegRegions {
+    uint32_t *counters; const unsigned long long *tails; uint32_t seg_cap, chunk; uint32_t home; uint32_t tries = 0;
+    MRT_DEV bool operator()(uint32_t &ob, uint32_t &oe) {
+        while (tries < 8u) {
+            const uint32_t x = (home + tries) & 7u;
+            const unsigned long long c = tails[(size_t)x * 16u];
+            const uint32_t n1 = (uint32_t)c, n2 = (uint32_t)(c >> 32), C1 = (n1 + chunk - 1u) / chunk, C = C1 + (n2 + chunk - 1u) / chunk;
+            if (C == 0u) { tries++; continue; }
+            uint32_t k = 0;
+            if ((threadIdx.x & 63) == 0) k = atomicAdd(&counters[x * XCD_COUNTER_STRIDE], 1u);
+            k = (uint32_t)__builtin_amdgcn_readfirstlane((int)k);
+            if (k >= C) { tries++; continue; }
+            const bool p2 = k >= C1;
+            const uint32_t kk = p2 ? k - C1 : k, lim = p2 ? n2 : n1, first = x * seg_cap, flag = p2 ? SEG_SHADOW_BIT : 0u;
+            ob = (first + kk * chunk) | flag; oe = (first + min(lim, (kk + 1u) * chunk)) | flag;
             return true;
         }
         return false;
```

Result: faster. 14800, median of 6 (+3.0%).
